# patrickfrey/strusPattern

Measured on AMD Instinct MI355X. Metric: GB/s input text scanned + matches/s, 10k-regex lexer + 10k-rule automaton, higher is better.
Workload: dtype u64; 1 GPU; configs[4] per-GPU shard: 10001 regexes + 10000 token rules, 12288 docs x 64KiB UTF-8 per step (the same 805 MB resident in HBM every step; configs[4] asks 32 GB per GPU: 39 such steps)

## Files before the change

### include/strus_pattern_amd.h

```cpp
#ifndef STRUS_PATTERN_AMD_H
#define STRUS_PATTERN_AMD_H
#include <stddef.h>
#include <stdint.h>

#ifdef __cplusplus
extern "C" {
#endif

#define SP_OK                    0
#define SP_ERR_INVALID          -1
#define SP_ERR_NOMEM            -2
#define SP_ERR_DEVICE           -3
#define SP_ERR_COMPILE          -4
#define SP_ERR_MATCH            -5
#define SP_ERR_UNAVAILABLE      -6

#define SP_DOC_OK                0
#define SP_DOC_ERR_ORDER         1
#define SP_DOC_ERR_ARENA         2
#define SP_DOC_ERR_KEYTRIGGERS   3
#define SP_DOC_ERR_PASTFOLLOW    4
#define SP_DOC_ERR_RANGE         5
#define SP_DOC_ERR_DATAREF       6
#define SP_DOC_ERR_LEXEMSIZE     7
#define SP_DOC_ERR_INTERNAL      8
#define SP_DOC_ERR_OUTPUT        9

enum sp_join_op {
	SP_OP_SEQUENCE = 0, SP_OP_SEQUENCE_IMM = 1, SP_OP_SEQUENCE_STRUCT = 2,
	SP_OP_WITHIN = 3, SP_OP_WITHIN_STRUCT = 4, SP_OP_ANY = 5, SP_OP_AND = 6
};

enum sp_position_bind {
	SP_BIND_CONTENT = 0, SP_BIND_SUCCESSOR = 1, SP_BIND_PREDECESSOR = 2, SP_BIND_UNIQUE = 3
};

typedef struct sp_lexem {
	uint32_t id;
	uint32_t ordpos;
	uint32_t origpos;
	uint32_t origsize;
} sp_lexem_t;

typedef struct sp_result {
	uint32_t handle;
	uint32_t ordpos;
	uint32_t ordend;
	uint32_t origseg;
	uint32_t origpos;
	uint32_t origendseg;
	uint32_t origend;
	uint32_t item_begin;
	uint32_t item_count;
} sp_result_t;

typedef struct sp_result_item {
	uint32_t variable;
	uint32_t ordpos;
	uint32_t ordend;
	uint32_t origseg;
	uint32_t origpos;
	uint32_t origendseg;
	uint32_t origend;
} sp_result_item_t;

typedef struct sp_matcher_stats {
	double nofProgramsInstalled;
	double nofAltKeyProgramsInstalled;
	double nofSignalsFired;
	double nofTriggersAvgActive;
} sp_matcher_stats_t;

typedef struct sp_matcher sp_matcher_t;
typedef struct sp_matcher_ctx sp_matcher_ctx_t;
typedef struct sp_lexer sp_lexer_t;
typedef struct sp_lexer_ctx sp_lexer_ctx_t;

const char* sp_version(void);
int sp_device_count(void);
void sp_free(void* p);
void sp_test_fail_alloc_above(uint64_t bytes);
struct sp_match_batch;
int sp_match_batch_regroup(const sp_result_t* results, uint64_t nresults, const sp_result_item_t* items, uint64_t nitems,
	const uint32_t* result_format, const uint32_t* item_format, const uint64_t* doc_ranges, const int32_t* doc_status,
	size_t batch_ndocs, size_t first_doc, size_t ndocs, int exclusive, uint32_t max_result_size,
	struct sp_match_batch* out, char* err, size_t errsize);


sp_matcher_t* sp_matcher_create(void);
void sp_matcher_free(sp_matcher_t* m);
const char* sp_matcher_last_error(const sp_matcher_t* m);

int sp_matcher_define_term_frequency(sp_matcher_t* m, uint32_t termid, double df);
int sp_matcher_push_term(sp_matcher_t* m, uint32_t termid);
int sp_matcher_push_expression(sp_matcher_t* m, int joinop, size_t argc, uint32_t range, uint32_t cardinality);
int sp_matcher_push_pattern(sp_matcher_t* m, const char* name);
int sp_matcher_attach_variable(sp_matcher_t* m, const char* name);
int sp_matcher_define_pattern(sp_matcher_t* m, const char* name, const char* formatstring, int visible);
int sp_matcher_define_option(sp_matcher_t* m, const char* name, double value);
int sp_matcher_compile(sp_matcher_t* m);
uint32_t sp_matcher_pattern_id(const sp_matcher_t* m, const char* name);
const char* sp_matcher_pattern_name(const sp_matcher_t* m, uint32_t handle);
uint32_t sp_matcher_variable_id(const sp_matcher_t* m, const char* name);
const char* sp_matcher_variable_name(const sp_matcher_t* m, uint32_t variable);
size_t sp_matcher_dump_table(const sp_matcher_t* m, uint32_t** out);
int sp_matcher_fast_tier(const sp_matcher_t* m, char* why, size_t whysize);
int sp_matcher_result_set_tier(const sp_matcher_t* m, char* why, size_t whysize, uint32_t* alt_programs);
int sp_matcher_launch_plan(const sp_matcher_t* m, uint32_t ctx_flags, unsigned num_cus, unsigned fast_blocks_per_cu,
                           size_t ndocs, size_t nlexems, size_t rerun_docs, uint32_t arena_grows,
                           uint64_t min_results, uint64_t min_items, char* buf, size_t bufsize);

int sp_matcher_serialize(const sp_matcher_t* m, void** blob, size_t* size);
sp_matcher_t* sp_matcher_deserialize(const void* blob, size_t size, char* err, size_t errsize);

uint32_t sp_matcher_format_count(const sp_matcher_t* m);
const char* sp_matcher_format_string(const sp_matcher_t* m, uint32_t format_handle);

sp_matcher_ctx_t* sp_matcher_ctx_create(const sp_matcher_t* m, int device);
#define SP_CTX_RESULT_SETS       1u
sp_matcher_ctx_t* sp_matcher_ctx_create_ex(const sp_matcher_t* m, int device, uint32_t flags);
void sp_matcher_ctx_free(sp_matcher_ctx_t* c);
const char* sp_matcher_ctx_last_error(const sp_matcher_ctx_t* c);

int sp_matcher_ctx_put_input(sp_matcher_ctx_t* c, const sp_lexem_t* lexems, const uint32_t* origseg, size_t n);
int sp_matcher_ctx_fetch_results(sp_matcher_ctx_t* c, sp_result_t** results, size_t* nresults,
                                 sp_result_item_t** items, size_t* nitems);
int sp_matcher_ctx_fetch_formats(sp_matcher_ctx_t* c, const uint32_t** result_format, const uint32_t** item_format);
int sp_matcher_ctx_statistics(sp_matcher_ctx_t* c, sp_matcher_stats_t* out);
int sp_matcher_ctx_reset(sp_matcher_ctx_t* c);

typedef struct sp_match_batch {
	size_t ndocs;
	size_t nresults;
	size_t nitems;
	sp_result_t* results;
	sp_result_item_t* items;
	uint64_t* doc_result_offsets;
	uint64_t* doc_stats;
	int32_t* doc_status;
	uint32_t* result_format;
	uint32_t* item_format;
} sp_match_batch_t;

int sp_matcher_ctx_match_docs(sp_matcher_ctx_t* c, const sp_lexem_t* lexems, const uint32_t* origseg,
                              const uint64_t* doc_offsets, size_t ndocs, sp_match_batch_t* out);
void sp_match_batch_free(sp_match_batch_t* b);

typedef struct sp_match_device_batch {
	size_t ndocs;
	void* d_results;
	void* d_items;
	void* d_doc_result_offsets;
	void* d_doc_stats;
	void* d_doc_status;
	void* d_counters;
	void* d_result_format;
	void* d_item_format;
} sp_match_device_batch_t;
int sp_matcher_ctx_match_docs_device(sp_matcher_ctx_t* c, const void* d_lexems, const void* d_origseg,
                                     const void* d_doc_offsets, size_t ndocs, size_t nlexems,
                                     void* stream, sp_match_device_batch_t* out);
int sp_matcher_ctx_match_lexed_device(sp_matcher_ctx_t* c, const void* d_lexems, const void* d_doc_ranges,
                                      size_t ndocs, size_t nlexems_hint, void* stream, sp_match_device_batch_t* out);
typedef struct sp_match_finished_batch {
	size_t ndocs;
	void* d_results;
	void* d_items;
	void* d_doc_result_offsets;
	void* d_doc_item_offsets;
	void* d_result_format;
	void* d_item_format;
	void* d_totals;
} sp_match_finished_batch_t;
int sp_matcher_ctx_batch_finish_device(sp_matcher_ctx_t* c, void* stream, sp_match_finished_batch_t* out);
#define SP_FINISH_CANONICAL      1u
int sp_matcher_ctx_batch_finish_device_ex(sp_matcher_ctx_t* c, void* stream, uint32_t flags, sp_match_finished_batch_t* out);
int sp_matcher_ctx_finished_fetch(sp_matcher_ctx_t* c, sp_match_batch_t* out);
int sp_matcher_ctx_last_finish_ms(sp_matcher_ctx_t* c, double* count_ms, double* offsets_ms, double* place_ms);
int sp_matcher_ctx_last_finish_sort_ms(sp_matcher_ctx_t* c, double* sort_ms);
uint32_t sp_matcher_finish_sort_tile(void);

#define SP_TEXT_RESULTS 1u
#define SP_TEXT_ITEMS   2u
typedef struct sp_text_source {
	const void* d_text;
	uint64_t nbytes;
	const void* d_seg_offsets;
	size_t nseg;
	const void* d_doc_seg_offsets;
} sp_text_source_t;
typedef struct sp_match_text_batch {
	size_t ndocs;
	void* d_result_text;
	void* d_result_text_offsets;
	void* d_item_text;
	void* d_item_text_offsets;
	void* d_doc_text_status;
	void* d_totals;
} sp_match_text_batch_t;
typedef struct sp_match_text {
	size_t ndocs;
	size_t nresults;
	size_t nitems;
	char* result_text;
	uint64_t* result_text_offsets;
	char* item_text;
	uint64_t* item_text_offsets;
	int32_t* doc_text_status;
	uint64_t totals[2];
} sp_match_text_t;
int sp_matcher_ctx_finished_text_device(sp_matcher_ctx_t* c, const sp_text_source_t* src, uint32_t flags, void* stream, sp_match_text_batch_t* out);
int sp_matcher_ctx_finished_text_fetch(sp_matcher_ctx_t* c, sp_match_text_t* out);
void sp_match_text_free(sp_match_text_t* t);
int sp_matcher_ctx_last_text_ms(sp_matcher_ctx_t* c, double* ms);
uint32_t sp_matcher_text_long_span(void);
int sp_match_batch_text(const sp_match_batch_t* mb, const char* text, uint64_t nbytes, const uint64_t* seg_offsets,
                        size_t nseg, const uint64_t* doc_seg_offsets, uint32_t flags,
                        sp_match_text_t* out, char* err, size_t errsize);

#define SP_VALUE_RESULTS 1u
#define SP_VALUE_ITEMS   2u
typedef struct sp_match_values_batch {
	size_t ndocs;
	void* d_result_values;
	void* d_result_value_offsets;
	void* d_item_values;
	void* d_item_value_offsets;
	void* d_doc_value_status;
	void* d_totals;
} sp_match_values_batch_t;
typedef struct sp_match_values {
	size_t ndocs;
	size_t nresults;
	size_t nitems;
	char* result_values;
	uint64_t* result_value_offsets;
	char* item_values;
	uint64_t* item_value_offsets;
	int32_t* doc_value_status;
	uint64_t totals[2];
} sp_match_values_t;
int sp_matcher_ctx_finished_values_device(sp_matcher_ctx_t* c, const sp_text_source_t* src, uint32_t flags, void* stream, sp_match_values_batch_t* out);
int sp_matcher_ctx_finished_values_fetch(sp_matcher_ctx_t* c, sp_match_values_t* out);
void sp_match_values_free(sp_match_values_t* v);
int sp_matcher_ctx_last_values_ms(sp_matcher_ctx_t* c, double* ms);
uint32_t sp_matcher_value_max_depth(void);
int sp_match_batch_values(const sp_matcher_t* m, const sp_match_batch_t* mb, const char* text, uint64_t nbytes,
                          const uint64_t* seg_offsets, size_t nseg, const uint64_t* doc_seg_offsets, uint32_t flags,
                          sp_match_values_t* out, char* err, size_t errsize);

typedef struct sp_pattern_freq {
	uint32_t handle;
	uint32_t count;
	uint32_t first_ordpos;
	uint32_t last_ordend;
} sp_pattern_freq_t;
typedef struct sp_pattern_freq_device {
	size_t ndocs;
	uint32_t handle_bound;
	void* d_records;
	void* d_doc_offsets;
	void* d_doc_freq_status;
	void* d_handle_results;
	void* d_handle_docs;
	void* d_totals;
} sp_pattern_freq_device_t;
typedef struct sp_pattern_freq_batch {
	size_t ndocs;
	size_t nrecords;
	uint32_t handle_bound;
	sp_pattern_freq_t* records;
	uint64_t* doc_offsets;
	int32_t* doc_freq_status;
	uint64_t* handle_results;
	uint32_t* handle_docs;
	uint64_t totals[1];
} sp_pattern_freq_batch_t;
uint32_t sp_matcher_handle_bound(const sp_matcher_t* m);
int sp_matcher_ctx_finished_pattern_freq_device(sp_matcher_ctx_t* c, void* stream, sp_pattern_freq_device_t* out);
int sp_matcher_ctx_finished_pattern_freq_fetch(sp_matcher_ctx_t* c, sp_pattern_freq_batch_t* out);
void sp_pattern_freq_batch_free(sp_pattern_freq_batch_t* b);
int sp_matcher_ctx_last_pattern_freq_ms(sp_matcher_ctx_t* c, double* ms);
uint32_t sp_matcher_pattern_freq_window(void);
int sp_match_batch_pattern_freq(const sp_match_batch_t* mb, uint32_t handle_bound, sp_pattern_freq_batch_t* out,
                                char* err, size_t errsize);

#define SP_TERM_VALUES 1u
#define SP_TERM_TEXT   2u
typedef struct sp_match_term {
	uint32_t handle;
	uint32_t count;
	uint32_t first_ordpos;
	uint32_t last_ordend;
	uint32_t first_result;
	uint32_t value_bytes;
} sp_match_term_t;
typedef struct sp_match_terms_device {
	size_t ndocs;
	uint32_t handle_bound;
	uint32_t flags;
	void* d_records;
	void* d_doc_term_offsets;
	void* d_result_term;
	void* d_doc_term_status;
	void* d_totals;
} sp_match_terms_device_t;
typedef struct sp_match_terms {
	size_t ndocs;
	size_t nresults;
	size_t nrecords;
	uint32_t handle_bound;
	uint32_t flags;
	sp_match_term_t* records;
	uint64_t* doc_term_offsets;
	uint32_t* result_term;
	int32_t* doc_term_status;
	uint64_t totals[1];
} sp_match_terms_t;
int sp_matcher_ctx_finished_terms_device(sp_matcher_ctx_t* c, uint32_t flags, void* stream, sp_match_terms_device_t* out);
int sp_matcher_ctx_finished_terms_fetch(sp_matcher_ctx_t* c, sp_match_terms_t* out);
void sp_match_terms_free(sp_match_terms_t* t);
int sp_matcher_ctx_last_terms_ms(sp_matcher_ctx_t* c, double* ms);
uint32_t sp_matcher_term_tile(void);
void sp_test_term_hash_bits(unsigned bits);
int sp_match_batch_terms(const sp_match_batch_t* mb, const sp_match_values_t* values, const sp_match_text_t* text,
                         uint32_t handle_bound, uint32_t flags, sp_match_terms_t* out, char* err, size_t errsize);

typedef struct sp_dict_term {
	uint32_t handle;
	uint32_t value_bytes;
	uint32_t first_doc;
	uint32_t first_term;
	uint32_t doc_freq;
	uint32_t max_count;
	uint64_t count;
} sp_dict_term_t;
typedef struct sp_match_dictionary_device {
	size_t ndocs;
	uint32_t handle_bound;
	uint32_t flags;
	void* d_records;
	void* d_term_dict;
	void* d_doc_dict_offsets;
	void* d_handle_terms;
	void* d_totals;
} sp_match_dictionary_device_t;
typedef struct sp_match_dictionary {
	size_t ndocs;
	size_t nterms;
	size_t ndict;
	uint32_t handle_bound;
	uint32_t flags;
	sp_dict_term_t* records;
	uint32_t* term_dict;
	uint64_t* doc_dict_offsets;
	uint32_t* handle_terms;
	uint64_t totals[1];
} sp_match_dictionary_t;
int sp_matcher_ctx_finished_dictionary_device(sp_matcher_ctx_t* c, void* stream, sp_match_dictionary_device_t* out);
int sp_matcher_ctx_finished_dictionary_fetch(sp_matcher_ctx_t* c, sp_match_dictionary_t* out);
void sp_match_dictionary_free(sp_match_dictionary_t* d);
int sp_matcher_ctx_last_dictionary_ms(sp_matcher_ctx_t* c, double* ms);
int sp_match_batch_dictionary(const sp_match_batch_t* mb, const sp_match_values_t* values, const sp_match_text_t* text,
                              const sp_match_terms_t* terms, sp_match_dictionary_t* out, char* err, size_t errsize);
int sp_matcher_ctx_batch_fetch(sp_matcher_ctx_t* c, sp_match_batch_t* out);
int sp_matcher_ctx_batch_fetch_docs(sp_matcher_ctx_t* c, size_t first_doc, size_t ndocs, sp_match_batch_t* out);
int sp_matcher_ctx_batch_counters(sp_matcher_ctx_t* c, uint64_t counters[8]);
double sp_matcher_ctx_last_kernel_ms(sp_matcher_ctx_t* c);
int sp_matcher_ctx_kernel_kind(const sp_matcher_ctx_t* c);
const char* sp_matcher_ctx_kernel_name(const sp_matcher_ctx_t* c);
int sp_matcher_ctx_batch_status(sp_matcher_ctx_t* c, int32_t* status, size_t ndocs);
int sp_matcher_ctx_grow_arena(sp_matcher_ctx_t* c);
int sp_matcher_ctx_reserve_output(sp_matcher_ctx_t* c, uint64_t results, uint64_t items);
int sp_matcher_ctx_set_arena(sp_matcher_ctx_t* c, uint32_t max_rules, uint32_t max_triggers, uint32_t bucket_capacity,
                             uint32_t max_items, uint32_t max_follow);


sp_lexer_t* sp_lexer_create(void);
void sp_lexer_free(sp_lexer_t* l);
const char* sp_lexer_last_error(const sp_lexer_t* l);

int sp_lexer_define_lexem_name(sp_lexer_t* l, uint32_t id, const char* name);
const char* sp_lexer_get_lexem_name(const sp_lexer_t* l, uint32_t id);
int sp_lexer_define_lexem(sp_lexer_t* l, uint32_t id, const char* expression, uint32_t resultIndex,
                          uint32_t level, int posbind);
int sp_lexer_define_symbol(sp_lexer_t* l, uint32_t symbolid, uint32_t patternid, const char* name);
uint32_t sp_lexer_get_symbol(const sp_lexer_t* l, uint32_t patternid, const char* name);
int sp_lexer_define_option(sp_lexer_t* l, const char* name, double value);
int sp_lexer_compile(sp_lexer_t* l);
int sp_lexer_serialize(const sp_lexer_t* l, void** blob, size_t* size);
sp_lexer_t* sp_lexer_deserialize(const void* blob, size_t size, char* err, size_t errsize);
size_t sp_lexer_dump_tables(const sp_lexer_t* l, uint64_t** out);
size_t sp_lexer_dump_image(const sp_lexer_t* l, int which, uint64_t** out);
int sp_lexer_launch_plan(const sp_lexer_t* l, unsigned num_cus, size_t ndocs, size_t nbytes, char* buf, size_t bufsize);

sp_lexer_ctx_t* sp_lexer_ctx_create(const sp_lexer_t* l, int device);
void sp_lexer_ctx_free(sp_lexer_ctx_t* c);
const char* sp_lexer_ctx_last_error(const sp_lexer_ctx_t* c);
int sp_lexer_ctx_match(sp_lexer_ctx_t* c, const char* src, size_t srclen, sp_lexem_t** lexems, size_t* nlexems);
int sp_lexer_ctx_reset(sp_lexer_ctx_t* c);

typedef struct sp_lex_batch {
	size_t ndocs;
	size_t nlexems;
	sp_lexem_t* lexems;
	uint64_t* doc_lexem_offsets;
	int32_t* doc_status;
} sp_lex_batch_t;
int sp_lexer_ctx_match_docs(sp_lexer_ctx_t* c, const char* text, const uint64_t* doc_offsets, size_t ndocs, sp_lex_batch_t* out);
void sp_lex_batch_free(sp_lex_batch_t* b);

typedef struct sp_lex_device_batch {
	size_t ndocs;
	void* d_lexems;
	void* d_doc_ranges;
	void* d_doc_status;
	void* d_counters;
} sp_lex_device_batch_t;
int sp_lexer_ctx_match_docs_device(sp_lexer_ctx_t* c, const void* d_text, const void* d_doc_offsets,
                                   size_t ndocs, size_t nbytes, void* stream, sp_lex_device_batch_t* out);
int sp_lexer_ctx_batch_fetch_docs(sp_lexer_ctx_t* c, size_t first_doc, size_t ndocs, sp_lex_batch_t* out);
typedef struct sp_lex_stitched_batch {
	size_t ndocs;
	void* d_lexems;
	void* d_origseg;
	void* d_doc_offsets;
	void* d_doc_status;
	void* d_totals;
} sp_lex_stitched_batch_t;
int sp_lexer_ctx_stitch_segments_device(sp_lexer_ctx_t* c, const void* d_doc_seg_offsets, size_t ndocs,
                                        void* stream, sp_lex_stitched_batch_t* out);
int sp_lexer_ctx_stitched_fetch(sp_lexer_ctx_t* c, sp_lex_batch_t* out, uint32_t** origseg);
int sp_lexer_ctx_stitched_status(sp_lexer_ctx_t* c, int32_t* status, size_t ndocs, size_t* ndocs_stitched);
int sp_lexer_ctx_last_stitch_ms(sp_lexer_ctx_t* c, double* ms);
int sp_lexer_ctx_batch_counters(sp_lexer_ctx_t* c, uint64_t counters[8]);
int sp_lexer_ctx_batch_status(sp_lexer_ctx_t* c, int32_t* status, size_t ndocs);
double sp_lexer_ctx_last_kernel_ms(sp_lexer_ctx_t* c);
int sp_lexer_ctx_last_kernel_ms_split(sp_lexer_ctx_t* c, double* scan_ms, double* post_ms);
int sp_lexer_ctx_last_kernel_ms_split3(sp_lexer_ctx_t* c, double* scan_ms, double* words_ms, double* post_ms);
const char* sp_lexer_ctx_scan_kernel_name(const sp_lexer_ctx_t* c);
const char* sp_lexer_ctx_words_kernel_name(const sp_lexer_ctx_t* c);
int sp_lexer_ctx_reserve_output(sp_lexer_ctx_t* c, uint64_t lexems);
int sp_lexer_ctx_grow_arena(sp_lexer_ctx_t* c);

#ifdef __cplusplus
}
#endif
#endif
```

### struspattern_amd/__init__.py

```python
import ctypes

import numpy as np

from . import capi
from .capi import SpLexem, SpResult, SpResultItem

__all__ = ["PatternMatcher", "PatternMatcherInstance", "PatternMatcherContext", "PatternLexer", "PatternLexerInstance",
           "PatternLexerContext", "PatternError", "JOIN_OP", "POSITION_BIND", "matchSegmentedDocs", "MatchText", "batchText", "MatchValues", "batchValues", "PatternFreq", "batchPatternFreq", "MatchTerms", "batchTerms", "MatchDictionary", "batchDictionary"]

SP_CTX_RESULT_SETS = 1
SP_FINISH_CANONICAL = 1
SP_TEXT_RESULTS, SP_TEXT_ITEMS = 1, 2
SP_VALUE_RESULTS, SP_VALUE_ITEMS = 1, 2
SP_TERM_VALUES, SP_TERM_TEXT = 1, 2
SP_ERR_UNAVAILABLE = -6

JOIN_OP = {"sequence": 0, "sequence_imm": 1, "sequence_struct": 2, "within": 3, "within_struct": 4, "any": 5, "and": 6}

DOC_STATUS = {
    0: "ok", 1: "term events not fed in ascending order", 2: "working set of the document exceeds the arena",
    3: "pattern with too many identical key events defined", 4: "internal: encountered past trigger with follow",
    5: "term event out of range", 6: "illegal free of event data reference",
}

# ... 372 lines not shown
            return _match_batch_of(b)
        finally:
            self._L.sp_match_batch_free(ctypes.byref(b))

    def matchDocsDevice(self, d_lexems, d_doc_offsets, ndocs, nlexems, stream=0, d_origseg=0):
        out = capi.SpMatchDeviceBatch()
        rc = self._L.sp_matcher_ctx_match_docs_device(self._h, d_lexems, d_origseg or None, d_doc_offsets, ndocs, nlexems, stream or None, ctypes.byref(out))
        if rc != 0:
            raise PatternError("device batch match failed (%d): %s" % (rc, self._err()))
        return out

    def matchLexedDevice(self, d_lexems, d_doc_ranges, ndocs, nlexems_hint, stream=0):
        out = capi.SpMatchDeviceBatch()
        rc = self._L.sp_matcher_ctx_match_lexed_device(self._h, d_lexems, d_doc_ranges, ndocs, nlexems_hint, stream or None, ctypes.byref(out))
        if rc != 0:
            raise PatternError("device batch match failed (%d): %s" % (rc, self._err()))
        return out

    def batchFinishDevice(self, stream=0, canonical=False):
        out = capi.SpMatchFinishedBatch()
        rc = self._L.sp_matcher_ctx_batch_finish_device_ex(self._h, stream or None, SP_FINISH_CANONICAL if canonical else 0, ctypes.byref(out))
        if rc != 0:
            raise PatternError("finishing the batch on the device failed (%d): %s" % (rc, self._err()))
        return out

    def finishedFetch(self):
        return self._fetched(self._L.sp_matcher_ctx_finished_fetch)

    def _fetch_product(self, struct_type, call, free, convert, what):
        return _product(struct_type, lambda s: call(self._h, ctypes.byref(s)), free, convert,
                        lambda rc: "fetching %s failed (%d): %s" % (what, rc, self._err()))

    def _last_ms(self, fn, what):
        a = ctypes.c_double(-1.0)
        if fn(self._h, ctypes.byref(a)) != 0:
            raise PatternError("no timed " + what)
        return a.value

    def lastFinishMs(self):
        a, b, d = ctypes.c_double(-1.0), ctypes.c_double(-1.0), ctypes.c_double(-1.0)
        if self._L.sp_matcher_ctx_last_finish_ms(self._h, ctypes.byref(a), ctypes.byref(b), ctypes.byref(d)) != 0:
            raise PatternError("no timed finish")
        return a.value, b.value, d.value

    def lastFinishSortMs(self):
        return self._last_ms(self._L.sp_matcher_ctx_last_finish_sort_ms, "finish")

    def finishedTextDevice(self, d_text, nbytes, d_seg_offsets, nseg, d_doc_seg_offsets=0, results=True, items=True, stream=0):
        src = capi.SpTextSource(d_text or None, nbytes, d_seg_offsets or None, nseg, d_doc_seg_offsets or None)
        out = capi.SpMatchTextBatch()
        flags = (SP_TEXT_RESULTS if results else 0) | (SP_TEXT_ITEMS if items else 0)
        rc = self._L.sp_matcher_ctx_finished_text_device(self._h, ctypes.byref(src), flags, stream or None, ctypes.byref(out))
        if rc != 0:
            raise PatternError("gathering the text of the batch on the device failed (%d): %s" % (rc, self._err()))
        return out

    def finishedTextFetch(self):
        return self._fetch_product(capi.SpMatchText, self._L.sp_matcher_ctx_finished_text_fetch, self._L.sp_match_text_free, _match_text_of, "the text of the batch")

    def lastTextMs(self):
        return self._last_ms(self._L.sp_matcher_ctx_last_text_ms, "text call")

    def finishedValuesDevice(self, d_text, nbytes, d_seg_offsets, nseg, d_doc_seg_offsets=0, flags=SP_VALUE_RESULTS | SP_VALUE_ITEMS, stream=0):
        src = capi.SpTextSource(d_text or None, nbytes, d_seg_offsets or None, nseg, d_doc_seg_offsets or None)
        out = capi.SpMatchValuesBatch()
        rc = self._L.sp_matcher_ctx_finished_values_device(self._h, ctypes.byref(src), flags, stream or None, ctypes.byref(out))
        if rc != 0:
            raise PatternError("building the values of the batch on the device failed (%d): %s" % (rc, self._err()))
        return out

    def finishedValuesFetch(self):
        return self._fetch_product(capi.SpMatchValues, self._L.sp_matcher_ctx_finished_values_fetch, self._L.sp_match_values_free, _match_values_of, "the values of the batch")

    def lastValuesMs(self):
        return self._last_ms(self._L.sp_matcher_ctx_last_values_ms, "values call")

    def finishedPatternFreqDevice(self, stream=0):
        out = capi.SpPatternFreqDevice()
        rc = self._L.sp_matcher_ctx_finished_pattern_freq_device(self._h, stream or None, ctypes.byref(out))
        if rc != 0:
            raise PatternError("summing the pattern frequencies of the batch on the device failed (%d): %s" % (rc, self._err()))
        return out

    def finishedPatternFreqFetch(self):
        return self._fetch_product(capi.SpPatternFreqBatch, self._L.sp_matcher_ctx_finished_pattern_freq_fetch, self._L.sp_pattern_freq_batch_free, _pattern_freq_of,
                                   "the pattern frequencies of the batch")

    def lastPatternFreqMs(self):
        return self._last_ms(self._L.sp_matcher_ctx_last_pattern_freq_ms, "pattern frequency call")

    def finishedTermsDevice(self, flags=SP_TERM_VALUES | SP_TERM_TEXT, stream=0):
        out = capi.SpMatchTermsDevice()
        rc = self._L.sp_matcher_ctx_finished_terms_device(self._h, flags, stream or None, ctypes.byref(out))
        if rc != 0:
            raise PatternError("grouping the terms of the batch on the device failed (%d): %s" % (rc, self._err()))
        return out

    def finishedTermsFetch(self):
        return self._fetch_product(capi.SpMatchTerms, self._L.sp_matcher_ctx_finished_terms_fetch, self._L.sp_match_terms_free, _match_terms_of, "the terms of the batch")

    def lastTermsMs(self):
        return self._last_ms(self._L.sp_matcher_ctx_last_terms_ms, "terms call")

    def finishedDictionaryDevice(self, stream=0):
        out = capi.SpMatchDictionaryDevice()
        rc = self._L.sp_matcher_ctx_finished_dictionary_device(self._h, stream or None, ctypes.byref(out))
        if rc != 0:
            raise PatternError("building the dictionary of the batch on the device failed (%d): %s" % (rc, self._err()))
        return out

    def finishedDictionaryFetch(self):
        return self._fetch_product(capi.SpMatchDictionary, self._L.sp_matcher_ctx_finished_dictionary_fetch, self._L.sp_match_dictionary_free,
                                   _match_dictionary_of, "the dictionary of the batch")

    def lastDictionaryMs(self):
        return self._last_ms(self._L.sp_matcher_ctx_last_dictionary_ms, "dictionary call")

    def batchFetch(self, first_doc=None, ndocs=None):
        if first_doc is None:
            return self._fetched(self._L.sp_matcher_ctx_batch_fetch)
        return self._fetched(lambda h, b: self._L.sp_matcher_ctx_batch_fetch_docs(h, first_doc, ndocs, b))

    def _fetched(self, call):
        return self._fetch_product(capi.SpMatchBatch, call, self._L.sp_match_batch_free, _match_batch_of, "the batch")

    def batchCounters(self):
        arr = (ctypes.c_uint64 * 8)()
        rc = self._L.sp_matcher_ctx_batch_counters(self._h, arr)
        if rc != 0:
            raise PatternError("reading batch counters failed: " + self._err())
        return {"results": arr[0], "items": arr[1], "events": arr[2], "failed_docs": arr[3], "handed_over": arr[4], "prof": [arr[4], arr[5], arr[6], arr[7]]}

    def batchStatus(self, ndocs):
        st = np.zeros(ndocs, np.int32)
        rc = self._L.sp_matcher_ctx_batch_status(self._h, st.ctypes.data, ndocs)
        if rc != 0:
            raise PatternError("reading batch status failed: " + self._err())
        return st

    def growArena(self):
        return self._L.sp_matcher_ctx_grow_arena(self._h) == 0

    def reserveOutput(self, results, items):
        self._L.sp_matcher_ctx_reserve_output(self._h, results, items)

    def lastKernelMs(self):
        return self._L.sp_matcher_ctx_last_kernel_ms(self._h)

    def kernelKind(self):
        return self._L.sp_matcher_ctx_kernel_kind(self._h)

    def kernelName(self):
        return self._L.sp_matcher_ctx_kernel_name(self._h).decode()


def _serialize(L, fn, handle, err):
    blob = ctypes.c_void_p()
    size = ctypes.c_size_t()
    if fn(handle, ctypes.byref(blob), ctypes.byref(size)) != 0:
        raise PatternError("serialisation failed: " + err())
    try:
        return ctypes.string_at(blob, size.value)
    finally:
        L.sp_free(blob)


class PatternMatcherInstance:

    def __init__(self, _handle=None):
        self._L = capi.lib()
        self._h = _handle or self._L.sp_matcher_create()
        if not self._h:
            raise PatternError("failed to create pattern matcher instance")

    def serialize(self):
        return _serialize(self._L, self._L.sp_matcher_serialize, self._h, lambda: self._L.sp_matcher_last_error(self._h).decode())

    @classmethod
    def deserialize(cls, blob):
        L = capi.lib()
        err = ctypes.create_string_buffer(256)
        h = L.sp_matcher_deserialize(blob, len(blob), err, 256)
        if not h:
            raise PatternError("cannot load the rule set: " + err.value.decode())
        return cls(_handle=h)

    def __del__(self):
        try:
            if self._h:
                self._L.sp_matcher_free(self._h)
        except Exception:
            pass

    def _chk(self, rc, what):
        if rc != 0:
            raise PatternError("%s: %s" % (what, self._L.sp_matcher_last_error(self._h).decode()))

    def defineTermFrequency(self, termid, df):
        self._chk(self._L.sp_matcher_define_term_frequency(self._h, termid, df), "failed to define term frequency")

    def pushTerm(self, termid):
        self._chk(self._L.sp_matcher_push_term(self._h, termid), "failed to push term on the pattern match expression stack")

    def pushExpression(self, joinop, argc, range_, cardinality=0):
        op = JOIN_OP[joinop] if isinstance(joinop, str) else int(joinop)
        self._chk(self._L.sp_matcher_push_expression(self._h, op, argc, range_, cardinality), "failed to push expression on the pattern match expression stack")

    def pushPattern(self, name):
        self._chk(self._L.sp_matcher_push_pattern(self._h, name.encode()), "failed to push pattern reference on the pattern match expression stack")

    def attachVariable(self, name):
        self._chk(self._L.sp_matcher_attach_variable(self._h, name.encode()), "failed to attach variable to top element of the pattern match expression stack")

    def definePattern(self, name, formatstring="", visible=True):
        self._chk(self._L.sp_matcher_define_pattern(self._h, name.encode(), formatstring.encode(), int(visible)), "failed to close pattern definition on the pattern match expression stack")

    def defineOption(self, name, value=0.0):
        self._chk(self._L.sp_matcher_define_option(self._h, name.encode(), value), "failed to define pattern matching automaton option")

    def compile(self):
        self._chk(self._L.sp_matcher_compile(self._h), "failed to compile (optimize) pattern matching automaton")
        return True

    def createContext(self, device=0, result_sets=False):
        return PatternMatcherContext(self, device, result_sets)

    def handleBound(self):
        return self._L.sp_matcher_handle_bound(self._h)

    def patternId(self, name):
        return self._L.sp_matcher_pattern_id(self._h, name.encode())

    def patternName(self, handle):
        s = self._L.sp_matcher_pattern_name(self._h, handle)
        return s.decode() if s else None

    def variableId(self, name):
        return self._L.sp_matcher_variable_id(self._h, name.encode())

    def variableName(self, vid):
        s = self._L.sp_matcher_variable_name(self._h, vid)
        return s.decode() if s else None

    def formatCount(self):
        return int(self._L.sp_matcher_format_count(self._h))

    def formatString(self, handle):
        s = self._L.sp_matcher_format_string(self._h, handle)
        return s.decode() if s else None

    def fastTier(self):
        buf = ctypes.create_string_buffer(256)
        ok = self._L.sp_matcher_fast_tier(self._h, buf, 256)
        return bool(ok), buf.value.decode()

    def resultSetTier(self):
        buf = ctypes.create_string_buffer(256)
        alt = ctypes.c_uint32(0)
        ok = self._L.sp_matcher_result_set_tier(self._h, buf, 256, ctypes.byref(alt))
        return bool(ok), buf.value.decode(), int(alt.value)

    def launchPlan(self, num_cus, ndocs, nlexems, result_sets=False, fast_blocks_per_cu=16, rerun_docs=0, arena_grows=0, min_results=0, min_items=0):
        buf = ctypes.create_string_buffer(2048)
        self._chk(self._L.sp_matcher_launch_plan(self._h, 1 if result_sets else 0, num_cus, fast_blocks_per_cu, ndocs, nlexems, rerun_docs, arena_grows,
                                                 min_results, min_items, buf, 2048), "no launch plan")
        return dict(f.split("=", 1) for f in buf.value.decode().split("\n") if f)

    def dumpTable(self):
        p = ctypes.POINTER(ctypes.c_uint32)()
        n = self._L.sp_matcher_dump_table(self._h, ctypes.byref(p))
        arr = np.ctypeslib.as_array(p, shape=(n,)).copy() if n else np.zeros(0, np.uint32)
        self._L.sp_free(p)
        return arr

    def name(self):
        return "std"


class PatternMatcher:

    def getCompileOptionNames(self):
        return ["stopwordOccurrenceFactor", "weightFactor", "maxRange", "exclusive", "maxResultSize"]

    def createInstance(self):
        return PatternMatcherInstance()

    def name(self):
        return "std"


POSITION_BIND = {"content": 0, "successor": 1, "predecessor": 2, "unique": 3}


class LexBatch:
    def __init__(self, lexems, doc_offsets, status):
        self.lexems = lexems
        self.doc_offsets = doc_offsets
        self.status = status

    def doc(self, i):
        return self.lexems[self.doc_offsets[i]:self.doc_offsets[i + 1]]


def _lex_batch_of(b):
    return LexBatch(_rows(b.lexems, b.nlexems, 4), _rows(b.doc_lexem_offsets, b.ndocs + 1, 0, ctypes.c_uint64), _rows(b.doc_status, b.ndocs, 0, ctypes.c_int32))

# ... 294 lines not shown
```

### struspattern_amd/capi.py

```python
import ctypes
import os

from . import build as _build

c_u32 = ctypes.c_uint32
c_u64 = ctypes.c_uint64
c_vp = ctypes.c_void_p
c_cp = ctypes.c_char_p
P = ctypes.POINTER


class SpLexem(ctypes.Structure):
    _fields_ = [("id", c_u32), ("ordpos", c_u32), ("origpos", c_u32), ("origsize", c_u32)]


class SpResult(ctypes.Structure):
    _fields_ = [(n, c_u32) for n in ("handle", "ordpos", "ordend", "origseg", "origpos", "origendseg", "origend", "item_begin", "item_count")]


class SpResultItem(ctypes.Structure):
    _fields_ = [(n, c_u32) for n in ("variable", "ordpos", "ordend", "origseg", "origpos", "origendseg", "origend")]


class SpMatcherStats(ctypes.Structure):
    _fields_ = [(n, ctypes.c_double) for n in ("nofProgramsInstalled", "nofAltKeyProgramsInstalled", "nofSignalsFired", "nofTriggersAvgActive")]


class SpMatchBatch(ctypes.Structure):
    _fields_ = [
        ("ndocs", ctypes.c_size_t), ("nresults", ctypes.c_size_t), ("nitems", ctypes.c_size_t),
        ("results", P(SpResult)), ("items", P(SpResultItem)),
        ("doc_result_offsets", P(c_u64)), ("doc_stats", P(c_u64)), ("doc_status", P(ctypes.c_int32)),
        ("result_format", P(c_u32)), ("item_format", P(c_u32)),
    ]


class SpLexBatch(ctypes.Structure):
    _fields_ = [
        ("ndocs", ctypes.c_size_t), ("nlexems", ctypes.c_size_t), ("lexems", P(SpLexem)),
        ("doc_lexem_offsets", P(c_u64)), ("doc_status", P(ctypes.c_int32)),
    ]


class SpLexDeviceBatch(ctypes.Structure):
    _fields_ = [("ndocs", ctypes.c_size_t), ("d_lexems", c_vp), ("d_doc_ranges", c_vp), ("d_doc_status", c_vp), ("d_counters", c_vp)]


class SpLexStitchedBatch(ctypes.Structure):
    _fields_ = [("ndocs", ctypes.c_size_t), ("d_lexems", c_vp), ("d_origseg", c_vp), ("d_doc_offsets", c_vp), ("d_doc_status", c_vp), ("d_totals", c_vp)]


class SpMatchDeviceBatch(ctypes.Structure):
    _fields_ = [
        ("ndocs", ctypes.c_size_t), ("d_results", c_vp), ("d_items", c_vp), ("d_doc_result_offsets", c_vp),
        ("d_doc_stats", c_vp), ("d_doc_status", c_vp), ("d_counters", c_vp),
        ("d_result_format", c_vp), ("d_item_format", c_vp),
    ]


class SpMatchFinishedBatch(ctypes.Structure):
    _fields_ = [
        ("ndocs", ctypes.c_size_t), ("d_results", c_vp), ("d_items", c_vp), ("d_doc_result_offsets", c_vp),
        ("d_doc_item_offsets", c_vp), ("d_result_format", c_vp), ("d_item_format", c_vp), ("d_totals", c_vp),
    ]


class SpTextSource(ctypes.Structure):
    _fields_ = [("d_text", c_vp), ("nbytes", c_u64), ("d_seg_offsets", c_vp), ("nseg", ctypes.c_size_t), ("d_doc_seg_offsets", c_vp)]


class SpMatchTextBatch(ctypes.Structure):
    _fields_ = [
        ("ndocs", ctypes.c_size_t), ("d_result_text", c_vp), ("d_result_text_offsets", c_vp), ("d_item_text", c_vp),
        ("d_item_text_offsets", c_vp), ("d_doc_text_status", c_vp), ("d_totals", c_vp),
    ]


class SpMatchText(ctypes.Structure):
    _fields_ = [
        ("ndocs", ctypes.c_size_t), ("nresults", ctypes.c_size_t), ("nitems", ctypes.c_size_t),
        ("result_text", P(ctypes.c_uint8)), ("result_text_offsets", P(c_u64)), ("item_text", P(ctypes.c_uint8)), ("item_text_offsets", P(c_u64)),
        ("doc_text_status", P(ctypes.c_int32)), ("totals", c_u64 * 2),
    ]


class SpMatchValuesBatch(ctypes.Structure):
    _fields_ = [
        ("ndocs", ctypes.c_size_t), ("d_result_values", c_vp), ("d_result_value_offsets", c_vp), ("d_item_values", c_vp),
        ("d_item_value_offsets", c_vp), ("d_doc_value_status", c_vp), ("d_totals", c_vp),
    ]


class SpMatchValues(ctypes.Structure):
    _fields_ = [
        ("ndocs", ctypes.c_size_t), ("nresults", ctypes.c_size_t), ("nitems", ctypes.c_size_t),
        ("result_values", P(ctypes.c_uint8)), ("result_value_offsets", P(c_u64)), ("item_values", P(ctypes.c_uint8)), ("item_value_offsets", P(c_u64)),
        ("doc_value_status", P(ctypes.c_int32)), ("totals", c_u64 * 2),
    ]


class SpPatternFreq(ctypes.Structure):
    _fields_ = [(n, c_u32) for n in ("handle", "count", "first_ordpos", "last_ordend")]


class SpPatternFreqDevice(ctypes.Structure):
    _fields_ = [
        ("ndocs", ctypes.c_size_t), ("handle_bound", c_u32), ("d_records", c_vp), ("d_doc_offsets", c_vp), ("d_doc_freq_status", c_vp),
        ("d_handle_results", c_vp), ("d_handle_docs", c_vp), ("d_totals", c_vp),
    ]


class SpPatternFreqBatch(ctypes.Structure):
    _fields_ = [
        ("ndocs", ctypes.c_size_t), ("nrecords", ctypes.c_size_t), ("handle_bound", c_u32),
        ("records", P(SpPatternFreq)), ("doc_offsets", P(c_u64)), ("doc_freq_status", P(ctypes.c_int32)),
        ("handle_results", P(c_u64)), ("handle_docs", P(c_u32)), ("totals", c_u64 * 1),
    ]


class SpMatchTerm(ctypes.Structure):
    _fields_ = [(n, c_u32) for n in ("handle", "count", "first_ordpos", "last_ordend", "first_result", "value_bytes")]


class SpMatchTermsDevice(ctypes.Structure):
    _fields_ = [
        ("ndocs", ctypes.c_size_t), ("handle_bound", c_u32), ("flags", c_u32), ("d_records", c_vp), ("d_doc_term_offsets", c_vp),
        ("d_result_term", c_vp), ("d_doc_term_status", c_vp), ("d_totals", c_vp),
    ]


class SpMatchTerms(ctypes.Structure):
    _fields_ = [
        ("ndocs", ctypes.c_size_t), ("nresults", ctypes.c_size_t), ("nrecords", ctypes.c_size_t), ("handle_bound", c_u32), ("flags", c_u32),
        ("records", P(SpMatchTerm)), ("doc_term_offsets", P(c_u64)), ("result_term", P(c_u32)), ("doc_term_status", P(ctypes.c_int32)),
        ("totals", c_u64 * 1),
    ]


class SpDictTerm(ctypes.Structure):
    _fields_ = [(n, c_u32) for n in ("handle", "value_bytes", "first_doc", "first_term", "doc_freq", "max_count")] + [("count", c_u64)]


class SpMatchDictionaryDevice(ctypes.Structure):
    _fields_ = [
        ("ndocs", ctypes.c_size_t), ("handle_bound", c_u32), ("flags", c_u32), ("d_records", c_vp), ("d_term_dict", c_vp),
        ("d_doc_dict_offsets", c_vp), ("d_handle_terms", c_vp), ("d_totals", c_vp),
    ]


class SpMatchDictionary(ctypes.Structure):
    _fields_ = [
        ("ndocs", ctypes.c_size_t), ("nterms", ctypes.c_size_t), ("ndict", ctypes.c_size_t), ("handle_bound", c_u32), ("flags", c_u32),
        ("records", P(SpDictTerm)), ("term_dict", P(c_u32)), ("doc_dict_offsets", P(c_u64)), ("handle_terms", P(c_u32)),
        ("totals", c_u64 * 1),
    ]


SIGNATURES = {
    "sp_version": (c_cp, []),
    "sp_device_count": (ctypes.c_int, []),
    "sp_free": (None, [c_vp]),
    "sp_test_fail_alloc_above": (None, [c_u64]),
    "sp_match_batch_regroup": (ctypes.c_int, [c_vp, c_u64, c_vp, c_u64, c_vp, c_vp, c_vp, c_vp, ctypes.c_size_t, ctypes.c_size_t, ctypes.c_size_t,
                                              ctypes.c_int, c_u32, P(SpMatchBatch), ctypes.c_char_p, ctypes.c_size_t]),
    "sp_matcher_create": (c_vp, []),
    "sp_matcher_free": (None, [c_vp]),
    "sp_matcher_last_error": (c_cp, [c_vp]),
    "sp_matcher_define_term_frequency": (ctypes.c_int, [c_vp, c_u32, ctypes.c_double]),
    "sp_matcher_push_term": (ctypes.c_int, [c_vp, c_u32]),
    "sp_matcher_push_expression": (ctypes.c_int, [c_vp, ctypes.c_int, ctypes.c_size_t, c_u32, c_u32]),
    "sp_matcher_push_pattern": (ctypes.c_int, [c_vp, c_cp]),
    "sp_matcher_attach_variable": (ctypes.c_int, [c_vp, c_cp]),
    "sp_matcher_define_pattern": (ctypes.c_int, [c_vp, c_cp, c_cp, ctypes.c_int]),
    "sp_matcher_define_option": (ctypes.c_int, [c_vp, c_cp, ctypes.c_double]),
    "sp_matcher_compile": (ctypes.c_int, [c_vp]),
    "sp_matcher_pattern_id": (c_u32, [c_vp, c_cp]),
    "sp_matcher_pattern_name": (c_cp, [c_vp, c_u32]),
    "sp_matcher_variable_id": (c_u32, [c_vp, c_cp]),
    "sp_matcher_variable_name": (c_cp, [c_vp, c_u32]),
    "sp_matcher_dump_table": (ctypes.c_size_t, [c_vp, P(P(c_u32))]),
    "sp_matcher_fast_tier": (ctypes.c_int, [c_vp, ctypes.c_char_p, ctypes.c_size_t]),
    "sp_matcher_result_set_tier": (ctypes.c_int, [c_vp, ctypes.c_char_p, ctypes.c_size_t, P(c_u32)]),
    "sp_matcher_launch_plan": (ctypes.c_int, [c_vp, c_u32, ctypes.c_uint, ctypes.c_uint, ctypes.c_size_t, ctypes.c_size_t, ctypes.c_size_t, c_u32, c_u64, c_u64, ctypes.c_char_p, ctypes.c_size_t]),
    "sp_matcher_serialize": (ctypes.c_int, [c_vp, P(c_vp), P(ctypes.c_size_t)]),
    "sp_matcher_deserialize": (c_vp, [c_vp, ctypes.c_size_t, ctypes.c_char_p, ctypes.c_size_t]),
    "sp_lexer_serialize": (ctypes.c_int, [c_vp, P(c_vp), P(ctypes.c_size_t)]),
    "sp_lexer_deserialize": (c_vp, [c_vp, ctypes.c_size_t, ctypes.c_char_p, ctypes.c_size_t]),
    "sp_matcher_format_count": (c_u32, [c_vp]),
    "sp_matcher_format_string": (c_cp, [c_vp, c_u32]),
    "sp_matcher_ctx_fetch_formats": (ctypes.c_int, [c_vp, P(P(c_u32)), P(P(c_u32))]),
    "sp_matcher_ctx_create": (c_vp, [c_vp, ctypes.c_int]),
    "sp_matcher_ctx_create_ex": (c_vp, [c_vp, ctypes.c_int, c_u32]),
    "sp_matcher_ctx_free": (None, [c_vp]),
    "sp_matcher_ctx_last_error": (c_cp, [c_vp]),
    "sp_matcher_ctx_put_input": (ctypes.c_int, [c_vp, c_vp, c_vp, ctypes.c_size_t]),
    "sp_matcher_ctx_fetch_results": (ctypes.c_int, [c_vp, P(P(SpResult)), P(ctypes.c_size_t), P(P(SpResultItem)), P(ctypes.c_size_t)]),
    "sp_matcher_ctx_statistics": (ctypes.c_int, [c_vp, P(SpMatcherStats)]),
    "sp_matcher_ctx_reset": (ctypes.c_int, [c_vp]),
    "sp_matcher_ctx_match_docs": (ctypes.c_int, [c_vp, c_vp, c_vp, c_vp, ctypes.c_size_t, P(SpMatchBatch)]),
    "sp_match_batch_free": (None, [P(SpMatchBatch)]),
    "sp_matcher_ctx_match_docs_device": (ctypes.c_int, [c_vp, c_vp, c_vp, c_vp, ctypes.c_size_t, ctypes.c_size_t, c_vp, P(SpMatchDeviceBatch)]),
    "sp_matcher_ctx_match_lexed_device": (ctypes.c_int, [c_vp, c_vp, c_vp, ctypes.c_size_t, ctypes.c_size_t, c_vp, P(SpMatchDeviceBatch)]),
    "sp_matcher_ctx_batch_fetch": (ctypes.c_int, [c_vp, P(SpMatchBatch)]),
    "sp_matcher_ctx_batch_fetch_docs": (ctypes.c_int, [c_vp, ctypes.c_size_t, ctypes.c_size_t, P(SpMatchBatch)]),
    "sp_matcher_ctx_batch_finish_device": (ctypes.c_int, [c_vp, c_vp, P(SpMatchFinishedBatch)]),
    "sp_matcher_ctx_batch_finish_device_ex": (ctypes.c_int, [c_vp, c_vp, c_u32, P(SpMatchFinishedBatch)]),
    "sp_matcher_ctx_finished_fetch": (ctypes.c_int, [c_vp, P(SpMatchBatch)]),
    "sp_matcher_ctx_last_finish_ms": (ctypes.c_int, [c_vp, P(ctypes.c_double), P(ctypes.c_double), P(ctypes.c_double)]),
    "sp_matcher_ctx_last_finish_sort_ms": (ctypes.c_int, [c_vp, P(ctypes.c_double)]),
    "sp_matcher_finish_sort_tile": (c_u32, []),
    "sp_matcher_ctx_finished_text_device": (ctypes.c_int, [c_vp, P(SpTextSource), c_u32, c_vp, P(SpMatchTextBatch)]),
    "sp_matcher_ctx_finished_text_fetch": (ctypes.c_int, [c_vp, P(SpMatchText)]),
    "sp_match_text_free": (None, [P(SpMatchText)]),
    "sp_matcher_ctx_last_text_ms": (ctypes.c_int, [c_vp, P(ctypes.c_double)]),
    "sp_matcher_text_long_span": (c_u32, []),
    "sp_matcher_ctx_finished_values_device": (ctypes.c_int, [c_vp, P(SpTextSource), c_u32, c_vp, P(SpMatchValuesBatch)]),
    "sp_matcher_ctx_finished_values_fetch": (ctypes.c_int, [c_vp, P(SpMatchValues)]),
    "sp_match_values_free": (None, [P(SpMatchValues)]),
    "sp_matcher_ctx_last_values_ms": (ctypes.c_int, [c_vp, P(ctypes.c_double)]),
    "sp_matcher_value_max_depth": (c_u32, []),
    "sp_match_batch_values": (ctypes.c_int, [c_vp, P(SpMatchBatch), c_vp, c_u64, c_vp, ctypes.c_size_t, c_vp, c_u32, P(SpMatchValues), ctypes.c_char_p, ctypes.c_size_t]),
    "sp_match_batch_text": (ctypes.c_int, [P(SpMatchBatch), c_vp, c_u64, c_vp, ctypes.c_size_t, c_vp, c_u32, P(SpMatchText), ctypes.c_char_p, ctypes.c_size_t]),
    "sp_matcher_handle_bound": (c_u32, [c_vp]),
    "sp_matcher_ctx_finished_pattern_freq_device": (ctypes.c_int, [c_vp, c_vp, P(SpPatternFreqDevice)]),
    "sp_matcher_ctx_finished_pattern_freq_fetch": (ctypes.c_int, [c_vp, P(SpPatternFreqBatch)]),
    "sp_pattern_freq_batch_free": (None, [P(SpPatternFreqBatch)]),
    "sp_matcher_ctx_last_pattern_freq_ms": (ctypes.c_int, [c_vp, P(ctypes.c_double)]),
    "sp_matcher_pattern_freq_window": (c_u32, []),
    "sp_match_batch_pattern_freq": (ctypes.c_int, [P(SpMatchBatch), c_u32, P(SpPatternFreqBatch), ctypes.c_char_p, ctypes.c_size_t]),
    "sp_matcher_ctx_finished_terms_device": (ctypes.c_int, [c_vp, c_u32, c_vp, P(SpMatchTermsDevice)]),
    "sp_matcher_ctx_finished_terms_fetch": (ctypes.c_int, [c_vp, P(SpMatchTerms)]),
    "sp_match_terms_free": (None, [P(SpMatchTerms)]),
    "sp_matcher_ctx_last_terms_ms": (ctypes.c_int, [c_vp, P(ctypes.c_double)]),
    "sp_matcher_term_tile": (c_u32, []),
    "sp_test_term_hash_bits": (None, [ctypes.c_uint]),
    "sp_match_batch_terms": (ctypes.c_int, [P(SpMatchBatch), P(SpMatchValues), P(SpMatchText), c_u32, c_u32, P(SpMatchTerms), ctypes.c_char_p, ctypes.c_size_t]),
    "sp_matcher_ctx_finished_dictionary_device": (ctypes.c_int, [c_vp, c_vp, P(SpMatchDictionaryDevice)]),
    "sp_matcher_ctx_finished_dictionary_fetch": (ctypes.c_int, [c_vp, P(SpMatchDictionary)]),
    "sp_match_dictionary_free": (None, [P(SpMatchDictionary)]),
    "sp_matcher_ctx_last_dictionary_ms": (ctypes.c_int, [c_vp, P(ctypes.c_double)]),
    "sp_match_batch_dictionary": (ctypes.c_int, [P(SpMatchBatch), P(SpMatchValues), P(SpMatchText), P(SpMatchTerms), P(SpMatchDictionary), ctypes.c_char_p, ctypes.c_size_t]),
    "sp_matcher_ctx_batch_counters": (ctypes.c_int, [c_vp, P(c_u64)]),
    "sp_matcher_ctx_last_kernel_ms": (ctypes.c_double, [c_vp]),
    "sp_matcher_ctx_kernel_kind": (ctypes.c_int, [c_vp]),
    "sp_matcher_ctx_kernel_name": (ctypes.c_char_p, [c_vp]),
    "sp_matcher_ctx_batch_status": (ctypes.c_int, [c_vp, c_vp, ctypes.c_size_t]),
    "sp_matcher_ctx_grow_arena": (ctypes.c_int, [c_vp]),
    "sp_matcher_ctx_reserve_output": (ctypes.c_int, [c_vp, c_u64, c_u64]),
    "sp_matcher_ctx_set_arena": (ctypes.c_int, [c_vp, c_u32, c_u32, c_u32, c_u32, c_u32]),
    "sp_lexer_create": (c_vp, []),
    "sp_lexer_free": (None, [c_vp]),
    "sp_lexer_last_error": (c_cp, [c_vp]),
    "sp_lexer_define_lexem_name": (ctypes.c_int, [c_vp, c_u32, c_cp]),
    "sp_lexer_get_lexem_name": (c_cp, [c_vp, c_u32]),
    "sp_lexer_define_lexem": (ctypes.c_int, [c_vp, c_u32, c_cp, c_u32, c_u32, ctypes.c_int]),
    "sp_lexer_define_symbol": (ctypes.c_int, [c_vp, c_u32, c_u32, c_cp]),
    "sp_lexer_get_symbol": (c_u32, [c_vp, c_u32, c_cp]),
    "sp_lexer_define_option": (ctypes.c_int, [c_vp, c_cp, ctypes.c_double]),
    "sp_lexer_compile": (ctypes.c_int, [c_vp]),
    "sp_lexer_dump_tables": (ctypes.c_size_t, [c_vp, P(P(c_u64))]),
    "sp_lexer_dump_image": (ctypes.c_size_t, [c_vp, ctypes.c_int, P(P(c_u64))]),
    "sp_lexer_launch_plan": (ctypes.c_int, [c_vp, ctypes.c_uint, ctypes.c_size_t, ctypes.c_size_t, ctypes.c_char_p, ctypes.c_size_t]),
    "sp_lexer_ctx_create": (c_vp, [c_vp, ctypes.c_int]),
    "sp_lexer_ctx_free": (None, [c_vp]),
    "sp_lexer_ctx_last_error": (c_cp, [c_vp]),
    "sp_lexer_ctx_match": (ctypes.c_int, [c_vp, c_cp, ctypes.c_size_t, P(P(SpLexem)), P(ctypes.c_size_t)]),
    "sp_lexer_ctx_reset": (ctypes.c_int, [c_vp]),
    "sp_lexer_ctx_match_docs": (ctypes.c_int, [c_vp, c_cp, c_vp, ctypes.c_size_t, P(SpLexBatch)]),
    "sp_lex_batch_free": (None, [P(SpLexBatch)]),
    "sp_lexer_ctx_match_docs_device": (ctypes.c_int, [c_vp, c_vp, c_vp, ctypes.c_size_t, ctypes.c_size_t, c_vp, P(SpLexDeviceBatch)]),
    "sp_lexer_ctx_batch_fetch_docs": (ctypes.c_int, [c_vp, ctypes.c_size_t, ctypes.c_size_t, P(SpLexBatch)]),
    "sp_lexer_ctx_stitch_segments_device": (ctypes.c_int, [c_vp, c_vp, ctypes.c_size_t, c_vp, P(SpLexStitchedBatch)]),
    "sp_lexer_ctx_stitched_fetch": (ctypes.c_int, [c_vp, P(SpLexBatch), P(P(c_u32))]),
    "sp_lexer_ctx_stitched_status": (ctypes.c_int, [c_vp, c_vp, ctypes.c_size_t, P(ctypes.c_size_t)]),
    "sp_lexer_ctx_last_stitch_ms": (ctypes.c_int, [c_vp, P(ctypes.c_double)]),
    "sp_lexer_ctx_batch_counters": (ctypes.c_int, [c_vp, P(c_u64)]),
    "sp_lexer_ctx_batch_status": (ctypes.c_int, [c_vp, c_vp, ctypes.c_size_t]),
    "sp_lexer_ctx_last_kernel_ms": (ctypes.c_double, [c_vp]),
    "sp_lexer_ctx_last_kernel_ms_split": (ctypes.c_int, [c_vp, ctypes.POINTER(ctypes.c_double), ctypes.POINTER(ctypes.c_double)]),
    "sp_lexer_ctx_scan_kernel_name": (ctypes.c_char_p, [c_vp]),
    "sp_lexer_ctx_words_kernel_name": (ctypes.c_char_p, [c_vp]),
    "sp_lexer_ctx_last_kernel_ms_split3": (ctypes.c_int, [c_vp, ctypes.POINTER(ctypes.c_double), ctypes.POINTER(ctypes.c_double), ctypes.POINTER(ctypes.c_double)]),
    "sp_lexer_ctx_reserve_output": (ctypes.c_int, [c_vp, c_u64]),
    "sp_lexer_ctx_grow_arena": (ctypes.c_int, [c_vp]),
}

_LIB = None


def lib():
    global _LIB
    if _LIB is None:
        path = _build.LIB
        if _build.needs_build():
            path = _build.build()
        L = ctypes.CDLL(path, mode=ctypes.RTLD_GLOBAL)
        for name, (res, args) in SIGNATURES.items():
            fn = getattr(L, name)
            fn.restype = res
            fn.argtypes = args
        _LIB = L
    return _LIB
```

### struspattern_amd/csrc/capi_l2.cpp

```cpp
#include "capi_l2_ctx.hpp"
#include <cstdio>

namespace {

L2Engine engineOf( const sp_matcher* m, uint32_t flags, const L2Switches& sw, FlatTables& ft)
{
	m->compiler.flatten( ft);
	return chooseL2Engine( m->compiler, ft, flags, sw);
}

FlatPlan flatPlanOf( const L2Engine& e, const L2Switches& sw)
{
	const char size[ 2] = {sw.fastSize, 0};
	const unsigned variant = fastVariantNamed( size);
	uint32_t R = 0, T = 0;
	fastCapacities( variant, R, T);
	return planFlat( e.flat, variant, fastKernelName( variant), R, T);
}

int tierQuery( const sp_matcher* m, uint32_t flags, L2EngineKind kind, char* why, size_t whysize, uint32_t* altPrograms)
{
	if (altPrograms) *altPrograms = 0;
	try
	{
		FlatTables ft;
		const L2Engine e = engineOf( m, flags, L2Switches(), ft);
		const std::string& reason = kind == L2_JOIN ? e.join.whyNot : e.flat.whyNot;
		copyText( why, whysize, reason.c_str());
		if (altPrograms) *altPrograms = e.altPrograms;
		return reason.empty() ? 1 : 0;
	}
	catch (const std::exception& e)
	{
		copyText( why, whysize, e.what());
		return 0;
	}
}

}

extern "C" {

const char* sp_version(void) { return "struspattern_amd 0.1 (gfx950)"; }

int sp_device_count(void)
{
	int n = 0;
	if (hipGetDeviceCount( &n) != hipSuccess) return 0;
	return n;
}

void sp_free( void* p) { std::free( p); }

void sp_test_fail_alloc_above( uint64_t bytes) { allocFailureThreshold().store( bytes, std::memory_order_relaxed); }

sp_matcher_t* sp_matcher_create(void) { try { return new sp_matcher(); } catch (...) { return 0; } }
void sp_matcher_free( sp_matcher_t* m) { delete m; }
const char* sp_matcher_last_error( const sp_matcher_t* m) { return m->lasterror.c_str(); }

#define MGUARD( CODE, BODY) return guardedCall( m->lasterror, CODE, [&]{ BODY; })

int sp_matcher_define_term_frequency( sp_matcher_t* m, uint32_t termid, double df)
{ MGUARD( SP_ERR_INVALID, m->compiler.defineTermFrequency( termid, df)); }
int sp_matcher_push_term( sp_matcher_t* m, uint32_t termid)
{ MGUARD( SP_ERR_INVALID, m->compiler.pushTerm( termid)); }
int sp_matcher_push_expression( sp_matcher_t* m, int joinop, size_t argc, uint32_t range, uint32_t cardinality)
{ MGUARD( SP_ERR_INVALID, m->compiler.pushExpression( joinop, argc, range, cardinality)); }
int sp_matcher_push_pattern( sp_matcher_t* m, const char* name)
{ MGUARD( SP_ERR_INVALID, m->compiler.pushPattern( name ? name : "")); }
int sp_matcher_attach_variable( sp_matcher_t* m, const char* name)
{ MGUARD( SP_ERR_INVALID, m->compiler.attachVariable( name ? name : "")); }
int sp_matcher_define_pattern( sp_matcher_t* m, const char* name, const char* formatstring, int visible)
{ MGUARD( SP_ERR_INVALID, m->compiler.definePattern( name ? name : "", formatstring ? formatstring : "", visible != 0)); }
int sp_matcher_define_option( sp_matcher_t* m, const char* name, double value)
{ MGUARD( SP_ERR_INVALID, m->compiler.defineOption( name ? name : "", value)); }
int sp_matcher_compile( sp_matcher_t* m)
{ MGUARD( SP_ERR_COMPILE, m->compiler.compile(); m->compiled = true; m->formats( true)); }

uint32_t sp_matcher_pattern_id( const sp_matcher_t* m, const char* name) { return m->compiler.patterns().get( name); }
const char* sp_matcher_pattern_name( const sp_matcher_t* m, uint32_t handle) { return m->compiler.patterns().key( handle); }
uint32_t sp_matcher_variable_id( const sp_matcher_t* m, const char* name) { return m->compiler.variables().get( name); }
const char* sp_matcher_variable_name( const sp_matcher_t* m, uint32_t variable) { return m->compiler.variables().key( variable); }

uint32_t sp_matcher_handle_bound( const sp_matcher_t* m) { return (uint32_t)m->compiler.patterns().names().size() + 1; }

uint32_t sp_matcher_format_count( const sp_matcher_t* m) { return m->compiler.formatCount(); }
const char* sp_matcher_format_string( const sp_matcher_t* m, uint32_t format_handle) { return m->compiler.formatString( format_handle); }

int sp_matcher_ctx_kernel_kind( const sp_matcher_ctx_t* c) { return c->kind; }
const char* sp_matcher_ctx_kernel_name( const sp_matcher_ctx_t* c) { return l2KernelName( c->kind, &c->flat.plan); }

int sp_matcher_fast_tier( const sp_matcher_t* m, char* why, size_t whysize)
{ return tierQuery( m, 0, L2_FLAT, why, whysize, 0); }

int sp_matcher_result_set_tier( const sp_matcher_t* m, char* why, size_t whysize, uint32_t* alt_programs)
{ return tierQuery( m, SP_CTX_RESULT_SETS, L2_JOIN, why, whysize, alt_programs); }

int sp_matcher_launch_plan( const sp_matcher_t* m, uint32_t ctx_flags, unsigned num_cus, unsigned fast_blocks_per_cu, size_t ndocs, size_t nlexems,
			    size_t rerun_docs, uint32_t arena_grows, uint64_t min_results, uint64_t min_items, char* buf, size_t bufsize)
{
	if (buf && bufsize) buf[ 0] = 0;
	return guardedCall( m->lasterror, SP_ERR_INVALID, [&]{
		if (ctx_flags & ~(uint32_t)SP_CTX_RESULT_SETS) throw std::runtime_error( "unknown context flags");
		const L2Switches sw = L2Switches::fromEnv();
		FlatTables ft;
		const L2Engine e = engineOf( m, ctx_flags, sw, ft);
		const FlatPlan fp = e.flat.on ? flatPlanOf( e, sw) : FlatPlan();
		ArenaLayout arena = initialArena();
		arena.nStop = ft.nofStopWords;
		for (uint32_t i=0; i<arena_grows; ++i) if (!growArena( arena)) throw std::runtime_error( "arena at its maximum size");
		const L2LaunchPlan p = planL2Launch( e.kind(), rerun_docs != 0, num_cus ? num_cus : 256u, fast_blocks_per_cu, rerun_docs ? rerun_docs : ndocs, ndocs, nlexems,
							arena, &fp, min_results, min_items);
		static const char* const engines[] = {"general", "flat", "join"};
		static const char* const routes[] = {"general", "flat+list", "join", "rerun-list"};
		int n = std::snprintf( buf, bufsize, "engine=%s\nkind=%d\nflat_why_not=%s\njoin_why_not=%s\nalt_programs=%u\nkernel=%s\nroute=%s\n"
			"general_blocks=%u\narena_run=%u\narena_alloc=%u\narena_alloc_waves=%u\narena_per_wave_bytes=%zu\narena_max_rules=%u\narena_scratch_cap=%u\nstop_words=%u\n"
			"fast_blocks=%u\nspill_alloc_waves=%llu\nspill_per_wave_bytes=%zu\nlist_blocks=%u\njoin_blocks=%u\nwant_results=%llu\nwant_items=%llu\n"
			"R=%u\nT=%u\nexp_shift=%u\nspill_words=%u\nmax_rules=%u\nmax_staged=%u\nbucket_caps=",
			engines[ e.kind()], (int)e.kind(), e.flat.whyNot.c_str(), e.join.whyNot.c_str(), e.altPrograms, p.kernelName, routes[ p.route],
			p.generalBlocks, p.arena.run, p.arena.alloc, p.arenaAllocWaves, p.arenaPerWaveBytes, p.layout.maxRules, p.layout.scratchCap, ft.nofStopWords,
			p.fastBlocks, (unsigned long long)p.spillAllocWaves, p.spillPerWaveBytes, p.listBlocks, p.joinBlocks, (unsigned long long)p.wantResults, (unsigned long long)p.wantItems,
			fp.R, fp.T, fp.expShift, fp.spill.totalWords, fp.spill.maxRules, fp.spill.maxStaged);
		for (int b=0; b<16 && n >= 0 && buf && (size_t)n < bufsize; ++b) n += std::snprintf( buf+n, bufsize-n, b ? ",%u" : "%u", fp.bucketMeta[ b] >> 16);
		if (n < 0 || !buf || (size_t)n >= bufsize) throw std::runtime_error( "buffer too small for the launch plan");
	});
}

int sp_matcher_serialize( const sp_matcher_t* m, void** blob, size_t* size)
{ return exportBlob( m->lasterror, blob, size, [&]( std::vector<uint8_t>& buf){ m->compiler.save( buf, m->compiled); }); }
sp_matcher_t* sp_matcher_deserialize( const void* blob, size_t size, char* err, size_t errsize)
{ return importBlob<sp_matcher>( err, errsize, [&]( sp_matcher& m){ m.compiled = m.compiler.load( blob, size); m.formats( true); }); }

size_t sp_matcher_dump_table( const sp_matcher_t* m, uint32_t** out)
{
	std::vector<uint32_t> buf = m->compiler.dump();
	*out = (uint32_t*)std::malloc( buf.size()*sizeof(uint32_t) + 4);
	if (!*out) return 0;
	std::memcpy( *out, buf.data(), buf.size()*sizeof(uint32_t));
	return buf.size();
}

sp_matcher_ctx_t* sp_matcher_ctx_create( const sp_matcher_t* m, int device) { return sp_matcher_ctx_create_ex( m, device, 0); }

sp_matcher_ctx_t* sp_matcher_ctx_create_ex( const sp_matcher_t* m, int device, uint32_t flags)
{
	sp_matcher_ctx* c = 0;
	if (flags & ~(uint32_t)SP_CTX_RESULT_SETS)
	{
		m->lasterror = "unknown context flags";
		return 0;
	}
	try
	{
		c = new sp_matcher_ctx();
		c->inst = m; c->device = device;
		int ndev = 0;
		hipError_t e = hipGetDeviceCount( &ndev);
		if (e != hipSuccess || ndev <= 0 || device < 0 || device >= ndev)
		{
			m->lasterror = "no usable HIP device: the rule automaton runs on the GPU only (no CPU fallback)";
			delete c; return 0;
		}
		HIP_CHECK( hipSetDevice( device));
		hipDeviceProp_t prop;
		HIP_CHECK( hipGetDeviceProperties( &prop, device));
		c->numCUs = prop.multiProcessorCount > 0 ? (unsigned)prop.multiProcessorCount : 256u;

		c->sw = L2Switches::fromEnv();
		FlatTables ft;
		const L2Engine engine = engineOf( m, flags, c->sw, ft);
		c->kind = engine.kind();
		c->exact.dPrograms.upload( ft.programs.data(), ft.programs.size()*sizeof(DevProgram));
		c->exact.dTrigdefs.upload( ft.trigdefs.data(), ft.trigdefs.size()*sizeof(DevTrigDef));
		c->exact.dKeytab.upload( ft.keytab.data(), ft.keytab.size()*sizeof(DevKeyEntry));
		c->exact.dKeylist.upload( ft.keylist.data(), ft.keylist.size()*sizeof(DevKeyRef));
		c->exact.keymask = (uint32_t)ft.keytab.size()-1;
		c->exact.nofStopWords = ft.nofStopWords;
		c->exact.layout.nStop = ft.nofStopWords;
		c->io.withFormats = m->compiler.formatCount() != 0;
		c->flat.on = engine.flat.on; c->flat.whyNot = engine.flat.whyNot;
		if (c->flat.on)
		{
			c->flat.dKeyinst.upload( engine.flat.keyinst.data(), engine.flat.keyinst.size()*sizeof(FastKeyInst));
			c->flat.dStatics.upload( engine.flat.statics.data(), engine.flat.statics.size()*sizeof(FastStatic));
			c->flat.plan = flatPlanOf( engine, c->sw);
			c->flat.blocksPerCU = (unsigned)fastBlocksPerCU( c->flat.plan.variant);
		}
		if (c->sw.verbose) fprintf( stderr, "[spa] fast tier: %s\n", c->flat.on ? "on" : c->flat.whyNot.c_str());
		c->join.on = engine.join.on; c->join.whyNot = engine.join.whyNot;
		if (c->join.on)
		{
			const L2Engine::Join& j = engine.join;
			c->join.dKeytab.upload( j.keytab.data(), j.keytab.size()*sizeof(JoinKey)); c->join.dRules.upload( j.rules.data(), j.rules.size()*sizeof(JoinRule)); c->join.dFilter.upload( j.filter.data(), j.filter.size()*sizeof(uint32_t));
			c->join.keymask = (uint32_t)j.keytab.size()-1; c->join.maxRange = j.maxRange; c->join.delimiter = j.delimiter;
			c->join.altRules = engine.altPrograms != 0;
		}
		if (c->sw.verbose && engine.join.asked) fprintf( stderr, "[spa] result-set mode: %s\n", c->join.on ? "join kernel" : c->join.whyNot.c_str());
		c->io.dCursor.alloc( 256);
		c->io.dCounters.alloc( SPC_COUNT*sizeof(uint64_t));
		c->own.create( device);
		c->evStart.create(); c->evStop.create();
		return c;
	}
	catch (const std::exception& e)
	{
		m->lasterror = e.what();
		delete c;
		return 0;
	}
}

void sp_matcher_ctx_free( sp_matcher_ctx_t* c) { delete c; }
const char* sp_matcher_ctx_last_error( const sp_matcher_ctx_t* c) { return c->lasterror.c_str(); }

int sp_matcher_ctx_set_arena( sp_matcher_ctx_t* c, uint32_t max_rules, uint32_t max_triggers, uint32_t bucket_capacity,
				uint32_t max_items, uint32_t max_follow)
{
	setArena( c->exact.layout, max_rules, max_triggers, bucket_capacity, max_items, max_follow);
	c->exact.arena.count = 0;
	return SP_OK;
}

}

namespace {

void copyOutBatch( sp_matcher_ctx* c, size_t firstDoc, size_t ndocs, const BatchCounts& counts, sp_match_batch_t* out)
{
	MatchBatchSource src;
	src.results = (const sp_result_t*)c->io.results.ptr(); src.nresults = counts.results;
	src.items = (const sp_result_item_t*)c->io.items.ptr(); src.nitems = counts.items;
	src.resultFormat = c->io.withFormats ? (const uint32_t*)c->io.dResultFormat.ptr : 0;
	src.itemFormat = c->io.withFormats ? (const uint32_t*)c->io.dItemFormat.ptr : 0;
	src.docRange = (const uint64_t*)c->io.dDocRange.ptr; src.docStatus = (const int32_t*)c->io.dDocStatus.ptr;
	src.docStats = (const uint64_t*)c->io.dDocStats.ptr;
	src.ndocs = c->lastNdocs;
	fetchMatchBatch( src, firstDoc, ndocs, c->inst->compiler.exclusive(), c->inst->compiler.maxResultSize(), deviceToHost( c->own), out);
}

}

extern "C" {

int sp_matcher_ctx_batch_fetch_docs( sp_matcher_ctx_t* c, size_t first_doc, size_t ndocs, sp_match_batch_t* out)
{
	std::memset( out, 0, sizeof(*out));
	return guardedCall( c->lasterror, SP_ERR_DEVICE, [&]{
		HIP_CHECK( hipSetDevice( c->device));
		HIP_CHECK( hipStreamSynchronize( c->lastStream));
		copyOutBatch( c, first_doc, ndocs, readCounts( c), out);
	});
}

int sp_matcher_ctx_batch_fetch( sp_matcher_ctx_t* c, sp_match_batch_t* out) { return sp_matcher_ctx_batch_fetch_docs( c, 0, c->lastNdocs, out); }

int sp_matcher_ctx_batch_status( sp_matcher_ctx_t* c, int32_t* status, size_t ndocs) { return batchStatus( c, c->io.dDocStatus, status, ndocs); }

int sp_matcher_ctx_grow_arena( sp_matcher_ctx_t* c)
{
	if (!growArena( c->exact.layout)) { c->lasterror = "arena at its maximum size"; return SP_ERR_INVALID; }
	c->exact.arena.count = 0;
	return SP_OK;
}

int sp_matcher_ctx_reserve_output( sp_matcher_ctx_t* c, uint64_t results, uint64_t items)
{
	if (results > c->io.minResults) c->io.minResults = results;
	if (items > c->io.minItems) c->io.minItems = items;
	return SP_OK;
}

}

namespace {

L2BatchIO batchIO( sp_matcher_ctx* c, const void* d_lexems, const void* d_origseg, const void* d_doc_offsets, const void* d_doc_ranges, size_t ndocs)
{
	L2BatchIO io;
	std::memset( &io, 0, sizeof(io));
	io.lexems = (const uint32_t*)d_lexems; io.origseg = (const uint32_t*)d_origseg;
	io.docOffsets = (const uint64_t*)d_doc_offsets; io.docRangesIn = (const uint64_t*)d_doc_ranges;
	io.ndocs = (uint32_t)ndocs; io.withItems = c->io.withItems ? 1u : 0u;
	io.docCursor = (uint32_t*)c->io.dCursor.ptr;
	io.counters = (uint64_t*)c->io.dCounters.ptr;
	io.results = (uint32_t*)c->io.results.ptr(); io.resultCapacity = c->io.results.count;
	io.items = (uint32_t*)c->io.items.ptr(); io.itemCapacity = c->io.items.count;
	io.docRange = (uint64_t*)c->io.dDocRange.ptr; io.docStats = (uint64_t*)c->io.dDocStats.ptr; io.docStatus = (int32_t*)c->io.dDocStatus.ptr;
	io.withFormats = c->io.withFormats ? 1u : 0u;
	io.resultFormat = (uint32_t*)c->io.dResultFormat.ptr; io.itemFormat = (uint32_t*)c->io.dItemFormat.ptr;
	return io;
}


void ensureArena( sp_matcher_ctx* c, const L2LaunchPlan& plan)
{
	if (c->exact.arena.count < plan.arena.run)
	{
		const ArenaLayout& L = plan.layout;
		if (c->sw.verbose) fprintf( stderr, "[spa] arena: rules %u bucket %u items %u refs %u staged %u winCap %u -> %.2f MB per wave, %u waves\n", L.maxRules, L.bucketCap, L.maxItems, L.maxRefs, L.maxStaged, L.winCap, L.totalWords*4/1e6, plan.arena.run);
		c->exact.arena.realloc( plan.arenaAllocWaves, plan.arenaPerWaveBytes);
	}
}

void ensureOutput( sp_matcher_ctx* c, const L2LaunchPlan& plan, size_t ndocs)
{
	sp_matcher_ctx::BatchIO& io = c->io;
	io.results.ensure( plan.wantResults, sizeof(sp_result_t));
	io.items.ensure( plan.wantItems, sizeof(sp_result_item_t));
	if (io.withFormats)
	{
		io.dResultFormat.reserve( io.results.count*sizeof(uint32_t));
		io.dItemFormat.reserve( io.items.count*2*sizeof(uint32_t));
	}
	io.dDocRange.reserve( (ndocs+1)*2*sizeof(uint64_t));
	io.dDocStats.reserve( (ndocs+1)*4*sizeof(uint64_t));
	io.dDocStatus.reserve( (ndocs+1)*sizeof(int32_t));
}

void resetCursorAndCounters( sp_matcher_ctx* c, bool rerun, hipStream_t stream)
{
	HIP_CHECK( hipMemsetAsync( c->io.dCursor.ptr, 0, 256, stream));
	if (!rerun) HIP_CHECK( hipMemsetAsync( c->io.dCounters.ptr, 0, SPC_COUNT*sizeof(uint64_t), stream));
	else HIP_CHECK( hipMemsetAsync( (uint64_t*)c->io.dCounters.ptr + SPC_FAILED, 0, sizeof(uint64_t), stream));
}

L2Params generalParams( const sp_matcher_ctx* c, const L2BatchIO& io, const L2LaunchPlan& plan)
{
	L2Params P;
	std::memset( &P, 0, sizeof(P));
	P.programs = (const DevProgram*)c->exact.dPrograms.ptr;
	P.trigdefs = (const DevTrigDef*)c->exact.dTrigdefs.ptr;
	P.keytab = (const DevKeyEntry*)c->exact.dKeytab.ptr;
	P.keylist = (const DevKeyRef*)c->exact.dKeylist.ptr;
	P.keymask = c->exact.keymask; P.nofStopWords = c->exact.nofStopWords;
	P.io = io;
	P.arenaBase = (uint32_t*)c->exact.arena.ptr(); P.arena = plan.layout;
	return P;
}

void listMode( const sp_matcher_ctx* c, L2Params& P)
{
	P.docList = (const uint32_t*)c->exact.dDocList.ptr; P.docListCount = (const uint32_t*)c->io.dCursor.ptr + 2;
	P.io.docCursor = (uint32_t*)c->io.dCursor.ptr + 1;
}

void launchRerun( sp_matcher_ctx* c, L2Params P, const L2LaunchPlan& plan, const std::vector<uint32_t>& rerun, hipStream_t stream)
{
	const uint32_t n = (uint32_t)rerun.size();
	c->exact.dDocList.reserve( ((size_t)P.io.ndocs+1)*sizeof(uint32_t));
	HIP_CHECK( hipMemcpyAsync( c->exact.dDocList.ptr, rerun.data(), n*sizeof(uint32_t), hipMemcpyHostToDevice, stream));
	HIP_CHECK( hipMemcpyAsync( (uint32_t*)c->io.dCursor.ptr + 2, &n, sizeof(uint32_t), hipMemcpyHostToDevice, stream));
	HIP_CHECK( hipStreamSynchronize( stream));
	listMode( c, P);
	HIP_CHECK( launchL2Match( P, plan.generalBlocks, stream));
}

void launchJoin( sp_matcher_ctx* c, const L2BatchIO& io, const L2LaunchPlan& plan, size_t nlexems, hipStream_t stream)
{
	JoinParams J;
	std::memset( &J, 0, sizeof(J));
	c->join.dCounts.reserve( (nlexems + 64) * sizeof(uint32_t));
	J.filter = (const uint32_t*)c->join.dFilter.ptr; J.counts = (uint32_t*)c->join.dCounts.ptr; J.countsCapacity = nlexems;
	J.keytab = (const JoinKey*)c->join.dKeytab.ptr; J.keymask = c->join.keymask; J.rules = (const JoinRule*)c->join.dRules.ptr; J.maxRange = c->join.maxRange; J.delimiter = c->join.delimiter; J.altRules = c->join.altRules ? 1u : 0u;
	J.io = io;
	HIP_CHECK( launchL2Join( J, plan.joinBlocks, stream));
}

void launchFlat( sp_matcher_ctx* c, L2Params P, const L2LaunchPlan& plan, hipStream_t stream)
{
	sp_matcher_ctx::Flat& f = c->flat;
	const size_t ndocs = P.io.ndocs;
	if (f.spill.count < plan.fastBlocks)
	{
		f.spill.realloc( plan.spillAllocWaves, plan.spillPerWaveBytes);
		if (c->sw.verbose) fprintf( stderr, "[spa] fast tier: %u waves/CU, LDS capacities R %u T %u, spill %.2f MB per wave\n", f.blocksPerCU, f.plan.R, f.plan.T, f.plan.spill.totalWords*4/1e6);
	}
	c->exact.dDocList.reserve( (ndocs+1)*sizeof(uint32_t));
	FastParams F;
	std::memset( &F, 0, sizeof(F));
	F.keyinst = (const FastKeyInst*)f.dKeyinst.ptr; F.statics = (const FastStatic*)f.dStatics.ptr; F.keytab = (const FastKeyEntry*)c->exact.dKeytab.ptr;
	F.keymask = c->exact.keymask; F.nofStopWords = c->exact.nofStopWords;
	F.io = P.io;
	std::memcpy( F.bucketMeta, f.plan.bucketMeta, sizeof(F.bucketMeta)); F.expShift = f.plan.expShift;
	F.spill = f.plan.spill; F.spillBase = (uint32_t*)f.spill.ptr();
	F.fallbackList = (uint32_t*)c->exact.dDocList.ptr; F.fallbackCount = (uint32_t*)c->io.dCursor.ptr + 2;
	F.diag = (uint32_t*)c->io.dCursor.ptr + 16; F.prof = (uint64_t*)((uint32_t*)c->io.dCursor.ptr + 32);
	HIP_CHECK( launchL2Fast( F, f.plan.variant, plan.fastBlocks, stream));
	listMode( c, P);
	HIP_CHECK( launchL2Match( P, plan.listBlocks, stream));
}

void launchBatch( sp_matcher_ctx* c, const void* d_lexems, const void* d_origseg, const void* d_doc_offsets,
		  size_t ndocs, size_t nlexems, hipStream_t stream, const void* d_doc_ranges=0, const std::vector<uint32_t>* rerun=0)
{
	const L2LaunchPlan plan = planL2Launch( c->kind, rerun != 0, c->numCUs, c->flat.blocksPerCU, rerun ? rerun->size() : ndocs, ndocs, nlexems,
						c->exact.layout, &c->flat.plan, c->io.minResults, c->io.minItems);
	HIP_CHECK( hipSetDevice( c->device));
	c->prod.drop();
	ensureArena( c, plan);
	ensureOutput( c, plan, ndocs);
	resetCursorAndCounters( c, rerun != 0, stream);
	const L2BatchIO io = batchIO( c, d_lexems, d_origseg, d_doc_offsets, d_doc_ranges, ndocs);
	HIP_CHECK( hipEventRecord( c->evStart, stream));
	switch (plan.route)
	{
		case L2_ROUTE_RERUN_LIST: launchRerun( c, generalParams( c, io, plan), plan, *rerun, stream); break;
		case L2_ROUTE_JOIN: launchJoin( c, io, plan, nlexems, stream); break;
		case L2_ROUTE_FLAT_LIST: launchFlat( c, generalParams( c, io, plan), plan, stream); break;
		case L2_ROUTE_GENERAL: HIP_CHECK( launchL2Match( generalParams( c, io, plan), plan.generalBlocks, stream)); break;
	}
	HIP_CHECK( hipEventRecord( c->evStop, stream));
	c->evValid = true; c->lastStream = stream; c->lastNdocs = ndocs; c->haveBatch = true;
}

void deviceBatch( const sp_matcher_ctx* c, size_t ndocs, sp_match_device_batch_t* out)
{
	out->ndocs = ndocs;
	out->d_results = c->io.results.ptr(); out->d_items = c->io.items.ptr();
	out->d_doc_result_offsets = c->io.dDocRange.ptr;
	out->d_doc_stats = c->io.dDocStats.ptr; out->d_doc_status = c->io.dDocStatus.ptr;
	out->d_counters = c->io.dCounters.ptr;
	out->d_result_format = c->io.withFormats ? c->io.dResultFormat.ptr : 0;
	out->d_item_format = c->io.withFormats ? c->io.dItemFormat.ptr : 0;
}

int matchDevice( sp_matcher_ctx* c, const void* d_lexems, const void* d_origseg, const void* d_doc_offsets, const void* d_doc_ranges,
		 size_t ndocs, size_t nlexems, void* stream, sp_match_device_batch_t* out)
{
	return guardedCall( c->lasterror, SP_ERR_INVALID, [&]{
		launchBatch( c, d_lexems, d_origseg, d_doc_offsets, ndocs, nlexems, (hipStream_t)stream, d_doc_ranges);
		if (out) deviceBatch( c, ndocs, out);
	});
}

}

extern "C" {

int sp_matcher_ctx_match_docs_device( sp_matcher_ctx_t* c, const void* d_lexems, const void* d_origseg, const void* d_doc_offsets,
				      size_t ndocs, size_t nlexems, void* stream, sp_match_device_batch_t* out)
{ return matchDevice( c, d_lexems, d_origseg, d_doc_offsets, 0, ndocs, nlexems, stream, out); }

int sp_matcher_ctx_match_lexed_device( sp_matcher_ctx_t* c, const void* d_lexems, const void* d_doc_ranges,
				       size_t ndocs, size_t nlexems_hint, void* stream, sp_match_device_batch_t* out)
{ return matchDevice( c, d_lexems, 0, 0, d_doc_ranges, ndocs, nlexems_hint, stream, out); }

int sp_matcher_ctx_batch_counters( sp_matcher_ctx_t* c, uint64_t counters[8])
{
	return guardedCall( c->lasterror, SP_ERR_DEVICE, [&]{
		HIP_CHECK( hipSetDevice( c->device));
		HIP_CHECK( hipStreamSynchronize( c->lastStream));
		copySync( c->own, counters, c->io.dCounters.ptr, SPC_COUNT*sizeof(uint64_t), hipMemcpyDeviceToHost);
		if (c->flat.on && c->sw.verbose)
		{
			uint32_t diag[ 16];
			copySync( c->own, diag, (const uint32_t*)c->io.dCursor.ptr + 16, sizeof(diag), hipMemcpyDeviceToHost);
#ifdef SPA_PROF
			uint64_t prof[ 12];
			copySync( c->own, prof, (const uint32_t*)c->io.dCursor.ptr + 32, sizeof(prof), hipMemcpyDeviceToHost);
			double tot = 0; for (int i=0; i<6; ++i) tot += (double)prof[ i];
			fprintf( stderr, "[spa] fast tier phases (share of wave cycles): scan+fire %.1f%% install %.1f%% deactivate %.1f%% expiry %.1f%% results %.1f%% fetch %.1f%% | inside deactivation: loads %.1f%% ranks+queue %.1f%% replay %.1f%% (%.2f replay steps, %.2f batches, %.2f rules per event); %.0f cycles per event\n",
				100*prof[0]/tot, 100*prof[1]/tot, 100*prof[2]/tot, 100*prof[3]/tot, 100*prof[4]/tot, 100*prof[5]/tot, 100*prof[6]/tot, 100*prof[7]/tot, 100*prof[11]/tot,
				(double)prof[ 8] / (double)(counters[ SPC_EVENTS] ? counters[ SPC_EVENTS] : 1), (double)prof[ 9] / (double)(counters[ SPC_EVENTS] ? counters[ SPC_EVENTS] : 1), (double)prof[ 10] / (double)(counters[ SPC_EVENTS] ? counters[ SPC_EVENTS] : 1),
				tot / (double)(counters[ SPC_EVENTS] ? counters[ SPC_EVENTS] : 1));
#endif
			if (diag[ 0])
			{
				fprintf( stderr, "[spa] fast tier handed %u of %zu documents to the general kernel; by reason:", diag[ 0], c->lastNdocs);
				for (int i=1; i<16; ++i) if (diag[ i]) fprintf( stderr, " [%d]=%u", i, diag[ i]);
				fprintf( stderr, "\n");
			}
		}
	});
}

double sp_matcher_ctx_last_kernel_ms( sp_matcher_ctx_t* c) { return lastKernelMs( c); }

int sp_matcher_ctx_match_docs( sp_matcher_ctx_t* c, const sp_lexem_t* lexems, const uint32_t* origseg,
			       const uint64_t* doc_offsets, size_t ndocs, sp_match_batch_t* out)
{
	std::memset( out, 0, sizeof(*out));
	const int rc = guardedCall( c->lasterror, SP_ERR_DEVICE, [&]{
		if (ndocs >= 0xFFFFFFFFull) throw std::runtime_error( "too many documents in one batch");
		HIP_CHECK( hipSetDevice( c->device));
		size_t nlex = ndocs ? (size_t)doc_offsets[ ndocs] : 0;
		c->io.dLexems.reserve( (nlex+1)*sizeof(sp_lexem_t));
		c->io.dDocOffsets.reserve( (ndocs+1)*sizeof(uint64_t));
		if (nlex) copySync( c->own, c->io.dLexems.ptr, lexems, nlex*sizeof(sp_lexem_t), hipMemcpyHostToDevice);
		copySync( c->own, c->io.dDocOffsets.ptr, doc_offsets, (ndocs+1)*sizeof(uint64_t), hipMemcpyHostToDevice);
		const void* dseg = 0;
		if (origseg)
		{
			c->io.dOrigseg.reserve( (nlex+1)*sizeof(uint32_t));
			if (nlex) copySync( c->own, c->io.dOrigseg.ptr, origseg, nlex*sizeof(uint32_t), hipMemcpyHostToDevice);
			dseg = c->io.dOrigseg.ptr;
		}
		BatchCounts counts;
		uint64_t* counters = counts.counters;
		std::vector<uint32_t> again;
		std::vector<int32_t> st( ndocs+1);
		for (int attempt=0;; ++attempt)
		{
			launchBatch( c, c->io.dLexems.ptr, dseg, c->io.dDocOffsets.ptr, ndocs, nlex, c->own, 0, again.empty() ? 0 : &again);
			HIP_CHECK( hipStreamSynchronize( c->own));
			counts = readCounts( c);
			if (ndocs) copySync( c->own, st.data(), c->io.dDocStatus.ptr, ndocs*sizeof(int32_t), hipMemcpyDeviceToHost);
			bool grow = false;
			again.clear();
			if (counters[ SPC_RESULTS] > c->io.results.count) { c->io.minResults = counters[ SPC_RESULTS] + counters[ SPC_RESULTS]/8 + 1024; grow = true; }
			if (counters[ SPC_ITEMS] > c->io.items.count) { c->io.minItems = counters[ SPC_ITEMS] + counters[ SPC_ITEMS]/8 + 1024; grow = true; }
			if (counters[ SPC_FAILED])
			{
				std::vector<uint32_t> arenaDocs;
				for (size_t di=0; di<ndocs; ++di) if (st[ di] == SPD_ERR_ARENA) arenaDocs.push_back( (uint32_t)di);
				if (!arenaDocs.empty() && sp_matcher_ctx_grow_arena( c) == SP_OK)
				{
					if (!grow) again.swap( arenaDocs);
					grow = true;
				}
			}
			if (!grow || attempt >= 12) break;
		}
		{
			uint64_t failed = 0;
			for (size_t di=0; di<ndocs; ++di) if (st[ di] != 0) ++failed;
			if (failed != counters[ SPC_FAILED])
			{
				counters[ SPC_FAILED] = failed;
				copySync( c->own, (uint64_t*)c->io.dCounters.ptr + SPC_FAILED, &failed, sizeof(failed), hipMemcpyHostToDevice);
			}
		}
		copyOutBatch( c, 0, ndocs, counts, out);
		if (counters[ SPC_FAILED])
		{
			size_t bad = 0;
			while (bad < ndocs && out->doc_status[ bad] == 0) ++bad;
			char msg[ 128];
			snprintf( msg, sizeof(msg), "at least one document failed: document %zu has status %d (see doc_status)", bad, bad < ndocs ? out->doc_status[ bad] : -1);
			throw DocumentFailed( msg);
		}
	});
	return (rc == SP_OK || rc == SP_ERR_MATCH) ? rc : SP_ERR_DEVICE;
}

void sp_match_batch_free( sp_match_batch_t* b)
{
	std::free( b->results); std::free( b->items); std::free( b->doc_result_offsets);
	std::free( b->doc_stats); std::free( b->doc_status); std::free( b->result_format); std::free( b->item_format);
	std::memset( b, 0, sizeof(*b));
}

int sp_matcher_ctx_put_input( sp_matcher_ctx_t* c, const sp_lexem_t* lexems, const uint32_t* origseg, size_t n)
{
	return guardedCall( c->lasterror, SP_ERR_INVALID, [&]{
		uint32_t cur = c->cur.lexems.empty() ? 0 : c->cur.lexems.back().ordpos;
		for (size_t i=0; i<n; ++i)
		{
			if (lexems[i].ordpos < cur) throw std::runtime_error( "term events not fed in ascending order");
			cur = lexems[i].ordpos;
		}
		if (origseg && !c->cur.hasSeg) { c->cur.origseg.assign( c->cur.lexems.size(), 0); c->cur.hasSeg = true; }
		c->cur.lexems.insert( c->cur.lexems.end(), lexems, lexems+n);
		if (c->cur.hasSeg)
		{
			if (origseg) c->cur.origseg.insert( c->cur.origseg.end(), origseg, origseg+n);
			else c->cur.origseg.insert( c->cur.origseg.end(), n, 0u);
		}
	});
}

int sp_matcher_ctx_fetch_results( sp_matcher_ctx_t* c, sp_result_t** results, size_t* nresults,
				  sp_result_item_t** items, size_t* nitems)
{
	uint64_t offs[2] = {0, (uint64_t)c->cur.lexems.size()};
	sp_match_batch_t b;
	sp_lexem_t dummy = {0,0,0,0};
	int rc = sp_matcher_ctx_match_docs( c, c->cur.lexems.empty() ? &dummy : c->cur.lexems.data(),
					c->cur.hasSeg ? c->cur.origseg.data() : 0, offs, 1, &b);
	if (rc != SP_OK && rc != SP_ERR_MATCH) { sp_match_batch_free( &b); return rc; }
	if (rc == SP_ERR_MATCH)
	{
		static const char* msg[] = {"ok", "term events not fed in ascending order", "working set of the document exceeds the arena",
			"pattern with too many identical key events defined", "internal: encountered past trigger with follow",
			"term event out of range", "illegal free of event data reference"};
		int st = b.doc_status ? b.doc_status[0] : 0;
		c->lasterror = std::string("failed to feed input to pattern matcher: ") + ((st >= 0 && st <= 6) ? msg[ st] : "unknown");
		sp_match_batch_free( &b);
		return SP_ERR_MATCH;
	}
	c->cur.stats.nofProgramsInstalled = (double)b.doc_stats[0];
	c->cur.stats.nofAltKeyProgramsInstalled = (double)b.doc_stats[1];
	c->cur.stats.nofSignalsFired = (double)b.doc_stats[2];
	c->cur.stats.nofTriggersAvgActive = c->cur.lexems.empty() ? 0.0 : (double)b.doc_stats[3] / (double)c->cur.lexems.size();
	c->cur.resultFormat.clear(); c->cur.itemFormat.clear();
	if (b.result_format) c->cur.resultFormat.assign( b.result_format, b.result_format + b.nresults);
	if (b.item_format) c->cur.itemFormat.assign( b.item_format, b.item_format + 2*b.nitems);
	*results = b.results; *nresults = b.nresults; b.results = 0;
	if (items) { *items = b.items; b.items = 0; }
	if (nitems) *nitems = b.nitems;
	sp_match_batch_free( &b);
	return SP_OK;
}

int sp_matcher_ctx_fetch_formats( sp_matcher_ctx_t* c, const uint32_t** result_format, const uint32_t** item_format)
{
	*result_format = c->io.withFormats ? c->cur.resultFormat.data() : 0;
	*item_format = c->io.withFormats ? c->cur.itemFormat.data() : 0;
	return SP_OK;
}

int sp_matcher_ctx_statistics( sp_matcher_ctx_t* c, sp_matcher_stats_t* out)
{
	if (c->join.on)
	{
		std::memset( out, 0, sizeof(*out));
		c->lasterror = "no statistics in result-set mode (nothing is installed)";
		return SP_ERR_UNAVAILABLE;
	}
	*out = c->cur.stats;
	return SP_OK;
}

int sp_matcher_ctx_reset( sp_matcher_ctx_t* c)
{
	c->cur.lexems.clear(); c->cur.origseg.clear(); c->cur.hasSeg = false;
	c->cur.resultFormat.clear(); c->cur.itemFormat.clear();
	c->cur.stats = sp_matcher_stats_t();
	return SP_OK;
}
// ... 3 lines not shown
```

### struspattern_amd/csrc/capi_l2_ctx.hpp

```cpp
#ifndef SPA_CAPI_L2_CTX_HPP
#define SPA_CAPI_L2_CTX_HPP
#include "l2_plan.hpp"
#include "result_values.hpp"
#include "capi_util.hpp"
#include <mutex>

using namespace spa;

struct sp_matcher
{
	RuleCompiler compiler;
	bool compiled = false;
	mutable std::string lasterror;
	mutable std::mutex formatMutex;
	mutable FormatTable formatTable;
	mutable bool haveFormatTable = false;
	mutable size_t formatTableVariables = 0;

	const FormatTable& formats( bool rebuild = false) const
	{
		std::lock_guard<std::mutex> lock( formatMutex);
		const size_t nvariables = compiler.variables().names().size();
		if (rebuild || !haveFormatTable || formatTable.count != compiler.formatCount() || formatTableVariables != nvariables)
		{
			formatTableVariables = nvariables;
			formatTable = buildFormatTable( compiler.formatCount(),
				[this]( uint32_t f) { return compiler.formatString( f); },
				[this]( const std::string& name) { return compiler.variables().get( name); });
			haveFormatTable = true;
		}
		return formatTable;
	}
};

struct sp_matcher_ctx
{
	const sp_matcher* inst = 0;
	int device = 0;
	unsigned numCUs = 256;
	L2Switches sw;
	L2EngineKind kind = L2_GENERAL;
	std::string lasterror;
	struct Exact
	{
		DeviceBuffer dPrograms, dTrigdefs, dKeytab, dKeylist, dDocList;
		uint32_t keymask = 0, nofStopWords = 0;
		ArenaLayout layout = initialArena();
		CountedBuffer arena;
	} exact;
	struct Flat
	{
		bool on = false;
		std::string whyNot;
		DeviceBuffer dKeyinst, dStatics;
		FlatPlan plan;
		CountedBuffer spill;
		unsigned blocksPerCU = 0;
	} flat;
	struct ResultSets
	{
		bool on = false, altRules = false;
		std::string whyNot;
		uint32_t keymask = 0, maxRange = 0, delimiter = 0;
		DeviceBuffer dKeytab, dRules, dFilter, dCounts;
	} join;
	struct BatchIO
	{
		DeviceBuffer dCursor, dCounters;
		DeviceBuffer dLexems, dOrigseg, dDocOffsets;
		CountedBuffer results, items;
		DeviceBuffer dDocRange, dDocStats, dDocStatus;
		DeviceBuffer dResultFormat, dItemFormat;
		bool withFormats = false, withItems = true;
		uint64_t minResults = 0, minItems = 0;
	} io;
	struct Finished
	{
		PassRun<5> run;
		DeviceBuffer dResults, dItems, dResultFormat, dItemFormat, dDocResultOffsets, dDocItemOffsets, dTotals, dKept, dCovered, dCursor;
		bool canonical = false;
		DeviceBuffer dSortKeys[ 2], dSortIdx[ 2], dSortCursor;
	};
	struct ByteFamilies
	{
		PassRun<2> run;
		DeviceBuffer dBytes[ 2], dOffsets[ 2], dWork[ 2], dDocBytes[ 2], dDocOffsets[ 2];
		DeviceBuffer dStatus, dTotals, dCursor;
		uint32_t flags = 0;
		size_t ndocs = 0;
		uint64_t nrecords[ 2] = {0, 0}, totals[ 2] = {0, 0};
	};
	struct Values :public ByteFamilies
	{
		DeviceBuffer dFmtParts, dParts, dPool;
		bool uploaded = false;
		uint32_t poolBytes = 0;
	};
	struct Freq
	{
		PassRun<2> run;
		DeviceBuffer dRecords, dDocOffsets, dStatus, dHandleResults, dHandleDocs, dTotals, dDocCount, dDocMeta, dCursor;
		size_t ndocs = 0;
		uint32_t handleBound = 0;
		uint64_t total = 0;
	};
	struct Terms
	{
		PassRun<2> run;
		DeviceBuffer dRecords, dDocOffsets, dResultTerm, dStatus, dTotals, dLeader, dTable, dHistogram, dDocCount, dCursor;
		size_t ndocs = 0;
		uint32_t handleBound = 0, flags = 0;
		uint64_t nresults = 0, total = 0;
	};
	struct Dict
	{
		PassRun<2> run;
		DeviceBuffer dRecords, dTermDict, dDocOffsets, dHandleTerms, dTotals, dTable, dSlot, dLeader, dDocCount, dCursor;
		size_t ndocs = 0;
		uint32_t handleBound = 0, flags = 0;
		uint64_t nterms = 0, total = 0;
	};
	struct Products
	{
		Finished fin;
		ByteFamilies txt;
		Values val;
		Freq frq;
		Terms trm;
		Dict dct;
		void drop() { fin.run.done = false; txt.run.done = false; val.run.done = false; frq.run.done = false; trm.run.done = false; dct.run.done = false; }
	} prod;
	struct SingleDoc
	{
		std::vector<sp_lexem_t> lexems;
		std::vector<uint32_t> origseg; bool hasSeg = false;
		std::vector<uint32_t> resultFormat, itemFormat;
		sp_matcher_stats_t stats = {};
	} cur;
	bool haveBatch = false;
	size_t lastNdocs = 0;
	hipStream_t lastStream = 0;
	Event evStart, evStop; bool evValid = false;
	Stream own;
};

namespace spa {

struct BatchCounts { uint64_t counters[ SPC_COUNT]; uint64_t results, items; };
inline BatchCounts readCounts( sp_matcher_ctx* c)
{
	BatchCounts b;
	copySync( c->own, b.counters, c->io.dCounters.ptr, sizeof(b.counters), hipMemcpyDeviceToHost);
	b.results = clampCount( b.counters[ SPC_RESULTS], c->io.results.count);
	b.items = clampCount( b.counters[ SPC_ITEMS], c->io.items.count);
	return b;
}

inline void reserveOrNoMem( DeviceBuffer& buf, size_t n)
{
	try { buf.reserve( n); }
	catch (const HipError&) { (void)hipGetLastError(); throw std::bad_alloc(); }
}

inline void requireFinished( const sp_matcher_ctx* c)
{
	if (!c->prod.fin.run.done) throw std::runtime_error( "the last batch of this context has not been finished (sp_matcher_ctx_batch_finish_device)");
}

struct ProductCall
{
	sp_matcher_ctx* c;
	PassRun<2>& run;
	hipStream_t stream;
	size_t ndocs;
	uint64_t finished[ 2];

	ProductCall( sp_matcher_ctx* c_, PassRun<2>& run_, void* stream_)
		:c(c_),run(run_),stream((hipStream_t)stream_),ndocs(c_->lastNdocs)
	{
		requireFinished( c);
		HIP_CHECK( hipSetDevice( c->device));
		run.done = run.evValid = false;
		HIP_CHECK( hipStreamSynchronize( c->prod.fin.run.stream));
		copySync( c->own, finished, c->prod.fin.dTotals.ptr, sizeof(finished), hipMemcpyDeviceToHost);
	}
	void begin( DeviceBuffer& dStatus, DeviceBuffer& dTotals, size_t ntotals, DeviceBuffer& dCursor, size_t ncursor)
	{
		reserveOrNoMem( dStatus, (ndocs+1)*sizeof(int32_t));
		reserveOrNoMem( dTotals, ntotals*sizeof(uint64_t));
		reserveOrNoMem( dCursor, ncursor*sizeof(uint32_t));
		run.begin( stream, c->prod.fin.run.stream, c->prod.fin.run.ev[ 3]);
		HIP_CHECK( hipMemsetAsync( dCursor.ptr, 0, ncursor*sizeof(uint32_t), stream));
		HIP_CHECK( hipMemsetAsync( dTotals.ptr, 0, ntotals*sizeof(uint64_t), stream));
		HIP_CHECK( hipMemsetAsync( dStatus.ptr, 0, (ndocs+1)*sizeof(int32_t), stream));
	}
	template <class PARAMS, class SIZED>
	void passes( PARAMS& P, hipError_t (*count)( const PARAMS&, unsigned, hipStream_t), hipError_t (*place)( const PARAMS&, unsigned, hipStream_t),
		     const DeviceBuffer& dTotals, uint64_t* totals, size_t n, SIZED sized)
	{
		HIP_CHECK( hipEventRecord( run.ev[ 0], stream));
		HIP_CHECK( count( P, c->numCUs, stream));
		HIP_CHECK( hipStreamSynchronize( stream));
		copySync( c->own, totals, dTotals.ptr, n*sizeof(uint64_t), hipMemcpyDeviceToHost);
		sized();
		HIP_CHECK( place( P, c->numCUs, stream));
		HIP_CHECK( hipEventRecord( run.ev[ 1], stream));
		run.completed( stream);
	}
};

}
#endif
```

### struspattern_amd/csrc/l2_device.h

```cpp
#ifndef SPA_L2_DEVICE_H
#define SPA_L2_DEVICE_H
#include <stdint.h>
#include <hip/hip_runtime_api.h>
#include "l2_tables.h"
#if defined(__HIPCC__)
#include "wave_scan.h"
#endif

namespace spa {

enum {SPD_OK=0, SPD_ERR_ORDER=1, SPD_ERR_ARENA=2, SPD_ERR_KEYTRIGGERS=3, SPD_ERR_PASTFOLLOW=4, SPD_ERR_RANGE=5, SPD_ERR_DATAREF=6, SPD_ERR_LEXEMSIZE=7, SPD_ERR_INTERNAL=8, SPD_ERR_OUTPUT=9};
enum {SPC_RESULTS=0, SPC_ITEMS=1, SPC_EVENTS=2, SPC_FAILED=3, SPC_HANDOVER=4 , SPC_COUNT=8};

struct ArenaLayout
{
	uint32_t maxRules, maxTrigs, bucketCap, maxItems, maxRefs, maxFollow, maxDispose, maxHeap, maxGStack, maxStaged, nStop, winCap, scratchCap, winChunk, winChunks;
	uint32_t oRules, oTrigs, oBEvent, oBIdx, oBSize, oWindow, oHeap, oFollow, oDispose, oStop, oItems, oRefs, oGStack, oStaged, oRuleFree, oTrigFree, oItemFree, oRefFree, oWinArr, oScratch, oWinChunk, oWinFree;
	uint32_t totalWords;
};

struct L2BatchIO
{
	const uint32_t* lexems;
	const uint32_t* origseg;
	const uint64_t* docOffsets;
	const uint64_t* docRangesIn;
	uint32_t* docCursor;
	uint64_t* counters;
	uint32_t* results;
	uint64_t resultCapacity;
	uint32_t* items;
	uint64_t itemCapacity;
	uint64_t* docRange;
	uint64_t* docStats;
	int32_t* docStatus;
	uint32_t* resultFormat;
	uint32_t* itemFormat;
	uint32_t ndocs;
	uint32_t withItems;
	uint32_t withFormats;
};

struct L2Params
{
	const DevProgram* programs;
	const DevTrigDef* trigdefs;
	const DevKeyEntry* keytab;
	const DevKeyRef* keylist;
	uint32_t keymask;
	uint32_t nofStopWords;
	L2BatchIO io;
	uint32_t* arenaBase;
	ArenaLayout arena;
	const uint32_t* docList;
	const uint32_t* docListCount;
};

hipError_t launchL2Match( const L2Params& P, unsigned nblocks, hipStream_t stream);

#if defined(__HIPCC__)

template <class IO>
__device__ __forceinline__ void docLexems( const IO& io, u32 doc, u64& lbeg, u64& lend)
{
	if (io.docRangesIn)
	{
		const u32* rp = (const u32*)&io.docRangesIn[ 2*(u64)doc];
		lbeg = ((u64)ldu( rp+1) << 32) | ldu( rp);
		lend = lbeg + (((u64)ldu( rp+3) << 32) | ldu( rp+2));
	}
	else
	{
		lbeg = ((u64)ldu( (const u32*)&io.docOffsets[ doc]+1) << 32) | ldu( (const u32*)&io.docOffsets[ doc]);
		lend = ((u64)ldu( (const u32*)&io.docOffsets[ doc+1]+1) << 32) | ldu( (const u32*)&io.docOffsets[ doc+1]);
	}
}

template <class IO>
__device__ __forceinline__ bool reserveOutput( const IO& io, u32 c, u64 n, u64& base)
{
	u64 b = 0;
	if (LANE == 0) b = atomicAdd( (unsigned long long*)&io.counters[ c], (unsigned long long)n);
	base = ((u64)uni( (u32)(b >> 32)) << 32) | uni( (u32)b);
	return base + n <= (c == SPC_RESULTS ? io.resultCapacity : io.itemCapacity);
}

template <class IO>
__device__ __forceinline__ void finishDocument( const IO& io, u32 doc, u64 resBase, u64 nres, u64 st0, u64 st1, u64 st2, u64 st3, u32 err, u64 events)
{
	if (LANE == 0)
	{
		io.docRange[ 2*(u64)doc] = resBase; io.docRange[ 2*(u64)doc+1] = nres;
		u64* st = io.docStats + 4*(u64)doc;
		st[0] = st0; st[1] = st1; st[2] = st2; st[3] = st3;
		io.docStatus[ doc] = (int32_t)err;
		atomicAdd( (unsigned long long*)&io.counters[ SPC_EVENTS], (unsigned long long)events);
		if (err) atomicAdd( (unsigned long long*)&io.counters[ SPC_FAILED], 1ull);
	}
}
#endif

}
#endif
```

### struspattern_amd/csrc/l2_fast.h

```cpp
#ifndef SPA_L2_FAST_H
#define SPA_L2_FAST_H
#include <stdint.h>
#include <string>
#include <vector>
#include "l2_tables.h"
#include "l2_device.h"

namespace spa {

struct FastKeyInst
{
	uint32_t resultHandle;
	uint32_t formatHandle;
	uint32_t pastEvent;
	uint32_t meta;
	struct { uint32_t event; uint32_t info; } trig[ 3];
	uint32_t hw0;
	uint32_t ranksA;
	uint32_t ranksB;
	uint32_t totals;
	uint32_t items;
	uint32_t flags;
};
enum {
	FKI_VALUE_MASK=0xFu, FKI_COUNT_SHIFT=4, FKI_COUNT_MASK=0x1Fu, FKI_RANGE_SHIFT=9, FKI_RANGE_MASK=0x3Fu,
	FKI_NTRIG_SHIFT=15, FKI_NTRIG_MASK=0x3u, FKI_PASTSTOP_SHIFT=17, FKI_PASTSTOP_MASK=0xFFu,
	FTI_SIGVAL_MASK=0xFu, FTI_SIGTYPE_SHIFT=4, FTI_SIGTYPE_MASK=0x7u, FTI_INSTALL=1u<<7, FTI_KEY=1u<<8,
	FTI_BUCKET_SHIFT=9, FTI_HASVAR=1u<<13, FTI_DELSTOP_SHIFT=14, FTI_DELSTOP_MASK=0xFFu, FTI_VAR_SHIFT=24,
	FKF_BATCH_STATIC=1u,
	FKF_END_SET=2u,
	FKF_START_SET=4u,
	FKF_RESULT_NOW=8u,
	FKF_DISPOSE_NOW=16u
};
struct FastStatic
{
	uint32_t ev0, info0;
	uint32_t ev1, info1;
	uint32_t hw0;
	uint32_t misc;
	uint32_t ranks;
	uint32_t totals;
};
enum {
	FSI_BUCKET_SHIFT=16, FSI_RANK_SHIFT=20, FSI_LAST=1u<<28, FSI_PRESENT=1u<<29, FSI_SLOT_SHIFT=30,
	FSM_RANGE_MASK=0x3Fu, FSM_EXPRANK_SHIFT=6, FSM_EXPCLOSE_SHIFT=14,
	FSM_END_SET=1u<<22, FSM_START_SET=1u<<23, FSM_RESULT_NOW=1u<<24, FSM_DISPOSE_NOW=1u<<25, FSM_BATCH_COMPACT=1u<<26
};

enum {
	H_VALUE_MASK=0xFu, H_COUNT_SHIFT=4, H_COUNT_MASK=0x1Fu, H_END_SHIFT=9, H_END_MASK=0xFFu, H_ENDZERO=1u<<17,
	H_DONE=1u<<18, H_ACTIVE=1u<<19, H_TMASK_SHIFT=20, H_TMASK_MASK=0x7u, H_NITEMS_SHIFT=23, H_NITEMS_MASK=0x3u, H_HASSTART=1u<<25,
	H_COLD=1u<<26,
	H_LISTED=1u<<27,
	H_VISIBLE=1u<<28,
	H_MARK=1u<<31
};

enum {S_HASSTART=1u, S_DONE=2u, S_FIN=4u, S_DEL=8u, S_ODD=16u, S_RESULT=32u, S_HASLIST=64u, S_TOOK=128u};
struct Sim
{
	uint32_t value, count, end, startLex, nItems, it0, it1, it2, nFires, flags;
};
SPA_HD static inline void fireLocal( Sim& s, uint32_t info, uint32_t esord, uint32_t elex, uint32_t withItems)
{
	const uint32_t sigtype = (info >> FTI_SIGTYPE_SHIFT) & FTI_SIGTYPE_MASK, sigval = info & FTI_SIGVAL_MASK;
	uint32_t m = 0, f = 0, took = 0;
	s.nFires += 1;
	if (sigtype == SIG_ANY)
	{
		took = 1;
		if (s.count > 0) { m = 1; s.count -= 1; f = (s.count == 0); if (s.end < esord+1) s.end = esord+1; }
	}
	else if (sigtype == SIG_SEQUENCE || sigtype == SIG_SEQUENCE_IMM)
	{
		if (sigval == s.value && (sigtype == SIG_SEQUENCE ? (s.end <= esord) : (s.end == esord)))
		{
			s.end = esord+1; s.value = sigval-1;
			if (s.count > 0) { s.count -= 1; m = (s.count == 0); } else m = 1;
			f = (s.value == 0); took = 1;
		}
	}
	else if (sigtype == SIG_WITHIN)
	{
		if ((sigval & s.value) != 0 && s.end <= esord)
		{
			s.end = esord+1; s.value &= ~sigval;
			if (s.count > 0) { s.count -= 1; m = (s.count == 0); } else m = 1;
			took = 1;
		}
	}
	else
	{
		s.count = 0; s.value = 0; s.flags |= S_DEL;
		return;
	}
	if (took)
	{
		if ((info & FTI_HASVAR) && withItems)
		{
			const uint32_t item = elex | ((info >> FTI_VAR_SHIFT) << 24);
			if ((s.flags & S_DONE) && !(s.flags & S_HASLIST)) {}
			else if (s.nItems == 0) { s.it0 = item; s.nItems = 1; }
			else if (s.nItems == 1) { s.it1 = item; s.nItems = 2; }
			else if (s.nItems == 2) { s.it2 = item; s.nItems = 3; }
			else s.flags |= S_ODD;
		}
		if (!(s.flags & S_HASSTART)) { s.startLex = elex; s.flags |= S_TOOK; if (esord) s.flags |= S_HASSTART; }
	}
	if (m)
	{
		if (!(s.flags & S_DONE)) { s.flags |= S_DONE | S_RESULT; if (s.nItems) s.flags |= S_HASLIST; }
		if (f) s.flags |= S_FIN;
	}
}

struct FastKeyEntry
{
	uint32_t event;
	uint32_t kiBegin;
	uint32_t kiCount;
	uint32_t stopIdx;
};

enum {FAST_LISTCAP=64, FAST_EXPCAP=1024, FAST_MAXSTOP=64, FAST_SPILL_BUCKET=1024, FAST_VARIANTS=5, FAST_RQCAP=192};

struct FastSpillLayout
{
	uint32_t maxRules;
	uint32_t oCold;
	uint32_t oHot, oLink;
	uint32_t oKi, oLex0;
	uint32_t oFree;
	uint32_t oEnt;
	uint32_t oStaged;
	uint32_t maxStaged;
	uint32_t oList;
	uint32_t oExp;
	uint32_t totalWords;
};

enum {SPD_FAST_FALLBACK=100};

struct FastParams
{
	const FastKeyInst* keyinst;
	const FastStatic* statics;
	const FastKeyEntry* keytab;
	uint32_t keymask;
	uint32_t nofStopWords;
	uint32_t expShift;
	uint32_t bucketMeta[ 16];
	FastSpillLayout spill;
	uint32_t* spillBase;
	uint32_t* fallbackList; uint32_t* fallbackCount;
	uint32_t* diag;
	L2BatchIO io;
	uint64_t* prof;
};

hipError_t launchL2Fast( const FastParams& P, unsigned variant, unsigned nblocks, hipStream_t stream);
int fastBlocksPerCU( unsigned variant);
void fastCapacities( unsigned variant, uint32_t& R, uint32_t& T);
unsigned fastVariantNamed( const char* size);
const char* fastKernelName( unsigned variant);

struct FlatTables;
std::string buildFastTables( const FlatTables& ft, std::vector<FastKeyInst>& out, std::vector<FastStatic>* statics);
void layoutFast( FastSpillLayout& S, uint32_t bucketMeta[16], uint32_t& expShift, const std::vector<FastKeyInst>& keyinst, uint32_t R, uint32_t T, uint32_t maxRules, uint32_t maxStaged);

}
#endif
```

### struspattern_amd/csrc/l2_fast_kernel.hip

```cpp
#include <hip/hip_runtime.h>
#include <stdint.h>
#include "l2_fast.h"
#include "l2_device.h"
#include "wave_scan.h"

using namespace spa;

namespace {

typedef uint16_t u16;
typedef uint8_t u8;

typedef const __attribute__((address_space(4))) FastParams& KP;
__device__ __forceinline__ KP kernelParams() { return *(const __attribute__((address_space(4))) FastParams*)__builtin_amdgcn_kernarg_segment_ptr(); }

#define WAVE_FENCE() __builtin_amdgcn_fence( __ATOMIC_ACQ_REL, "wavefront")

enum {NIL16=0xFFFFu};

#ifdef SPA_PROF
#define PROF_DECL u64 prof_t0 = __builtin_amdgcn_s_memtime()
#define PROF_ADD( SLOT) do { const u64 prof_t1 = __builtin_amdgcn_s_memtime(); w.prof[ SLOT] += prof_t1 - prof_t0; prof_t0 = prof_t1; } while (0)
#else
#define PROF_DECL do {} while (0)
#define PROF_ADD( SLOT) do {} while (0)
#endif

__device__ __forceinline__ u64 lanesBelow() { return (1ull << LANE) - 1ull; }
__device__ __forceinline__ u32 evhash( u32 a)
{
	a += ~(a>>5);
	a +=  (a<<3);
	a ^=  (a>>4);
	return a;
}
__device__ __forceinline__ void st4( void* p, u32 a, u32 b, u32 c, u32 d) { u32x4 v; v.x = a; v.y = b; v.z = c; v.w = d; *(u32x4*)p = v; }
__device__ __forceinline__ uint4 ldu4( const void* p)
{
	uint4 v = ld4( p);
	v.x = uni( v.x); v.y = uni( v.y); v.z = uni( v.z); v.w = uni( v.w);
	return v;
}
__device__ __forceinline__ u32 waveScanOr( u32 v)
{
	v |= (u32)__builtin_amdgcn_update_dpp( 0, (int)v, 0x111, 0xF, 0xF, true);
	v |= (u32)__builtin_amdgcn_update_dpp( 0, (int)v, 0x112, 0xF, 0xF, true);
	v |= (u32)__builtin_amdgcn_update_dpp( 0, (int)v, 0x114, 0xF, 0xF, true);
	v |= (u32)__builtin_amdgcn_update_dpp( 0, (int)v, 0x118, 0xF, 0xF, true);
	v |= (u32)__builtin_amdgcn_update_dpp( 0, (int)v, 0x142, 0xA, 0xF, false);
	v |= (u32)__builtin_amdgcn_update_dpp( 0, (int)v, 0x143, 0xC, 0xF, false);
	return v;
}
__device__ __forceinline__ u32 fromLaneBelow( u32 v)
{
	const u32 t = (u32)__builtin_amdgcn_ds_bpermute( (int)((LANE - 1u) << 2), (int)v);
	return LANE ? t : 0u;
}
__device__ __forceinline__ u32 byteField( u32 c0, u32 c1, u32 c2, u32 c3, u32 h)
{
	const u32 wsel = h >> 2;
	const u32 v = wsel == 0 ? c0 : wsel == 1 ? c1 : wsel == 2 ? c2 : c3;
	return (v >> ((h & 3u)*8)) & 0xFFu;
}
__device__ __forceinline__ void byteInc( u32& c0, u32& c1, u32& c2, u32& c3, u32 h)
{
	const u32 inc = 1u << ((h & 3u)*8), ws = h >> 2;
	c0 += ws == 0 ? inc : 0u; c1 += ws == 1 ? inc : 0u; c2 += ws == 2 ? inc : 0u; c3 += ws == 3 ? inc : 0u;
}

#define FALLBACK( WHY) do { w.err = SPD_FAST_FALLBACK; w.why = (WHY); } while (0)
enum {FB_LEXEMS=1, FB_DISPOSE=2, FB_ITEM_AFTER_RESULT=3, FB_ITEMS=4, FB_STAGED=5, FB_RULES=8, FB_BUCKET_SIZE=9, FB_POSLEXEMS=10};

__device__ __forceinline__ bool endLE( u32 hw, u32 pos) { return (hw & H_ENDZERO) || ((hw >> H_END_SHIFT) & H_END_MASK) != ((pos + 1u) & 0xFFu); }
__device__ __forceinline__ bool endEQ( u32 hw, u32 pos) { return (hw & H_ENDZERO) ? (pos == 0) : (((hw >> H_END_SHIFT) & H_END_MASK) == (pos & 0xFFu)); }
__device__ __forceinline__ u32 withEnd( u32 hw, u32 end) { return (hw & ~((H_END_MASK << H_END_SHIFT) | H_ENDZERO)) | ((end & 0xFFu) << H_END_SHIFT); }

template <bool SMALL> struct FreeId { typedef u8 type; };
template <> struct FreeId<false> { typedef u16 type; };
template <int R, int T>
struct LdsDoc
{
	u32 hot[ R];
	u32 kl[ R];
	u64 ent[ T];
	u32 bsize[ 16];
	u32 bmeta[ 16];
	u16 link[ 3*R];
	typename FreeId<(R <= 256)>::type freeS[ R];
	u16 exp[ FAST_EXPCAP];
	u16 expCnt[ 64];
	u16 list[ FAST_LISTCAP];
	u16 rq[ FAST_RQCAP];
};

struct Wave
{
	u32* sp;
	u32 curpos, timestamp, nInstalled, nAlt, nSignals, nTrig, openLo, openHi;
	u32 freeN, usedL, sFreeN, usedS;
	u32 nDispose, nStaged, nStagedItems, err;
	u32 lbase;
	u32 spill;
	u32 why;
	u32 posLexems;
	u32 stopLex, stopOrd, stopTs;
	u32 bsizeV, bmetaV;
	u32 expCntV;
#ifdef SPA_PROF
	u64 prof[ 12];
#endif
};

template <int R, int T>
struct Engine
{
typedef LdsDoc<R,T> Lds;
typedef __attribute__((address_space(3))) Lds& LR;

template <bool SP> static __device__ __forceinline__ u32 ldHot( LR L, const Wave& w, KP P, u32 r) { if (!SP || r < (u32)R) return L.hot[ r]; return w.sp[ P.spill.oHot + (r - R)]; }
template <bool SP> static __device__ __forceinline__ void stHot( LR L, const Wave& w, KP P, u32 r, u32 v) { if (!SP || r < (u32)R) L.hot[ r] = v; else w.sp[ P.spill.oHot + (r - R)] = v; }
template <bool SP> static __device__ __forceinline__ u32 ldLink( LR L, const Wave& w, KP P, u32 r, u32 j) { if (!SP || r < (u32)R) return (u32)L.link[ 3*r + j]; return w.sp[ P.spill.oLink + 3*(r - R) + j]; }
template <bool SP> static __device__ __forceinline__ void stLink( LR L, const Wave& w, KP P, u32 r, u32 j, u32 v) { if (!SP || r < (u32)R) L.link[ 3*r + j] = (u16)v; else w.sp[ P.spill.oLink + 3*(r - R) + j] = v; }
template <bool SP> static __device__ __forceinline__ void ldLinks( LR L, const Wave& w, KP P, u32 r, u32& l0, u32& l1, u32& l2)
{
	if (!SP || r < (u32)R) { l0 = (u32)L.link[ 3*r]; l1 = (u32)L.link[ 3*r+1]; l2 = (u32)L.link[ 3*r+2]; }
	else { const u32* q = &w.sp[ P.spill.oLink + 3*(r - R)]; l0 = q[0]; l1 = q[1]; l2 = q[2]; }
}
template <bool SP> static __device__ __forceinline__ u32 ldKl( LR L, const Wave& w, KP P, u32 r) { if (!SP || r < (u32)R) return L.kl[ r]; return w.sp[ P.spill.oKi + (r - R)]; }
template <bool SP> static __device__ __forceinline__ void stKl( LR L, const Wave& w, KP P, u32 r, u32 ki, u32 lx)
{ const u32 v = ki | (lx << 20); if (!SP || r < (u32)R) L.kl[ r] = v; else w.sp[ P.spill.oKi + (r - R)] = v; }
static __device__ __forceinline__ u32 keyLexemOf( u32 kl, u32 lbase) { return lbase - ((lbase - (kl >> 20)) & 0xFFFu); }
template <bool SP> static __device__ __forceinline__ u32 ldExp( LR L, const Wave& w, KP P, u32 row, u32 i)
{ const u32 C = (u32)FAST_EXPCAP >> P.expShift; if (!SP || i < C) return (u32)L.exp[ row*C + i]; return w.sp[ P.spill.oExp + row*P.spill.maxRules + (i - C)]; }
template <bool SP> static __device__ __forceinline__ void stExp( LR L, const Wave& w, KP P, u32 row, u32 i, u32 r)
{ const u32 C = (u32)FAST_EXPCAP >> P.expShift; if (!SP || i < C) L.exp[ row*C + i] = (u16)r; else w.sp[ P.spill.oExp + row*P.spill.maxRules + (i - C)] = r; }
template <bool SP> static __device__ __forceinline__ u32 ldEv( LR L, const Wave& w, KP P, u32 h, u32 meta, u32 pos)
{ if (!SP || pos < (meta >> 16)) return (u32)L.ent[ (meta & 0xFFFFu) + pos]; return w.sp[ P.spill.oEnt + 2*(h*FAST_SPILL_BUCKET + pos - (meta >> 16))]; }
template <bool SP> static __device__ __forceinline__ uint2 ldEnt( LR L, const Wave& w, KP P, u32 h, u32 meta, u32 pos)
{ if (!SP || pos < (meta >> 16)) { const u64 v = L.ent[ (meta & 0xFFFFu) + pos]; return make_uint2( (u32)v, (u32)(v >> 32)); } return *(const uint2*)&w.sp[ P.spill.oEnt + 2*(h*FAST_SPILL_BUCKET + pos - (meta >> 16))]; }
template <bool SP> static __device__ __forceinline__ u32 ldTs( LR L, const Wave& w, KP P, u32 h, u32 meta, u32 pos) { return ldEnt<SP>( L, w, P, h, meta, pos).y; }
template <bool SP> static __device__ __forceinline__ void stEnt( LR L, const Wave& w, KP P, u32 h, u32 meta, u32 pos, u32 e, u32 t)
{
	if (!SP || pos < (meta >> 16)) L.ent[ (meta & 0xFFFFu) + pos] = (u64)e | ((u64)t << 32);
	else *(uint2*)&w.sp[ P.spill.oEnt + 2*(h*FAST_SPILL_BUCKET + pos - (meta >> 16))] = make_uint2( e, t);
}
template <bool SP> static __device__ __forceinline__ u32 ldList( LR L, const Wave& w, KP P, u32 i) { if (!SP || i < (u32)FAST_LISTCAP) return (u32)L.list[ i]; return w.sp[ P.spill.oList + i]; }
static __device__ __forceinline__ void pushList( LR L, Wave& w, KP P, u32 i, u32 r)
{
	if (i < (u32)FAST_LISTCAP) { if (LANE == 0) L.list[ i] = (u16)r; }
	else { w.spill = 1; if (LANE == 0) w.sp[ P.spill.oList + i] = r; }
}

enum {STAGED_LINE=0x80000000u};
static __device__ __forceinline__ void stageLineResult( Wave& w, KP P, u32 at, u32 ki, u32 startLex, u32 endLex, u32 nStatic, u32 hasNew, u32 newVar, u32 keyLex)
{
	u32* S = &w.sp[ P.spill.oStaged + 8*at];
	st4( S, (u32)STAGED_LINE | ki, 0u, startLex, endLex);
// ... 787 lines not shown
				{
					if (info[ t] & FSI_PRESENT) { hB[ t] = (info[ t] >> FSI_BUCKET_SHIFT) & 15u; inst[ t] = true; oldB[ t] = L.bsize[ hB[ t]]; metaB[ t] = L.bmeta[ hB[ t]]; }
				}
			}
			w.nInstalled += nb;
			u32 r;
			if (!allocRuleIds( L, w, P, __ballot( have), r)) return;
			if (!w.spill)
			{
				if (__ballot( have && cnt + nb > ((u32)FAST_EXPCAP >> P.expShift))) w.spill = 1;
			}
			if (!checkBuckets( L, w, P, uni( c1.w) & 0xFFu, inst, hB)) return;
			PROF_I( 7, cnt + oldB[ 0] + oldB[ 1] + r);
			if (w.spill) installCompactT<true>( L, w, P, kb + base, nb, sord, r, c0, c1, row, cnt, oldB, metaB);
			else installCompactT<false>( L, w, P, kb + base, nb, sord, r, c0, c1, row, cnt, oldB, metaB);
			PROF_I( 11, 0u);
			w.bsizeV = L.bsize[ LANE & 15u];
			continue;
		}
		uint4 q0 = make_uint4( 0,0,0,0), q1 = q0, q2 = q0, q3 = q0;
		if (have)
		{
			const FastKeyInst* K = &P.keyinst[ kb + base + LANE];
			q0 = ld4( K); q1 = ld4( (const u32*)K + 4); q2 = ld4( (const u32*)K + 8); q3 = ld4( (const u32*)K + 12);
		}
		const bool isStatic = (uni( q3.w) & FKF_BATCH_STATIC) != 0 && sord != 0;
		const u32 pastEvent = q0.z, meta = q0.w;
		const u32 tEv[ 3] = {q1.x, q1.z, q2.x};
		const u32 tInfo[ 3] = {q1.y, q1.w, q2.y};
		const u32 range = (meta >> FKI_RANGE_SHIFT) & FKI_RANGE_MASK;
		Sim sim;
		sim.value = meta & FKI_VALUE_MASK; sim.count = (meta >> FKI_COUNT_SHIFT) & FKI_COUNT_MASK; sim.end = 0;
		sim.startLex = 0; sim.nItems = 0; sim.it0 = 0; sim.it1 = 0; sim.it2 = 0; sim.nFires = 0; sim.flags = 0;
		bool dropped = false;
		if (!isStatic && __ballot( have && pastEvent != 0))
		{
			const u32 psi = (have && pastEvent) ? ((meta >> FKI_PASTSTOP_SHIFT) & FKI_PASTSTOP_MASK) : 0u;
			const u32 plex = (u32)__builtin_amdgcn_ds_bpermute( (int)((psi-1u) << 2), (int)w.stopLex);
			const u32 psord = (u32)__builtin_amdgcn_ds_bpermute( (int)((psi-1u) << 2), (int)w.stopOrd);
			const u32 pts = (u32)__builtin_amdgcn_ds_bpermute( (int)((psi-1u) << 2), (int)w.stopTs);
			u32 delTs[ 3];
#pragma unroll
			for (int j=0; j<3; ++j)
			{
				const u32 esi = (tInfo[ j] >> FTI_DELSTOP_SHIFT) & FTI_DELSTOP_MASK;
				delTs[ j] = (u32)__builtin_amdgcn_ds_bpermute( (int)((esi-1u) << 2), (int)w.stopTs);
				if (!esi) delTs[ j] = 0;
			}
			if (psi)
			{
				if (pts && psord + range >= w.curpos)
				{
#pragma unroll
					for (int j=2; j>=0; --j)
					{
						if ((tInfo[ j] & FTI_INSTALL) && tEv[ j] == pastEvent) fireLocal( sim, tInfo[ j], psord, plex, P.io.withItems);
					}
					if (sim.flags & S_DONE) sim.flags |= S_ODD;
					bool cancelled = false;
#pragma unroll
					for (int j=0; j<3; ++j)
					{
						if ((tInfo[ j] & FTI_INSTALL) && ((tInfo[ j] >> FTI_SIGTYPE_SHIFT) & FTI_SIGTYPE_MASK) == SIG_DEL)
						{
							const u32 ts = delTs[ j];
							if (ts && ts > pts) cancelled = true;
						}
					}
					if (cancelled || (sim.flags & (S_DEL | S_FIN))) dropped = true;
				}
			}
			w.nAlt += (u32)__popcll( __ballot( have && pastEvent != 0));
		}
		if (!isStatic)
		{
			if (have && !dropped)
			{
#pragma unroll
				for (int j=0; j<3; ++j) if (tInfo[ j] & FTI_KEY) fireLocal( sim, tInfo[ j], sord, w.lbase, P.io.withItems);
			}
			if (__ballot( (sim.flags & S_ODD) != 0)) { FALLBACK( FB_ITEMS); return; }
		}
		const bool mat = have && !dropped;
		const u64 matMask = __ballot( mat);
		const u32 nmat = (u32)__popcll( matMask);
		w.nInstalled += nb;
		if (isStatic) w.nSignals += (uni( q3.y) >> 8) & 0xFFu;
		else
		{
			u32 incl = waveScanAdd( have ? sim.nFires : 0u);
			w.nSignals += (u32)__builtin_amdgcn_readlane( incl, 63);
		}
		u32 r;
		if (!allocRuleIds( L, w, P, matMask, r)) return;
		if (nmat && !w.spill)
		{
			const u32 row = (sord + range) & ((1u << P.expShift) - 1u);
			const bool over = mat && (u32)L.expCnt[ row] + nmat > ((u32)FAST_EXPCAP >> P.expShift);
			if (__ballot( over)) w.spill = 1;
		}
		{
			bool inst[ 3]; u32 hB[ 3];
#pragma unroll
			for (int j=0; j<3; ++j) { inst[ j] = mat && (tInfo[ j] & FTI_INSTALL); hB[ j] = (tInfo[ j] >> FTI_BUCKET_SHIFT) & 15u; }
			if (!checkBuckets( L, w, P, isStatic ? (uni( q3.y) & 0xFFu) : 3*nmat, inst, hB)) return;
		}
		if (isStatic)
		{
			if (w.spill) installStaticT<true>( L, w, P, kb + base, nb, sord, r, q0, q1, q2, q3);
			else installStaticT<false>( L, w, P, kb + base, nb, sord, r, q0, q1, q2, q3);
		}
		else if (w.spill) installBatchT<true>( L, w, P, kb, nb, sord, matMask, r, q0, q1, q2, sim);
		else installBatchT<false>( L, w, P, kb, nb, sord, matMask, r, q0, q1, q2, sim);
		w.bsizeV = L.bsize[ LANE & 15u];
	}
	w.bsizeV = L.bsize[ LANE & 15u];
	w.expCntV = (u32)L.expCnt[ LANE];
}

template <bool SP>
static __device__ __forceinline__ void scanAndFire( LR L, Wave& w, KP P, u32 id, u32 ordpos)
{
	const u32 h = evhash( id) & 15u;
	const u32 n = (u32)__builtin_amdgcn_readlane( w.bsizeV, h);
	const u32 meta = (u32)__builtin_amdgcn_readlane( w.bmetaV, h);
	for (u32 base=0; base<n && !w.err; base+=64)
	{
		const u32 i = base + LANE;
		uint2 en = make_uint2( 0, 0);
		if (i < n) en = ldEnt<SP>( L, w, P, h, meta, i);
		u64 m = __ballot( i < n && en.x == id);
		if (!SP && (m & (m - 1ull)) != 0)
		{
			if (fireBatch( L, w, P, m, en.y, ordpos)) m = 0;
		}
		while (m && !w.err)
		{
			const u32 p = (u32)__builtin_ctzll( m);
			m &= m-1;
			const u32 tsv = (u32)__builtin_amdgcn_readlane( en.y, p);
			fireSignal<SP>( L, w, P, tsv, ordpos);
		}
	}
}

static __device__ __forceinline__ void runKernel()
{
	KP P = kernelParams();
	__shared__ Lds ldsDoc;
	LR L = *(__attribute__((address_space(3))) Lds*)&ldsDoc;
	Wave w;
	w.sp = P.spillBase + (u64)blockIdx.x * P.spill.totalWords;
	const u32 ndocs = P.io.ndocs;
	const u32 waveSlot = blockIdx.x, nWaveSlots = gridDim.x;

	for (u32 round=0; round<=ndocs; ++round)
	{
		u32 doc = waveSlot;
		if (round)
		{
			u32 nx = 0;
			if (LANE == 0) nx = atomicAdd( P.io.docCursor, 1u);
			doc = nWaveSlots + uni( nx);
		}
		if (doc >= ndocs) break;
		w.bmetaV = P.bucketMeta[ LANE & 15u]; w.bsizeV = 0; w.expCntV = 0;
		if (LANE < 16u) { L.bsize[ LANE] = 0; L.bmeta[ LANE] = w.bmetaV; }
		L.expCnt[ LANE] = 0;
		w.stopLex = 0; w.stopOrd = 0; w.stopTs = 0; w.posLexems = 0;
		w.curpos = 0; w.timestamp = 0; w.nInstalled = 0; w.nAlt = 0; w.nSignals = 0; w.nTrig = 0; w.openLo = 0; w.openHi = 0;
		w.freeN = 0; w.usedL = 0; w.sFreeN = 0; w.usedS = 0;
		w.nDispose = 0; w.nStaged = 0; w.nStagedItems = 0; w.err = 0; w.lbase = 0; w.why = 0; w.spill = 0;
#ifdef SPA_PROF
		for (int pi=0; pi<12; ++pi) w.prof[ pi] = 0;
#endif
		WAVE_FENCE();

		u64 lbeg, lend;
		docLexems( P.io, doc, lbeg, lend);
		if (lend - lbeg >= (1ull << 24)) FALLBACK( FB_LEXEMS);
		u32 curPosition = 0, nEvents = 0;
		for (u64 tile=lbeg; tile<lend && !w.err; tile+=64)
		{
			PROF_DECL;
			uint4 lx = make_uint4( 0,0,0,0); u32 seg = 0;
			const bool mine = tile + LANE < lend;
			if (mine)
			{
				lx = ((const uint4*)P.io.lexems)[ tile + LANE];
				if (P.io.origseg) seg = P.io.origseg[ tile + LANE];
			}
			u32 kBegin = 0, kCount = 0, kStop = 0;
			if (mine && lx.x && lx.x < (1u<<29))
			{
				u32 slot = keyHash( lx.x) & P.keymask;
				for (u32 probes=0; probes<=P.keymask; ++probes)
				{
					const uint4 eq = ld4( &P.keytab[ slot]);
					if (eq.x == lx.x) { kBegin = eq.y; kCount = eq.z; kStop = eq.w; break; }
					if (eq.x == 0) break;
					slot = (slot+1) & P.keymask;
				}
			}
			const u32 cnt = (lend - tile) < 64 ? (u32)(lend - tile) : 64u;
#ifdef SPA_PROF
			if (__ballot( kBegin == 0xFFFFFFFFu)) break;
#endif
			PROF_ADD( 5);
			for (u32 k=0; k<cnt && !w.err; ++k)
			{
				const u32 id = __builtin_amdgcn_readlane( lx.x, k), ordpos = __builtin_amdgcn_readlane( lx.y, k);
				const u32 origpos = __builtin_amdgcn_readlane( lx.z, k), origsize = __builtin_amdgcn_readlane( lx.w, k);
				const u32 origseg = __builtin_amdgcn_readlane( seg, k);
				if (curPosition > ordpos) { w.err = SPD_ERR_ORDER; break; }
				else if (curPosition < ordpos) { curPosition = ordpos; w.posLexems = 0; }
				else if (origsize >= 0x7FFFFFFFu || origseg >= 0x7FFFFFFFu || origpos >= 0x7FFFFFFFu) { w.err = SPD_ERR_RANGE; break; }
				if (w.curpos != ordpos || w.nDispose) { setCurrentPos( L, w, P, ordpos); PROF_ADD( 3); if (w.err) break; }
				if (id >= (1u<<29)) { w.err = SPD_ERR_RANGE; break; }
				w.lbase = (u32)(tile - lbeg) + k;
				if (++w.posLexems > 60u) { FALLBACK( FB_POSLEXEMS); break; }
				{
					const u32 lo = w.openLo + w.nTrig;
					if (lo < w.openLo) w.openHi += 1;
					w.openLo = lo;
				}
				const u32 kb = __builtin_amdgcn_readlane( kBegin, k), kc = __builtin_amdgcn_readlane( kCount, k);
				const u32 stopIdx = __builtin_amdgcn_readlane( kStop, k);
				uint4 pc0 = make_uint4( 0,0,0,0), pc1 = pc0;
				if (LANE < kc) { const u32* S = (const u32*)&P.statics[ kb + LANE]; pc0 = ld4( S); pc1 = ld4( S+4); }
				if (id)
				{
					if (w.spill) scanAndFire<true>( L, w, P, id, ordpos); else scanAndFire<false>( L, w, P, id, ordpos);
				}
				PROF_ADD( 0);
				if (w.err) break;
				if (kc) installBatch( L, w, P, kb, kc, ordpos, pc0, pc1);
				PROF_ADD( 1);
				if (w.err) break;
				WAVE_FENCE();
				if (stopIdx)
				{
					if (LANE == stopIdx-1u) { w.stopLex = w.lbase; w.stopOrd = ordpos; w.stopTs = w.timestamp + 1u; }
					w.timestamp += 1;
					WAVE_FENCE();
				}
				PROF_ADD( 2);
				++nEvents;
			}
		}

		PROF_DECL;
		u32 nres = w.err ? 0 : w.nStaged;
		const u32 nitems = (w.err || !P.io.withItems) ? 0 : w.nStagedItems;
		u64 resBase = 0, itemBase = 0;
		if (nres && !reserveOutput( P.io, SPC_RESULTS, nres, resBase)) { w.err = SPD_ERR_OUTPUT; nres = 0; }
		if (nres && nitems && !reserveOutput( P.io, SPC_ITEMS, nitems, itemBase)) { w.err = SPD_ERR_OUTPUT; nres = 0; }
		if (nres)
		{
			WAVE_FENCE();
			u64 ip = itemBase;
			for (u32 base=0; base<nres; base+=64)
			{
				const u32 ri = base + LANE;
				const bool hv = ri < nres;
				uint4 s0 = make_uint4( 0,0,0,0), s1 = s0;
				if (hv) { const u32* S = &w.sp[ P.spill.oStaged + 8*ri]; s0 = ld4( S); s1 = ld4( S+4); }
				if (hv && (s0.x & (u32)STAGED_LINE))
				{
					const u32* K = (const u32*)&P.keyinst[ s0.x & 0xFFFFFu];
					const u32 handle = K[ 0], fmt = K[ 1], vw = K[ 14];
					const u32 nStatic = s1.x & 3u, hasNew = (s1.x >> 2) & 1u, newVar = (s1.x >> 8) & 0xFFu, lx = s1.y, endLex = s0.w;
					u32 vv[ 3] = {0,0,0}, ll[ 3] = {0,0,0};
					u32 n = 0;
					if (hasNew) { vv[ 0] = newVar; ll[ 0] = endLex; n = 1; }
#pragma unroll
					for (int k=2; k>=0; --k)
					{
						if ((u32)k < nStatic)
						{
							const u32 v = (vw >> (8*k)) & 0xFFu;
							if (n == 0) { vv[ 0] = v; ll[ 0] = lx; } else if (n == 1) { vv[ 1] = v; ll[ 1] = lx; } else if (n == 2) { vv[ 2] = v; ll[ 2] = lx; }
							++n;
						}
					}
					s0.x = handle; s0.y = fmt;
					s1.x = n | (vv[ 0] << 8) | (vv[ 1] << 16) | (vv[ 2] << 24); s1.y = ll[ 0]; s1.z = ll[ 1]; s1.w = ll[ 2];
				}
				const u32 ni = P.io.withItems ? (s1.x & 0xFFu) : 0u;
				u32 incl = waveScanAdd( ni);
				const u64 mine = ip + (incl - ni);
				if (hv)
				{
					const uint4 a = ((const uint4*)P.io.lexems)[ lbeg + s0.z], z = ((const uint4*)P.io.lexems)[ lbeg + s0.w];
					const u32 sa = P.io.origseg ? P.io.origseg[ lbeg + s0.z] : 0u, sz = P.io.origseg ? P.io.origseg[ lbeg + s0.w] : 0u;
					u32* o = P.io.results + (resBase + ri)*9;
					o[0] = s0.x; o[1] = a.y; o[2] = z.y + 1u; o[3] = sa; o[4] = a.z; o[5] = sz; o[6] = z.z + z.w;
					o[7] = P.io.withItems ? (u32)mine : 0u; o[8] = ni;
					if (P.io.withFormats) P.io.resultFormat[ resBase + ri] = s0.y;
					const u32 il[ 3] = {s1.y, s1.z, s1.w};
#pragma unroll
					for (int q=0; q<3; ++q)
					{
						if ((u32)q < ni)
						{
							const uint4 t = ((const uint4*)P.io.lexems)[ lbeg + il[ q]];
							const u32 st = P.io.origseg ? P.io.origseg[ lbeg + il[ q]] : 0u;
							u32* io = P.io.items + (mine + (u32)q)*7;
							io[0] = (s1.x >> (8 + 8*q)) & 0xFFu; io[1] = t.y; io[2] = t.y + 1u; io[3] = st; io[4] = t.z; io[5] = st; io[6] = t.z + t.w;
							if (P.io.withFormats) { P.io.itemFormat[ 2*(mine + (u32)q)] = 0; P.io.itemFormat[ 2*(mine + (u32)q)+1] = 0; }
						}
					}
				}
				ip += (u32)__builtin_amdgcn_readlane( incl, 63);
			}
		}
		PROF_ADD( 4);
#ifdef SPA_PROF
		if (LANE == 0 && P.prof) for (int pi=0; pi<12; ++pi) atomicAdd( (unsigned long long*)&P.prof[ pi], (unsigned long long)w.prof[ pi]);
#endif
		if (w.err != SPD_FAST_FALLBACK) finishDocument( P.io, doc, resBase, nres, w.nInstalled, w.nAlt, w.nSignals, ((u64)w.openHi << 32) | w.openLo, w.err, nEvents);
		else if (LANE == 0)
		{
			const u32 at = atomicAdd( P.fallbackCount, 1u);
			P.fallbackList[ at] = doc;
			P.io.docRange[ 2*(u64)doc] = 0; P.io.docRange[ 2*(u64)doc+1] = 0;
			P.io.docStatus[ doc] = (int32_t)SPD_FAST_FALLBACK;
			atomicAdd( (unsigned long long*)&P.io.counters[ SPC_HANDOVER], 1ull);
			if (P.diag) { atomicAdd( &P.diag[ 0], 1u); atomicAdd( &P.diag[ w.why & 15u], 1u); }
		}
	}
}
};

}

#ifndef SPA_L2_FAST_WAVES_PER_EU
#define SPA_L2_FAST_WAVES_PER_EU 4
#endif
#define SPA_L2_FAST_OCC __attribute__((amdgpu_waves_per_eu( SPA_L2_FAST_WAVES_PER_EU, SPA_L2_FAST_WAVES_PER_EU)))
#define SPA_FAST_VARIANTS( V) \
	V( s, 192, 312) \
	V( m, 320, 512) \
	V( l, 512, 1024) \
	V( t, 8, 128)		 \
	V( n, 256, 448)
#define SPA_FAST_INSTANCE( X, RR, TT) \
	extern "C" __global__ __launch_bounds__(64) SPA_L2_FAST_OCC void spa_l2_fast_kernel_##X( FastParams kernelArgs) { Engine<RR,TT>::runKernel(); }
SPA_FAST_VARIANTS( SPA_FAST_INSTANCE)

namespace spa {
struct FastVariant { void (*kernel)( FastParams); uint32_t R, T; const char* name; };
#define SPA_FAST_ENTRY( X, RR, TT) {spa_l2_fast_kernel_##X, RR, TT, "spa_l2_fast_kernel_" #X},
static const FastVariant fastVariants[ FAST_VARIANTS] = { SPA_FAST_VARIANTS( SPA_FAST_ENTRY) };
static const FastVariant& fastVariantOf( unsigned variant) { return fastVariants[ variant < FAST_VARIANTS ? variant : FAST_VARIANTS-1]; }

unsigned fastVariantNamed( const char* size)
{
	for (unsigned v=0; v<FAST_VARIANTS; ++v) if (size[ 0] == fastVariants[ v].name[ sizeof("spa_l2_fast_kernel_")-1]) return v;
	return FAST_VARIANTS-1;
}
const char* fastKernelName( unsigned variant) { return fastVariantOf( variant).name; }
void fastCapacities( unsigned variant, uint32_t& R, uint32_t& T) { R = fastVariantOf( variant).R; T = fastVariantOf( variant).T; }
int fastBlocksPerCU( unsigned variant)
{
	int n = 0;
	if (hipOccupancyMaxActiveBlocksPerMultiprocessor( &n, (const void*)fastVariantOf( variant).kernel, 64, 0) != hipSuccess || n < 1) n = 1;
	if (n > 32) n = 32;
	return n;
}
hipError_t launchL2Fast( const FastParams& P, unsigned variant, unsigned nblocks, hipStream_t stream)
{
	hipLaunchKernelGGL( fastVariantOf( variant).kernel, dim3( nblocks), dim3( 64), 0, stream, P);
	return hipGetLastError();
}
}
```

### struspattern_amd/csrc/l2_kernel.hip

```cpp
#include <hip/hip_runtime.h>
#include <stdint.h>
#include "l2_tables.h"
#include "l2_device.h"
#include "wave_scan.h"

using namespace spa;

namespace {

#ifndef SPA_L2_BATCH_MIN
#define SPA_L2_BATCH_MIN 1
#endif
#ifndef SPA_L2_DEACT_MIN
#define SPA_L2_DEACT_MIN 2
#endif
#ifndef SPA_L2_WAVES_PER_EU
#define SPA_L2_WAVES_PER_EU 3
#endif

#ifdef SPA_PROF
#define PROF_DECL u64 prof_t0 = __builtin_amdgcn_s_memtime()
#define PROF_ADD( SLOT) do { u64 prof_t1 = __builtin_amdgcn_s_memtime(); w.raw->prof[ SLOT] += prof_t1 - prof_t0; prof_t0 = prof_t1; } while (0)
#else
#define PROF_DECL do {} while (0)
#define PROF_ADD( SLOT) do {} while (0)
#endif
#ifdef SPA_PROF2
#define P2C( SLOT, N) do { w.raw->prof[ SLOT] += (N); } while (0)
#define P2_DECL u64 p2_t0 = __builtin_amdgcn_s_memtime()
#define P2_ADD( SLOT) do { u64 p2_t1 = __builtin_amdgcn_s_memtime(); w.raw->prof[ SLOT] += p2_t1 - p2_t0; p2_t0 = p2_t1; } while (0)
#else
#define P2C( SLOT, N) do {} while (0)
#define P2_DECL do {} while (0)
#define P2_ADD( SLOT) do {} while (0)
#endif
#ifdef SPA_PROF2
#define ARENA_FAIL do { w.err = SPD_ERR_ARENA; w.raw->prof[3] = __LINE__; } while (0)
#else
#define ARENA_FAIL w.err = SPD_ERR_ARENA
#endif

typedef const __attribute__((address_space(4))) L2Params& KP;
__device__ __forceinline__ KP kernelParams() { return *(const __attribute__((address_space(4))) L2Params*)__builtin_amdgcn_kernarg_segment_ptr(); }

enum {F_ACTIVE=1u, F_DONE=2u, F_EXT=4u};

struct EvData { u32 sseg, eseg, spos, epos, sord, eord, sub, fmt; };

struct Trig
{
	u32 event, sigval, typevar, link;
};
struct Rule
{
	u32 value, count, flags, start_ordpos;
	u32 end_ordpos, start_origseg, start_origpos, program;
	u32 trigMask, dataRef, ext, owner;
	u32 nInline, _pad[3];
	Trig trig[4];
};
struct Item { u32 variable, next, _a, _b; EvData d; };
struct Follow { EvData d; u32 event, _a, _b, _c; };
struct StopLog { EvData d; u32 timestamp, _a, _b, _c; };
struct StagedResult { u32 program, sord, eord, sseg, spos, eseg, epos, dataRef; };

#define LDSQ __attribute__((address_space(3)))
#define HOT
#define CAP_RULES	(P.arena.maxRules)
#define CAP_BUCKET	(P.arena.bucketCap)
#define CAP_FOLLOW	(P.arena.maxFollow)
#define CAP_DISPOSE	(P.arena.maxDispose)
#define CAP_HEAP	(P.arena.maxHeap)
#define WIN_CHUNK	(P.arena.winChunk)
#define WIN_NCHUNKS	(P.arena.winChunks)
#define CAP_SCRATCH	(P.arena.scratchCap)
#define CAP_ITEMS	(P.arena.maxItems)
#define CAP_REFS	(P.arena.maxRefs)
typedef HOT u32 hu32;
typedef HOT Rule HRule;
typedef Trig HTrig;
typedef Item HItem;
typedef HOT Follow HFollow;
typedef HOT EvData HEvData;

struct WS
{
	u32 curpos, timestamp, nInstalled, nAlt, nSignals, nTrig;
	u64 open;
	u32 ruleFreeN, ruleUsed, itemFreeN, itemUsed, refFreeN, refUsed;
	u32 heapSize, nFollow, nDispose, nStaged, err;
	u32 winFreeN, winUsed;
#if defined(SPA_PROF) || defined(SPA_PROF2)
	u64 prof[4];
#endif
};
typedef LDSQ WS HWS;
typedef LDSQ u32 lu32;
typedef LDSQ u64 lu64;
struct WSField
{
	lu32* p;
	__device__ __forceinline__ operator u32() const { return __builtin_amdgcn_readfirstlane( *p); }
	__device__ __forceinline__ u32 operator=( u32 v) const { *p = v; return v; }
	__device__ __forceinline__ u32 operator=( const WSField& o) const { u32 v = o; *p = v; return v; }
	__device__ __forceinline__ u32 operator+=( u32 v) const { u32 n = (u32)*this + v; *p = n; return n; }
	__device__ __forceinline__ u32 operator-=( u32 v) const { u32 n = (u32)*this - v; *p = n; return n; }
	__device__ __forceinline__ u32 operator++() const { return *this += 1u; }
	__device__ __forceinline__ u32 operator--() const { return *this -= 1u; }
	__device__ __forceinline__ u32 operator++( int) const { u32 o = *this; *p = o+1; return o; }
	__device__ __forceinline__ u32 operator--( int) const { u32 o = *this; *p = o-1; return o; }
};
struct WSField64
{
	lu64* p;
	__device__ __forceinline__ operator u64() const { u64 v = *p; return ((u64)__builtin_amdgcn_readfirstlane( (u32)(v >> 32)) << 32) | __builtin_amdgcn_readfirstlane( (u32)v); }
	__device__ __forceinline__ void operator=( u64 v) const { *p = v; }
	__device__ __forceinline__ void operator+=( u64 v) const { *p = (u64)*this + v; }
};
struct WSV
{
	HWS* raw;
	u32* arena;
	WSField curpos, timestamp, nInstalled, nAlt, nSignals, nTrig;
	WSField64 open;
	WSField ruleFreeN, ruleUsed, itemFreeN, itemUsed, refFreeN, refUsed;
	WSField heapSize, nFollow, nDispose, nStaged, err;
	WSField winFreeN, winUsed;
	__device__ __forceinline__ WSV( HWS* b, u32* a)
		:raw(b),arena(a),curpos{&b->curpos},timestamp{&b->timestamp},nInstalled{&b->nInstalled},nAlt{&b->nAlt},nSignals{&b->nSignals},nTrig{&b->nTrig}
		,open{&b->open},ruleFreeN{&b->ruleFreeN},ruleUsed{&b->ruleUsed}
		,itemFreeN{&b->itemFreeN},itemUsed{&b->itemUsed},refFreeN{&b->refFreeN},refUsed{&b->refUsed}
		,heapSize{&b->heapSize},nFollow{&b->nFollow},nDispose{&b->nDispose},nStaged{&b->nStaged},err{&b->err}
		,winFreeN{&b->winFreeN},winUsed{&b->winUsed} {}
};
typedef const WSV& WSR;

#define ARENA( OFS)	(w.arena + (OFS))
#define RULES		((Rule*)ARENA( P.arena.oRules))
#define TRIG( T)	(&RULES[ (T) >> 2].trig[ (T) & 3u])
#define BKT		ARENA( P.arena.oBEvent)
#define BSIZE		((lu32*)w.raw + 64)
#define WINDOW		((lu32*)w.raw + 80)
#define WINCHUNK	((lu32*)w.raw + 144)
#define SCRLDS		((lu32*)w.raw + 656)
#define EXPLIST		((lu32*)w.raw + 1168)
#define WINARR		ARENA( P.arena.oWinArr)
#define WINFREE		ARENA( P.arena.oWinFree)
#define SCRATCH		ARENA( P.arena.oScratch)
#define HEAP		ARENA( P.arena.oHeap)
#define FOLLOW		((Follow*)ARENA( P.arena.oFollow))
#define DISPOSE		ARENA( P.arena.oDispose)
#define RULEFREE	ARENA( P.arena.oRuleFree)
#define ITEMS		((Item*)ARENA( P.arena.oItems))
#define REFS		ARENA( P.arena.oRefs)
#define ITEMFREE	ARENA( P.arena.oItemFree)
#define REFFREE		ARENA( P.arena.oRefFree)
#define STOP		((StopLog*)ARENA( P.arena.oStop))
// ... 1300 lines not shown
			}
		}
		PROF_ADD( 0);
		uint4 eq = make_uint4( 0, 0, 0, 0);
		bool e = false;
		if (ev)
		{
			u32 slot = keyHash( ev) & P.keymask;
			for (u32 probes=0; probes<=P.keymask; ++probes)
			{
				eq = ldu4( &P.keytab[ slot]);
				if (eq.x == ev) { e = true; break; }
				if (eq.x == 0) break;
				slot = (slot+1) & P.keymask;
			}
		}
		u32 stopIdx = 0;
		if (e)
		{
			stopIdx = eq.w;
			u32 lb = eq.y, lc = eq.z;
			if (lc >= SPA_L2_BATCH_MIN && !(P.io.withItems && d.sub)) installBatch( w, P, ev, lb, lc, d);
			else for (u32 k=0; k<lc && !w.err; ++k) installProgram( w, P, ev, &P.keylist[ lb+k], d);
		}
		PROF_ADD( 1);
		if (w.nDispose >= SPA_L2_DEACT_MIN) deactivateBatch( w.raw, w.arena, P, DISPOSE, w.nDispose, false, false, true);
		else for (u32 di=0; di<w.nDispose; ++di) deactivateRule( w, P, ldu( &DISPOSE[ di]));
		PROF_ADD( 2);

		if (stopIdx)
		{
			StopLog* L = &STOP[ stopIdx-1];
			stEv( &L->d, d); L->timestamp = ++w.timestamp;
		}
		else if (d.sub && P.io.withItems)
		{
			disposeRef( w, P, d.sub);
		}
	}
}

__device__ __forceinline__ u32 walkItems( WSR w, KP P, u32 ref, u32* out)
{
	u32 n = 0, sp = 0;
	u32 cur = ldu( &REFS[ 2*(ref-1)]);
	for (u32 guard=0;; ++guard)
	{
		if (guard > (1u<<22)) { w.err = SPD_ERR_INTERNAL; break; }
		if (!cur)
		{
			if (!sp) break;
			cur = ldu( &GSTACK[ --sp]);
			continue;
		}
		const HItem* I = &ITEMS[ cur-1];
		EvData d; ldEv( d, &I->d);
		if (out)
		{
			u32* o = out + (u64)n*7;
			o[0] = ldu( &I->variable); o[1] = d.sord; o[2] = d.eord; o[3] = d.sseg; o[4] = d.spos; o[5] = d.eseg; o[6] = d.epos;
		}
		++n;
		cur = ldu( &I->next);
		if (d.sub && !d.fmt)
		{
			if (sp >= P.arena.maxGStack) { ARENA_FAIL; break; }
			GSTACK[ sp++] = cur;
			cur = ldu( &REFS[ 2*(d.sub-1)]);
		}
	}
	return n;
}

__device__ __forceinline__ u32 walkItemsFormatted( WSR w, KP P, u32 ref, u32* out, u32* fmtout)
{
	u32 n = 0, sp = 0;
	u32 cur = ldu( &REFS[ 2*(ref-1)]);
	for (u32 guard=0;; ++guard)
	{
		if (guard > (1u<<22)) { w.err = SPD_ERR_INTERNAL; break; }
		if (!cur)
		{
			if (!sp) break;
			sp -= 2;
			cur = ldu( &GSTACK[ sp]);
			const u32 owner = ldu( &GSTACK[ sp+1]);
			if (owner && out) fmtout[ 2*(u64)(owner-1)+1] = n - owner;
			continue;
		}
		const HItem* I = &ITEMS[ cur-1];
		EvData d; ldEv( d, &I->d);
		if (out)
		{
			u32* o = out + (u64)n*7;
			o[0] = ldu( &I->variable); o[1] = d.sord; o[2] = d.eord; o[3] = d.sseg; o[4] = d.spos; o[5] = d.eseg; o[6] = d.epos;
			fmtout[ 2*(u64)n] = d.fmt; fmtout[ 2*(u64)n+1] = 0;
		}
		++n;
		cur = ldu( &I->next);
		if (d.sub)
		{
			if (sp+2 > P.arena.maxGStack) { ARENA_FAIL; break; }
			GSTACK[ sp] = cur; GSTACK[ sp+1] = d.fmt ? n : 0u;
			sp += 2;
			cur = ldu( &REFS[ 2*(d.sub-1)]);
		}
	}
	return n;
}

__device__ __forceinline__ u32 walkItemsLane( WSR w, KP P, u32 ref, u32* out, bool& deep)
{
	u32 n = 0, sp = 0, s0 = 0, s1 = 0, s2 = 0, s3 = 0;
	u32 cur = REFS[ 2*(ref-1)];
	for (u32 guard=0;; ++guard)
	{
		if (guard > (1u<<22)) { deep = true; break; }
		if (!cur)
		{
			if (!sp) break;
			--sp;
			cur = sp == 0 ? s0 : sp == 1 ? s1 : sp == 2 ? s2 : s3;
			continue;
		}
		const Item* I = &ITEMS[ cur-1];
		const uint4 a = ld4( I), b = ld4( W( I) + 4), c = ld4( W( I) + 8);
		if (out)
		{
			u32* o = out + (u64)n*7;
			o[0] = a.x; o[1] = c.x; o[2] = c.y; o[3] = b.x; o[4] = b.z; o[5] = b.y; o[6] = b.w;
		}
		++n;
		cur = a.y;
		if (c.z && !c.w)
		{
			if (sp >= 4) { deep = true; break; }
			if (sp == 0) s0 = cur; else if (sp == 1) s1 = cur; else if (sp == 2) s2 = cur; else s3 = cur;
			++sp;
			cur = REFS[ 2*(c.z-1)];
		}
	}
	return n;
}

}

extern "C" __global__ __launch_bounds__(64) __attribute__((amdgpu_waves_per_eu(SPA_L2_WAVES_PER_EU, 8)))
void spa_l2_match_kernel( L2Params kernelArgs)
{
	KP P = kernelParams();
	__shared__ __attribute__((aligned(16))) u32 ldsSlice[ 64 + 16 + 64 + 512 + 16*SCRLDS_CAP + EXPLIST_CAP];
	const WSV w( (HWS*)ldsSlice, P.arenaBase + (u64)blockIdx.x * P.arena.totalWords);
	const u32 ndocs = P.docList ? ldu( P.docListCount) : P.io.ndocs;
	const u32 waveSlot = blockIdx.x;
	const u32 nWaveSlots = gridDim.x;

	for (u32 round=0; round<=ndocs; ++round)
	{
		u32 doc = waveSlot;
		if (round)
		{
			u32 nx = 0;
			if (LANE == 0) nx = atomicAdd( P.io.docCursor, 1u);
			doc = nWaveSlots + uni( nx);
		}
		if (doc >= ndocs) break;
		if (P.docList) doc = ldu( &P.docList[ doc]);
		if (LANE < 16) BSIZE[ LANE] = 0;
		WINDOW[ LANE] = 0;
		for (u32 s=LANE; s<P.nofStopWords; s+=64) STOP[ s].timestamp = 0;
		w.curpos = 0; w.timestamp = 0; w.nInstalled = 0; w.nAlt = 0; w.nSignals = 0; w.nTrig = 0; w.open = 0;
		w.ruleFreeN = 0; w.ruleUsed = 0; w.itemFreeN = 0; w.itemUsed = 0;
#if defined(SPA_PROF) || defined(SPA_PROF2)
		w.raw->prof[0] = w.raw->prof[1] = w.raw->prof[2] = w.raw->prof[3] = 0;
#endif
		w.winFreeN = 0; w.winUsed = 0;
		w.refFreeN = 0; w.refUsed = 0; w.heapSize = 0; w.nFollow = 0; w.nDispose = 0; w.nStaged = 0; w.err = 0;

		u64 lbeg, lend;
		docLexems( P.io, doc, lbeg, lend);
		u32 curPosition = 0, nEvents = 0;
		for (u64 lbase=lbeg; lbase<lend && !w.err; lbase+=64)
		{
			uint4 lx = make_uint4( 0,0,0,0); u32 seg = 0;
			if (lbase + LANE < lend)
			{
				lx = ((const uint4*)P.io.lexems)[ lbase + LANE];
				if (P.io.origseg) seg = P.io.origseg[ lbase + LANE];
			}
			u32 cnt = (lend - lbase) < 64 ? (u32)(lend - lbase) : 64u;
			for (u32 k=0; k<cnt && !w.err; ++k)
			{
				u32 id = __builtin_amdgcn_readlane( lx.x, k), ordpos = __builtin_amdgcn_readlane( lx.y, k);
				u32 origpos = __builtin_amdgcn_readlane( lx.z, k), origsize = __builtin_amdgcn_readlane( lx.w, k);
				u32 origseg = __builtin_amdgcn_readlane( seg, k);
				if (curPosition > ordpos) { w.err = SPD_ERR_ORDER; break; }
				else if (curPosition < ordpos) { curPosition = ordpos; PROF_DECL; setCurrentPos( w, P, ordpos); PROF_ADD( 3); }
				else if (origsize >= 0x7FFFFFFFu || origseg >= 0x7FFFFFFFu || origpos >= 0x7FFFFFFFu) { w.err = SPD_ERR_RANGE; break; }
				if (id >= (1u<<29)) { w.err = SPD_ERR_RANGE; break; }
				EvData d;
				d.sseg = origseg; d.eseg = origseg; d.spos = origpos; d.epos = origpos + origsize;
				d.sord = ordpos; d.eord = ordpos+1; d.sub = 0; d.fmt = 0;
				doTransition( w.raw, w.arena, P, id , d);
				++nEvents;
			}
		}

		u32 nres = w.err ? 0 : w.nStaged;
		u64 resBase = 0;
		if (nres)
		{
			u64 b = 0;
			if (LANE == 0) b = atomicAdd( (unsigned long long*)&P.io.counters[ SPC_RESULTS], (unsigned long long)nres);
			resBase = ((u64)uni( (u32)(b >> 32)) << 32) | uni( (u32)b);
			if (resBase + nres > P.io.resultCapacity) { w.err = SPD_ERR_OUTPUT; nres = 0; }
		}
		if (P.io.withItems && nres)
		{
			u32 total = 0;
			bool sequential = P.io.withFormats != 0;
			for (u32 base=0; base<nres && !sequential; base+=64)
			{
				const u32 ri = base + LANE;
				u32 n = 0; bool deep = false;
				if (ri < nres)
				{
					const u32 ref = STAGED[ ri].dataRef;
					if (ref) n = walkItemsLane( w, P, ref, 0, deep);
					P.io.results[ (resBase + ri)*9 + 8] = n;
				}
				if (__ballot( deep)) { sequential = true; break; }
				u32 incl = n;
				incl = waveScanAdd( incl);
				total += (u32)__builtin_amdgcn_readlane( incl, 63);
			}
			if (sequential)
			{
				total = 0;
				for (u32 ri=0; ri<nres && !w.err; ++ri)
				{
					u32 ref = ldu( &STAGED[ ri].dataRef);
					if (ref) total += P.io.withFormats ? walkItemsFormatted( w, P, ref, 0, 0) : walkItems( w, P, ref, 0);
				}
			}
			u64 itemBase = 0;
			if (w.err) nres = 0;
			else if (total && !reserveOutput( P.io, SPC_ITEMS, total, itemBase)) { w.err = SPD_ERR_OUTPUT; nres = 0; }
			if (nres && sequential)
			{
				u64 ip = itemBase;
				for (u32 ri=0; ri<nres; ++ri)
				{
					u32 ref = ldu( &STAGED[ ri].dataRef);
					u32 n = !ref ? 0u : P.io.withFormats ? walkItemsFormatted( w, P, ref, P.io.items + ip*7, P.io.itemFormat + ip*2) : walkItems( w, P, ref, P.io.items + ip*7);
					u32* o = P.io.results + (resBase + ri)*9;
					o[7] = (u32)ip; o[8] = n;
					ip += n;
				}
			}
			else if (nres)
			{
				u64 ip = itemBase;
				for (u32 base=0; base<nres; base+=64)
				{
					const u32 ri = base + LANE;
					u32 n = 0;
					if (ri < nres) n = P.io.results[ (resBase + ri)*9 + 8];
					u32 incl = n;
					incl = waveScanAdd( incl);
					if (ri < nres)
					{
						const u64 mine = ip + (incl - n);
						P.io.results[ (resBase + ri)*9 + 7] = (u32)mine;
						const u32 ref = STAGED[ ri].dataRef;
						bool deep = false;
						if (ref) (void)walkItemsLane( w, P, ref, P.io.items + mine*7, deep);
					}
					ip += (u32)__builtin_amdgcn_readlane( incl, 63);
				}
			}
		}
		if (nres)
		{
			for (u32 ri=LANE; ri<nres; ri+=64)
			{
				const StagedResult* S = &STAGED[ ri];
				u32* o = P.io.results + (resBase + ri)*9;
				const uint4 g0 = ld4( &P.programs[ S->program]);
				o[0] = g0.w; o[1] = S->sord; o[2] = S->eord; o[3] = S->sseg; o[4] = S->spos; o[5] = S->eseg; o[6] = S->epos;
				if (P.io.withFormats) P.io.resultFormat[ resBase + ri] = P.programs[ S->program].formatHandle;
				if (!P.io.withItems) { o[7] = 0; o[8] = 0; }
			}
		}
#ifdef SPA_PROF2
		finishDocument( P.io, doc, resBase, nres, w.refUsed, w.ruleUsed, w.nTrig, w.itemUsed, w.err, w.err ? 0 : nEvents);
#else
		finishDocument( P.io, doc, resBase, nres, w.nInstalled, w.nAlt, w.nSignals, w.open, w.err, w.err ? 0 : nEvents);
#endif
#if defined(SPA_PROF) || defined(SPA_PROF2)
		if (LANE == 0) for (int pi=0; pi<4; ++pi) atomicAdd( (unsigned long long*)&P.io.counters[ 4+pi], (unsigned long long)w.raw->prof[ pi]);
#endif
	}
}

namespace spa {
hipError_t launchL2Match( const L2Params& P, unsigned nblocks , hipStream_t stream)
{
	hipLaunchKernelGGL( spa_l2_match_kernel, dim3( nblocks), dim3( 64), 0, stream, P);
	return hipGetLastError();
}
}
```

### struspattern_amd/csrc/l2_plan.cpp

```cpp
#include "l2_plan.hpp"
#include "../../include/strus_pattern_amd.h"
#include <cstdlib>
#include <cstring>
#include <stdexcept>

namespace spa {

L2Switches L2Switches::fromEnv()
{
	L2Switches sw;
	if (const char* e = getenv( "SPA_L2_FAST")) sw.fast = e[ 0] != '0';
	if (const char* e = getenv( "SPA_L2_FAST_SIZE")) sw.fastSize = e[ 0];
	if (const char* e = getenv( "SPA_L2_FAST_MAXRULES")) sw.fastMaxRules = (uint32_t)atoi( e);
	if (const char* e = getenv( "SPA_L2_FAST_MAXSTAGED")) sw.fastMaxStaged = (uint32_t)atoi( e);
	if (const char* e = getenv( "SPA_L2_JOIN")) sw.join = e[ 0] == '1';
	sw.verbose = getenv( "SPA_L2_VERBOSE") != 0;
	return sw;
}

static uint32_t alignUp( uint32_t v, uint32_t a) { return (v + a-1) / a * a; }

ArenaLayout initialArena()
{
	ArenaLayout a;
	std::memset( &a, 0, sizeof(a));
	a.maxRules = 1024; a.maxTrigs = 1024; a.bucketCap = 256; a.maxItems = 2048;
	a.maxRefs = 1024; a.maxFollow = 256; a.maxDispose = 512; a.maxHeap = 256;
	a.maxGStack = 64; a.maxStaged = 1024; a.winCap = 128; a.scratchCap = 256;
	return a;
}

void layoutArena( ArenaLayout& L)
{
	uint32_t o = 0;
	L.oRules = o;	o += L.maxRules*32;
	L.oTrigs = 0; L.oBIdx = 0; L.oTrigFree = 0;
	L.oBEvent = o;	o += alignUp( 2*16*L.bucketCap, 32);
	L.oBSize = o;	o += 16;
	L.oWindow = o;	o += 64;
	L.oHeap = o;	o += alignUp( L.maxHeap*2, 4);
	L.oFollow = o;	o += alignUp( L.maxFollow*12, 4);
	L.oDispose = o;	o += alignUp( L.maxDispose, 4);
	L.oStop = o;	o += alignUp( (L.nStop?L.nStop:1)*12, 4);
	L.oItems = o;	o += alignUp( L.maxItems*12, 4);
	L.oRefs = o;	o += alignUp( L.maxRefs*2, 4);
	L.oGStack = o;	o += alignUp( L.maxGStack, 4);
	L.oStaged = o;	o += alignUp( L.maxStaged*8, 4);
	L.oRuleFree = o; o += alignUp( L.maxRules, 4);
	L.oItemFree = o; o += alignUp( L.maxItems, 4);
	L.oRefFree = o;	o += alignUp( L.maxRefs, 4);
	L.winChunk = L.winCap/8 < 16 ? 16 : L.winCap/8;
	L.winChunks = L.maxRules/L.winChunk + 64;
	L.oWinArr = o;	o += alignUp( L.winChunks*L.winChunk, 4);
	L.oWinChunk = o; o += 64*8;
	L.oWinFree = o;	o += alignUp( L.winChunks, 4);
	L.oScratch = o;	o += alignUp( 16*L.scratchCap, 4);
	L.totalWords = alignUp( o, 64);
}

void setArena( ArenaLayout& L, uint32_t maxRules, uint32_t maxTrigs, uint32_t bucketCap, uint32_t maxItems, uint32_t maxFollow)
{
	if (maxRules) { L.maxRules = maxRules; L.maxHeap = maxRules; L.maxDispose = maxRules; L.winCap = maxRules/4 < 64 ? 64 : maxRules/4; }
	if (maxTrigs) L.maxTrigs = maxTrigs;
	if (bucketCap) L.bucketCap = bucketCap;
	if (maxItems) { L.maxItems = maxItems; L.maxRefs = maxItems; }
	if (maxFollow) L.maxFollow = maxFollow;
}

bool growArena( ArenaLayout& L)
{
	if (L.maxRules >= (1u<<20)) return false;
	L.maxRules *= 2; L.maxTrigs *= 2; L.bucketCap *= 2; L.maxItems *= 2;
	L.maxRefs *= 2; L.maxFollow *= 2; L.maxDispose *= 2; L.maxHeap *= 2;
	L.maxStaged *= 2; L.maxGStack *= 2; L.winCap *= 2;
	if (L.scratchCap < 256) L.scratchCap = 256;
	return true;
}

ArenaWaves arenaWaves( size_t perWaveBytes, unsigned wanted, size_t fullSlots, unsigned multiple)
{
	const size_t fit = ((size_t)48 << 30) / perWaveBytes;
	const size_t maxRun = fit < 4 ? 4 : fit;
	const size_t full = fullSlots < fit ? fullSlots : fit;
	ArenaWaves w;
	w.run = wanted > maxRun ? (unsigned)(maxRun / multiple * multiple) : wanted;
	w.alloc = (w.run >= 64 && w.run < full) ? (unsigned)full : w.run;
	return w;
}

L2Engine chooseL2Engine( const RuleCompiler& compiler, const FlatTables& ft, uint32_t ctxFlags, const L2Switches& sw)
{
	L2Engine e;
	e.flat.whyNot = buildFastTables( ft, e.flat.keyinst, &e.flat.statics);
	if (!sw.fast) e.flat.whyNot = "disabled by SPA_L2_FAST=0";
	e.flat.on = e.flat.whyNot.empty();
	if (e.flat.on && e.flat.keyinst.empty()) e.flat.keyinst.resize( 1);
	e.flat.maxRules = sw.fastMaxRules > 4095 ? 4095 : sw.fastMaxRules;
	e.flat.maxStaged = sw.fastMaxStaged;
	e.join.asked = (ctxFlags & SP_CTX_RESULT_SETS) != 0 || sw.join;
	if (!e.join.asked) e.join.whyNot = "result sets not asked for";
	else if (compiler.exclusive()) e.join.whyNot = "the `exclusive` option (its outcome depends on the order of the results)";
	else e.join.whyNot = buildJoinTables( ft, e.join.keytab, e.join.rules, e.join.filter, e.join.maxRange, e.join.delimiter, e.altPrograms);
	e.join.on = e.join.whyNot.empty();
	if (!e.join.on) e.altPrograms = 0;
	return e;
}

FlatPlan planFlat( const L2Engine::Flat& flat, unsigned variant, const char* kernelName, uint32_t R, uint32_t T)
{
	FlatPlan p;
	p.variant = variant; p.kernelName = kernelName; p.R = R; p.T = T;
	layoutFast( p.spill, p.bucketMeta, p.expShift, flat.keyinst, R, T, flat.maxRules, flat.maxStaged);
	return p;
}

const char* l2KernelName( L2EngineKind kind, const FlatPlan* flat)
{
	return kind == L2_JOIN ? "spa_l2_join_kernel" : kind == L2_FLAT ? flat->kernelName : "spa_l2_match_kernel";
}

L2LaunchPlan planL2Launch( L2EngineKind kind, bool rerun, unsigned numCUs, unsigned fastBlocksPerCU, size_t docsToRun, size_t ndocs, size_t nlexems,
			   const ArenaLayout& arena, const FlatPlan* flat, uint64_t minResults, uint64_t minItems)
{
	if (ndocs >= 0xFFFFFFFFull) throw std::runtime_error( "too many documents in one batch");
	auto blocksFor = []( size_t docs, size_t slots) { return (unsigned)(docs < slots ? (docs ? docs : 1) : slots); };
	L2LaunchPlan p;
	p.route = rerun ? L2_ROUTE_RERUN_LIST : kind == L2_JOIN ? L2_ROUTE_JOIN : kind == L2_FLAT ? L2_ROUTE_FLAT_LIST : L2_ROUTE_GENERAL;
	p.kernelName = l2KernelName( kind, flat);
	const size_t waveSlots = (size_t)numCUs * L2_WAVES_PER_CU;
	p.layout = arena;
	layoutArena( p.layout);
	p.arenaPerWaveBytes = (size_t)p.layout.totalWords * sizeof(uint32_t);
	p.arena = arenaWaves( p.arenaPerWaveBytes, blocksFor( docsToRun, waveSlots), waveSlots, 1);
	p.generalBlocks = p.arena.run;
	p.arenaAllocWaves = rerun ? p.arena.run : p.arena.alloc;
	if (p.route == L2_ROUTE_FLAT_LIST)
	{
		const size_t fslots = (size_t)numCUs * fastBlocksPerCU;
		p.fastBlocks = blocksFor( ndocs, fslots);
		p.spillAllocWaves = p.fastBlocks >= 64 ? fslots : p.fastBlocks;
		p.spillPerWaveBytes = (size_t)flat->spill.totalWords * sizeof(uint32_t);
		const unsigned listSlots = L2_LIST_BLOCKS_PER_CU * numCUs;
		p.listBlocks = p.generalBlocks < listSlots ? p.generalBlocks : listSlots;
	}
	if (p.route == L2_ROUTE_JOIN) p.joinBlocks = blocksFor( ndocs, (size_t)numCUs * L2_JOIN_WAVES_PER_CU);
	auto want = []( uint64_t fromInput, uint64_t reserved) { const uint64_t n = fromInput < reserved ? reserved : fromInput; return n > 0xFFFFFFFFull ? 0xFFFFFFFFull : n; };
	p.wantResults = want( (uint64_t)nlexems*2 + 1024, minResults);
	p.wantItems = want( (uint64_t)nlexems*6 + 1024, minItems);
	return p;
}

}
```

### struspattern_amd/csrc/l2_plan.hpp

```cpp
#ifndef SPA_L2_PLAN_HPP
#define SPA_L2_PLAN_HPP
#include <stdint.h>
#include <cstddef>
#include <string>
#include <vector>
#include "l2_compile.hpp"
#include "l2_device.h"
#include "l2_fast.h"
#include "l2_join.h"

namespace spa {

struct L2Switches
{
	bool fast = true;
	char fastSize = 0;
	uint32_t fastMaxRules = 2048;
	uint32_t fastMaxStaged = 32768;
	bool join = false;
	bool verbose = false;
	static L2Switches fromEnv();
};

ArenaLayout initialArena();
void layoutArena( ArenaLayout& L);
void setArena( ArenaLayout& L, uint32_t maxRules, uint32_t maxTrigs, uint32_t bucketCap, uint32_t maxItems, uint32_t maxFollow);
bool growArena( ArenaLayout& L);

struct ArenaWaves { unsigned run, alloc; };
ArenaWaves arenaWaves( size_t perWaveBytes, unsigned wanted, size_t fullSlots, unsigned multiple);

enum L2EngineKind {L2_GENERAL=0, L2_FLAT=1, L2_JOIN=2};
struct L2Engine
{
	struct Flat
	{
		bool on = false;
		std::string whyNot;
		std::vector<FastKeyInst> keyinst;
		std::vector<FastStatic> statics;
		uint32_t maxRules = 0, maxStaged = 0;
	} flat;
	struct Join
	{
		bool asked = false, on = false;
		std::string whyNot;
		std::vector<JoinKey> keytab; std::vector<JoinRule> rules; std::vector<uint32_t> filter;
		uint32_t maxRange = 0, delimiter = 0;
	} join;
	uint32_t altPrograms = 0;
	L2EngineKind kind() const	{return join.on ? L2_JOIN : flat.on ? L2_FLAT : L2_GENERAL;}
};
L2Engine chooseL2Engine( const RuleCompiler& compiler, const FlatTables& ft, uint32_t ctxFlags, const L2Switches& sw);

struct FlatPlan
{
	unsigned variant = 0;
	const char* kernelName = "(none)";
	uint32_t R = 0, T = 0;
	FastSpillLayout spill = {};
	uint32_t bucketMeta[ 16] = {};
	uint32_t expShift = 0;
};
FlatPlan planFlat( const L2Engine::Flat& flat, unsigned variant, const char* kernelName, uint32_t R, uint32_t T);

const char* l2KernelName( L2EngineKind kind, const FlatPlan* flat);

#ifndef SPA_L2_WAVES_PER_CU
#define SPA_L2_WAVES_PER_CU 12
#endif
enum {
	L2_WAVES_PER_CU=SPA_L2_WAVES_PER_CU,
	L2_JOIN_WAVES_PER_CU=32,
	L2_LIST_BLOCKS_PER_CU=2
};
enum L2Route {L2_ROUTE_GENERAL, L2_ROUTE_FLAT_LIST , L2_ROUTE_JOIN, L2_ROUTE_RERUN_LIST};
struct L2LaunchPlan
{
	L2Route route = L2_ROUTE_GENERAL;
	const char* kernelName = "(none)";
	ArenaLayout layout;
	ArenaWaves arena = {1, 1};
	unsigned generalBlocks = 1;
	size_t arenaPerWaveBytes = 0;
	unsigned arenaAllocWaves = 1;
	unsigned fastBlocks = 0;
	uint64_t spillAllocWaves = 0;
	size_t spillPerWaveBytes = 0;
	unsigned listBlocks = 0;
	unsigned joinBlocks = 0;
	uint64_t wantResults = 0, wantItems = 0;
};
L2LaunchPlan planL2Launch( L2EngineKind kind, bool rerun, unsigned numCUs, unsigned fastBlocksPerCU, size_t docsToRun, size_t ndocs, size_t nlexems,
			   const ArenaLayout& arena, const FlatPlan* flat, uint64_t minResults, uint64_t minItems);

}
#endif
```

Measured before the change: 4.260 GB/s.

## Schedule documents longest-first via device-side size-class ordering kernel

Adds a single-block kernel that buckets documents by log2 of their lexem count and writes a descending-size permutation. The general and flat matcher kernels take documents from that order through a shared cursor (nextDocument) instead of first assigning doc=blockIdx, which reduces tail imbalance when wave slots finish unevenly. In exchange it adds a serial single-workgroup pre-pass on every batch and an indirection load per document, and it breaks input locality between consecutive documents. It also adds profiling hooks, a test entry point and a wave-slot query.

```diff
diff --git a/include/strus_pattern_amd.h b/include/strus_pattern_amd.h
--- a/include/strus_pattern_amd.h
+++ b/include/strus_pattern_amd.h
@@ -80,6 +80,7 @@
 int sp_device_count(void);
 void sp_free(void* p);
 void sp_test_fail_alloc_above(uint64_t bytes);
+int sp_test_doc_order(const uint64_t* counts, size_t ndocs, uint32_t* order, double* ms, char* err, size_t errsize);
 struct sp_match_batch;
 int sp_match_batch_regroup(const sp_result_t* results, uint64_t nresults, const sp_result_item_t* items, uint64_t nitems,
 	const uint32_t* result_format, const uint32_t* item_format, const uint64_t* doc_ranges, const int32_t* doc_status,
@@ -369,6 +370,7 @@
 double sp_matcher_ctx_last_kernel_ms(sp_matcher_ctx_t* c);
 int sp_matcher_ctx_kernel_kind(const sp_matcher_ctx_t* c);
 const char* sp_matcher_ctx_kernel_name(const sp_matcher_ctx_t* c);
+unsigned sp_matcher_ctx_wave_slots(const sp_matcher_ctx_t* c);
 int sp_matcher_ctx_batch_status(sp_matcher_ctx_t* c, int32_t* status, size_t ndocs);
 int sp_matcher_ctx_grow_arena(sp_matcher_ctx_t* c);
 int sp_matcher_ctx_reserve_output(sp_matcher_ctx_t* c, uint64_t results, uint64_t items);
diff --git a/struspattern_amd/__init__.py b/struspattern_amd/__init__.py
--- a/struspattern_amd/__init__.py
+++ b/struspattern_amd/__init__.py
@@ -548,6 +548,9 @@
 
     def kernelName(self):
         return self._L.sp_matcher_ctx_kernel_name(self._h).decode()
+
+    def waveSlots(self):
+        return self._L.sp_matcher_ctx_wave_slots(self._h)
 
 
 def _serialize(L, fn, handle, err):
diff --git a/struspattern_amd/capi.py b/struspattern_amd/capi.py
--- a/struspattern_amd/capi.py
+++ b/struspattern_amd/capi.py
@@ -161,6 +161,7 @@
     "sp_device_count": (ctypes.c_int, []),
     "sp_free": (None, [c_vp]),
     "sp_test_fail_alloc_above": (None, [c_u64]),
+    "sp_test_doc_order": (ctypes.c_int, [c_vp, ctypes.c_size_t, c_vp, P(ctypes.c_double), ctypes.c_char_p, ctypes.c_size_t]),
     "sp_match_batch_regroup": (ctypes.c_int, [c_vp, c_u64, c_vp, c_u64, c_vp, c_vp, c_vp, c_vp, ctypes.c_size_t, ctypes.c_size_t, ctypes.c_size_t,
                                               ctypes.c_int, c_u32, P(SpMatchBatch), ctypes.c_char_p, ctypes.c_size_t]),
     "sp_matcher_create": (c_vp, []),
@@ -244,6 +245,7 @@
     "sp_matcher_ctx_last_kernel_ms": (ctypes.c_double, [c_vp]),
     "sp_matcher_ctx_kernel_kind": (ctypes.c_int, [c_vp]),
     "sp_matcher_ctx_kernel_name": (ctypes.c_char_p, [c_vp]),
+    "sp_matcher_ctx_wave_slots": (ctypes.c_uint, [c_vp]),
     "sp_matcher_ctx_batch_status": (ctypes.c_int, [c_vp, c_vp, ctypes.c_size_t]),
     "sp_matcher_ctx_grow_arena": (ctypes.c_int, [c_vp]),
     "sp_matcher_ctx_reserve_output": (ctypes.c_int, [c_vp, c_u64, c_u64]),
diff --git a/struspattern_amd/csrc/capi_l2.cpp b/struspattern_amd/csrc/capi_l2.cpp
--- a/struspattern_amd/csrc/capi_l2.cpp
+++ b/struspattern_amd/csrc/capi_l2.cpp
@@ -53,6 +53,32 @@
 void sp_free( void* p) { std::free( p); }
 
 void sp_test_fail_alloc_above( uint64_t bytes) { allocFailureThreshold().store( bytes, std::memory_order_relaxed); }
+
+int sp_test_doc_order( const uint64_t* counts, size_t ndocs, uint32_t* order, double* ms, char* err, size_t errsize)
+{
+	std::string msg;
+	const int rc = guardedCall( msg, SP_ERR_DEVICE, [&]{
+		if (ndocs >= 0xFFFFFFFFull) throw std::runtime_error( "too many documents in one batch");
+		std::vector<uint64_t> ranges( 2*ndocs + 2);
+		uint64_t first = 0;
+		for (size_t i=0; i<ndocs; ++i) { ranges[ 2*i] = first; ranges[ 2*i+1] = counts[ i]; first += counts[ i]; }
+		DeviceBuffer dRanges, dOrder;
+		dRanges.upload( ranges.data(), ranges.size()*sizeof(uint64_t));
+		dOrder.alloc( (ndocs+1)*sizeof(uint32_t));
+		Event e0, e1; e0.create(); e1.create();
+		const DocOrderParams O = {0, (const uint64_t*)dRanges.ptr, (uint32_t)ndocs, (uint32_t*)dOrder.ptr};
+		HIP_CHECK( launchL2DocOrder( O, 0));
+		HIP_CHECK( hipEventRecord( e0, 0));
+		HIP_CHECK( launchL2DocOrder( O, 0));
+		HIP_CHECK( hipEventRecord( e1, 0));
+		HIP_CHECK( hipStreamSynchronize( 0));
+		double t = 0;
+		if (ms) *ms = elapsedMs( e0, e1, t) ? t : -1.0;
+		if (ndocs) HIP_CHECK( hipMemcpy( order, dOrder.ptr, ndocs*sizeof(uint32_t), hipMemcpyDeviceToHost));
+	});
+	if (rc != SP_OK) copyText( err, errsize, msg.c_str());
+	return rc;
+}
 
 sp_matcher_t* sp_matcher_create(void) { try { return new sp_matcher(); } catch (...) { return 0; } }
 void sp_matcher_free( sp_matcher_t* m) { delete m; }
@@ -89,6 +115,8 @@
 
 int sp_matcher_ctx_kernel_kind( const sp_matcher_ctx_t* c) { return c->kind; }
 const char* sp_matcher_ctx_kernel_name( const sp_matcher_ctx_t* c) { return l2KernelName( c->kind, &c->flat.plan); }
+unsigned sp_matcher_ctx_wave_slots( const sp_matcher_ctx_t* c)
+{ return c->numCUs * (c->kind == L2_JOIN ? (unsigned)L2_JOIN_WAVES_PER_CU : c->kind == L2_FLAT ? c->flat.blocksPerCU : (unsigned)L2_WAVES_PER_CU); }
 
 int sp_matcher_fast_tier( const sp_matcher_t* m, char* why, size_t whysize)
 { return tierQuery( m, 0, L2_FLAT, why, whysize, 0); }
@@ -115,11 +143,11 @@
 		static const char* const routes[] = {"general", "flat+list", "join", "rerun-list"};
 		int n = std::snprintf( buf, bufsize, "engine=%s\nkind=%d\nflat_why_not=%s\njoin_why_not=%s\nalt_programs=%u\nkernel=%s\nroute=%s\n"
 			"general_blocks=%u\narena_run=%u\narena_alloc=%u\narena_alloc_waves=%u\narena_per_wave_bytes=%zu\narena_max_rules=%u\narena_scratch_cap=%u\nstop_words=%u\n"
-			"fast_blocks=%u\nspill_alloc_waves=%llu\nspill_per_wave_bytes=%zu\nlist_blocks=%u\njoin_blocks=%u\nwant_results=%llu\nwant_items=%llu\n"
+			"fast_blocks=%u\nspill_alloc_waves=%llu\nspill_per_wave_bytes=%zu\nlist_blocks=%u\njoin_blocks=%u\ndoc_order=%d\nwant_results=%llu\nwant_items=%llu\n"
 			"R=%u\nT=%u\nexp_shift=%u\nspill_words=%u\nmax_rules=%u\nmax_staged=%u\nbucket_caps=",
 			engines[ e.kind()], (int)e.kind(), e.flat.whyNot.c_str(), e.join.whyNot.c_str(), e.altPrograms, p.kernelName, routes[ p.route],
 			p.generalBlocks, p.arena.run, p.arena.alloc, p.arenaAllocWaves, p.arenaPerWaveBytes, p.layout.maxRules, p.layout.scratchCap, ft.nofStopWords,
-			p.fastBlocks, (unsigned long long)p.spillAllocWaves, p.spillPerWaveBytes, p.listBlocks, p.joinBlocks, (unsigned long long)p.wantResults, (unsigned long long)p.wantItems,
+			p.fastBlocks, (unsigned long long)p.spillAllocWaves, p.spillPerWaveBytes, p.listBlocks, p.joinBlocks, p.docOrder ? 1 : 0, (unsigned long long)p.wantResults, (unsigned long long)p.wantItems,
 			fp.R, fp.T, fp.expShift, fp.spill.totalWords, fp.spill.maxRules, fp.spill.maxStaged);
 		for (int b=0; b<16 && n >= 0 && buf && (size_t)n < bufsize; ++b) n += std::snprintf( buf+n, bufsize-n, b ? ",%u" : "%u", fp.bucketMeta[ b] >> 16);
 		if (n < 0 || !buf || (size_t)n >= bufsize) throw std::runtime_error( "buffer too small for the launch plan");
@@ -315,6 +343,7 @@
 	io.dDocRange.reserve( (ndocs+1)*2*sizeof(uint64_t));
 	io.dDocStats.reserve( (ndocs+1)*4*sizeof(uint64_t));
 	io.dDocStatus.reserve( (ndocs+1)*sizeof(int32_t));
+	if (plan.docOrder) io.dDocOrder.reserve( (ndocs+1)*sizeof(uint32_t));
 }
 
 void resetCursorAndCounters( sp_matcher_ctx* c, bool rerun, hipStream_t stream)
@@ -341,7 +370,7 @@
 void listMode( const sp_matcher_ctx* c, L2Params& P)
 {
 	P.docList = (const uint32_t*)c->exact.dDocList.ptr; P.docListCount = (const uint32_t*)c->io.dCursor.ptr + 2;
-	P.io.docCursor = (uint32_t*)c->io.dCursor.ptr + 1;
+	P.io.docCursor = (uint32_t*)c->io.dCursor.ptr + 1; P.io.docOrder = 0;
 }
 
 void launchRerun( sp_matcher_ctx* c, L2Params P, const L2LaunchPlan& plan, const std::vector<uint32_t>& rerun, hipStream_t stream)
@@ -385,6 +414,11 @@
 	F.spill = f.plan.spill; F.spillBase = (uint32_t*)f.spill.ptr();
 	F.fallbackList = (uint32_t*)c->exact.dDocList.ptr; F.fallbackCount = (uint32_t*)c->io.dCursor.ptr + 2;
 	F.diag = (uint32_t*)c->io.dCursor.ptr + 16; F.prof = (uint64_t*)((uint32_t*)c->io.dCursor.ptr + 32);
+#ifdef SPA_PROF
+	f.dProfSlots.reserve( (size_t)plan.fastBlocks*4*sizeof(uint64_t)); f.profSlots = plan.fastBlocks;
+	HIP_CHECK( hipMemsetAsync( f.dProfSlots.ptr, 0, (size_t)plan.fastBlocks*4*sizeof(uint64_t), stream));
+	F.profSlots = (uint64_t*)f.dProfSlots.ptr;
+#endif
 	HIP_CHECK( launchL2Fast( F, f.plan.variant, plan.fastBlocks, stream));
 	listMode( c, P);
 	HIP_CHECK( launchL2Match( P, plan.listBlocks, stream));
@@ -400,8 +434,14 @@
 	ensureArena( c, plan);
 	ensureOutput( c, plan, ndocs);
 	resetCursorAndCounters( c, rerun != 0, stream);
-	const L2BatchIO io = batchIO( c, d_lexems, d_origseg, d_doc_offsets, d_doc_ranges, ndocs);
+	L2BatchIO io = batchIO( c, d_lexems, d_origseg, d_doc_offsets, d_doc_ranges, ndocs);
 	HIP_CHECK( hipEventRecord( c->evStart, stream));
+	if (plan.docOrder)
+	{
+		DocOrderParams O = {io.docOffsets, io.docRangesIn, io.ndocs, (uint32_t*)c->io.dDocOrder.ptr};
+		HIP_CHECK( launchL2DocOrder( O, stream));
+		io.docOrder = O.docOrder;
+	}
 	switch (plan.route)
 	{
 		case L2_ROUTE_RERUN_LIST: launchRerun( c, generalParams( c, io, plan), plan, *rerun, stream); break;
@@ -475,6 +515,19 @@
 }
 
 double sp_matcher_ctx_last_kernel_ms( sp_matcher_ctx_t* c) { return lastKernelMs( c); }
+
+#ifdef SPA_PROF
+size_t sp_matcher_ctx_prof_slots( sp_matcher_ctx_t* c, uint64_t* out, size_t nslots)
+{
+	size_t n = c->flat.profSlots;
+	guardedCall( c->lasterror, SP_ERR_DEVICE, [&]{
+		HIP_CHECK( hipSetDevice( c->device));
+		HIP_CHECK( hipStreamSynchronize( c->lastStream));
+		if (n && nslots) copySync( c->own, out, c->flat.dProfSlots.ptr, (n < nslots ? n : nslots)*4*sizeof(uint64_t), hipMemcpyDeviceToHost);
+	});
+	return n;
+}
+#endif
 
 int sp_matcher_ctx_match_docs( sp_matcher_ctx_t* c, const sp_lexem_t* lexems, const uint32_t* origseg,
 			       const uint64_t* doc_offsets, size_t ndocs, sp_match_batch_t* out)
diff --git a/struspattern_amd/csrc/capi_l2_ctx.hpp b/struspattern_amd/csrc/capi_l2_ctx.hpp
--- a/struspattern_amd/csrc/capi_l2_ctx.hpp
+++ b/struspattern_amd/csrc/capi_l2_ctx.hpp
@@ -1,6 +1,7 @@
 #ifndef SPA_CAPI_L2_CTX_HPP
 #define SPA_CAPI_L2_CTX_HPP
 #include "l2_plan.hpp"
+#include "l2_order.h"
 #include "result_values.hpp"
 #include "capi_util.hpp"
 #include <mutex>
@@ -56,6 +57,9 @@
 		FlatPlan plan;
 		CountedBuffer spill;
 		unsigned blocksPerCU = 0;
+#ifdef SPA_PROF
+		DeviceBuffer dProfSlots; unsigned profSlots = 0;
+#endif
 	} flat;
 	struct ResultSets
 	{
@@ -70,6 +74,7 @@
 		DeviceBuffer dLexems, dOrigseg, dDocOffsets;
 		CountedBuffer results, items;
 		DeviceBuffer dDocRange, dDocStats, dDocStatus;
+		DeviceBuffer dDocOrder;
 		DeviceBuffer dResultFormat, dItemFormat;
 		bool withFormats = false, withItems = true;
 		uint64_t minResults = 0, minItems = 0;
diff --git a/struspattern_amd/csrc/l2_device.h b/struspattern_amd/csrc/l2_device.h
--- a/struspattern_amd/csrc/l2_device.h
+++ b/struspattern_amd/csrc/l2_device.h
@@ -39,6 +39,7 @@
 	uint32_t ndocs;
 	uint32_t withItems;
 	uint32_t withFormats;
+	const uint32_t* docOrder;
 };
 
 struct L2Params
diff --git a/struspattern_amd/csrc/l2_fast.h b/struspattern_amd/csrc/l2_fast.h
--- a/struspattern_amd/csrc/l2_fast.h
+++ b/struspattern_amd/csrc/l2_fast.h
@@ -157,6 +157,9 @@
 	uint32_t* diag;
 	L2BatchIO io;
 	uint64_t* prof;
+#ifdef SPA_PROF
+	uint64_t* profSlots;
+#endif
 };
 
 hipError_t launchL2Fast( const FastParams& P, unsigned variant, unsigned nblocks, hipStream_t stream);
diff --git a/struspattern_amd/csrc/l2_fast_kernel.hip b/struspattern_amd/csrc/l2_fast_kernel.hip
--- a/struspattern_amd/csrc/l2_fast_kernel.hip
+++ b/struspattern_amd/csrc/l2_fast_kernel.hip
@@ -3,6 +3,7 @@
 #include "l2_fast.h"
 #include "l2_device.h"
 #include "wave_scan.h"
+#include "doc_passes.h"
 
 using namespace spa;
 
@@ -1096,18 +1097,20 @@
 	Wave w;
 	w.sp = P.spillBase + (u64)blockIdx.x * P.spill.totalWords;
 	const u32 ndocs = P.io.ndocs;
-	const u32 waveSlot = blockIdx.x, nWaveSlots = gridDim.x;
+#ifdef SPA_PROF
+	const u32 waveSlot = blockIdx.x;
+	u64 slotFirst = 0, slotLastStart = 0, slotEnd = 0; u32 slotDocs = 0;
+#endif
 
 	for (u32 round=0; round<=ndocs; ++round)
 	{
-		u32 doc = waveSlot;
-		if (round)
-		{
-			u32 nx = 0;
-			if (LANE == 0) nx = atomicAdd( P.io.docCursor, 1u);
-			doc = nWaveSlots + uni( nx);
-		}
+		u32 doc = nextDocument( P.io.docCursor);
 		if (doc >= ndocs) break;
+		if (P.io.docOrder) doc = ldu( &P.io.docOrder[ doc]);
+#ifdef SPA_PROF
+		slotLastStart = __builtin_amdgcn_s_memrealtime();
+		if (!slotDocs++) slotFirst = slotLastStart;
+#endif
 		w.bmetaV = P.bucketMeta[ LANE & 15u]; w.bsizeV = 0; w.expCntV = 0;
 		if (LANE < 16u) { L.bsize[ LANE] = 0; L.bmeta[ LANE] = w.bmetaV; }
 		L.expCnt[ LANE] = 0;
@@ -1272,7 +1275,18 @@
 			atomicAdd( (unsigned long long*)&P.io.counters[ SPC_HANDOVER], 1ull);
 			if (P.diag) { atomicAdd( &P.diag[ 0], 1u); atomicAdd( &P.diag[ w.why & 15u], 1u); }
 		}
-	}
+#ifdef SPA_PROF
+		WAVE_FENCE();
+		slotEnd = __builtin_amdgcn_s_memrealtime();
+#endif
+	}
+#ifdef SPA_PROF
+	if (LANE == 0 && P.profSlots)
+	{
+		u64* o = P.profSlots + 4*(u64)waveSlot;
+		o[ 0] = slotFirst; o[ 1] = slotEnd; o[ 2] = slotDocs; o[ 3] = slotLastStart;
+	}
+#endif
 }
 };
 
diff --git a/struspattern_amd/csrc/l2_kernel.hip b/struspattern_amd/csrc/l2_kernel.hip
--- a/struspattern_amd/csrc/l2_kernel.hip
+++ b/struspattern_amd/csrc/l2_kernel.hip
@@ -3,6 +3,7 @@
 #include "l2_tables.h"
 #include "l2_device.h"
 #include "wave_scan.h"
+#include "doc_passes.h"
 
 using namespace spa;
 
@@ -1609,20 +1610,13 @@
 	__shared__ __attribute__((aligned(16))) u32 ldsSlice[ 64 + 16 + 64 + 512 + 16*SCRLDS_CAP + EXPLIST_CAP];
 	const WSV w( (HWS*)ldsSlice, P.arenaBase + (u64)blockIdx.x * P.arena.totalWords);
 	const u32 ndocs = P.docList ? ldu( P.docListCount) : P.io.ndocs;
-	const u32 waveSlot = blockIdx.x;
-	const u32 nWaveSlots = gridDim.x;
 
 	for (u32 round=0; round<=ndocs; ++round)
 	{
-		u32 doc = waveSlot;
-		if (round)
-		{
-			u32 nx = 0;
-			if (LANE == 0) nx = atomicAdd( P.io.docCursor, 1u);
-			doc = nWaveSlots + uni( nx);
-		}
+		u32 doc = nextDocument( P.io.docCursor);
 		if (doc >= ndocs) break;
 		if (P.docList) doc = ldu( &P.docList[ doc]);
+		else if (P.io.docOrder) doc = ldu( &P.io.docOrder[ doc]);
 		if (LANE < 16) BSIZE[ LANE] = 0;
 		WINDOW[ LANE] = 0;
 		for (u32 s=LANE; s<P.nofStopWords; s+=64) STOP[ s].timestamp = 0;
diff --git a/struspattern_amd/csrc/l2_order.h b/struspattern_amd/csrc/l2_order.h
--- /dev/null
+++ b/struspattern_amd/csrc/l2_order.h
@@ -0,0 +1,23 @@
+#ifndef SPA_L2_ORDER_H
+#define SPA_L2_ORDER_H
+#include <stdint.h>
+#include <hip/hip_runtime_api.h>
+
+namespace spa {
+
+enum { ORDER_CLASSES = 65 };
+
+struct DocOrderParams
+{
+	const uint64_t* docOffsets;
+	const uint64_t* docRangesIn;
+	uint32_t ndocs;
+	uint32_t* docOrder;
+};
+
+inline uint32_t docOrderClass( uint64_t n) { uint32_t k = 0; while (n) { ++k; n >>= 1; } return k; }
+
+hipError_t launchL2DocOrder( const DocOrderParams& P, hipStream_t stream);
+
+}
+#endif
diff --git a/struspattern_amd/csrc/l2_order_kernel.hip b/struspattern_amd/csrc/l2_order_kernel.hip
--- /dev/null
+++ b/struspattern_amd/csrc/l2_order_kernel.hip
@@ -0,0 +1,74 @@
+#include <hip/hip_runtime.h>
+#include "l2_order.h"
+#include "wave_scan.h"
+
+using namespace spa;
+
+namespace {
+
+__device__ __forceinline__ u32 classOf( const DocOrderParams& P, u64 d)
+{
+	const u64 n = P.docRangesIn ? P.docRangesIn[ 2*d+1] : P.docOffsets[ d+1] - P.docOffsets[ d];
+	return n ? 64u - (u32)__builtin_clzll( n) : 0u;
+}
+
+}
+
+extern "C" __global__ __launch_bounds__(1024) void spa_l2_doc_order_kernel( DocOrderParams P)
+{
+	__shared__ u32 next[ ORDER_CLASSES];
+	__shared__ u32 waveCnt[ 16][ ORDER_CLASSES];
+	const u32 tid = threadIdx.x, wave = tid >> 6;
+	const u64 ndocs = P.ndocs;
+	if (tid < ORDER_CLASSES) next[ tid] = 0;
+	for (u32 i=tid; i<16*ORDER_CLASSES; i+=1024) (&waveCnt[ 0][ 0])[ i] = 0;
+	__syncthreads();
+	for (u64 d=tid; d<ndocs; d+=1024) atomicAdd( &next[ classOf( P, d)], 1u);
+	__syncthreads();
+	if (tid == 0)
+	{
+		u32 at = 0;
+		for (int k=ORDER_CLASSES-1; k>=0; --k) { const u32 n = next[ k]; next[ k] = at; at += n; }
+	}
+	__syncthreads();
+	for (u64 t0=0; t0<ndocs; t0+=1024)
+	{
+		const u64 d = t0 + tid;
+		const bool have = d < ndocs;
+		const u32 k = have ? classOf( P, d) : 0xFFFFFFFFu;
+		u32 rank = 0;
+		u64 todo = __ballot( have);
+		while (todo)
+		{
+			const u32 first = (u32)__builtin_ctzll( todo);
+			const u32 kk = (u32)__builtin_amdgcn_readlane( (int)k, first);
+			const u64 m = __ballot( k == kk);
+			if (k == kk) rank = (u32)__builtin_popcountll( m & ((1ull << LANE) - 1ull));
+			if (LANE == first) waveCnt[ wave][ kk] = (u32)__builtin_popcountll( m);
+			todo &= ~m;
+		}
+		__syncthreads();
+		if (have)
+		{
+			u32 before = 0;
+			for (u32 w=0; w<16; ++w) { const u32 a = waveCnt[ w][ k]; before += w < wave ? a : 0u; }
+			P.docOrder[ next[ k] + before + rank] = (u32)d;
+		}
+		__syncthreads();
+		if (tid < ORDER_CLASSES)
+		{
+			u32 s = 0;
+			for (u32 w=0; w<16; ++w) { s += waveCnt[ w][ tid]; waveCnt[ w][ tid] = 0; }
+			next[ tid] += s;
+		}
+		__syncthreads();
+	}
+}
+
+namespace spa {
+hipError_t launchL2DocOrder( const DocOrderParams& P, hipStream_t stream)
+{
+	hipLaunchKernelGGL( spa_l2_doc_order_kernel, dim3( 1), dim3( 1024), 0, stream, P);
+	return hipGetLastError();
+}
+}
diff --git a/struspattern_amd/csrc/l2_plan.cpp b/struspattern_amd/csrc/l2_plan.cpp
--- a/struspattern_amd/csrc/l2_plan.cpp
+++ b/struspattern_amd/csrc/l2_plan.cpp
@@ -143,6 +143,7 @@
 		const unsigned listSlots = L2_LIST_BLOCKS_PER_CU * numCUs;
 		p.listBlocks = p.generalBlocks < listSlots ? p.generalBlocks : listSlots;
 	}
+	p.docOrder = (p.route == L2_ROUTE_FLAT_LIST && ndocs > p.fastBlocks) || (p.route == L2_ROUTE_GENERAL && ndocs > p.generalBlocks);
 	if (p.route == L2_ROUTE_JOIN) p.joinBlocks = blocksFor( ndocs, (size_t)numCUs * L2_JOIN_WAVES_PER_CU);
 	auto want = []( uint64_t fromInput, uint64_t reserved) { const uint64_t n = fromInput < reserved ? reserved : fromInput; return n > 0xFFFFFFFFull ? 0xFFFFFFFFull : n; };
 	p.wantResults = want( (uint64_t)nlexems*2 + 1024, minResults);
diff --git a/struspattern_amd/csrc/l2_plan.hpp b/struspattern_amd/csrc/l2_plan.hpp
--- a/struspattern_amd/csrc/l2_plan.hpp
+++ b/struspattern_amd/csrc/l2_plan.hpp
@@ -89,6 +89,7 @@
 	size_t spillPerWaveBytes = 0;
 	unsigned listBlocks = 0;
 	unsigned joinBlocks = 0;
+	bool docOrder = false;
 	uint64_t wantResults = 0, wantItems = 0;
 };
 L2LaunchPlan planL2Launch( L2EngineKind kind, bool rerun, unsigned numCUs, unsigned fastBlocksPerCU, size_t docsToRun, size_t ndocs, size_t nlexems,
```

Result: no change. 4.251 GB/s (-0.2%).
